# mapbox/robosat

Measured on AMD Instinct MI355X. Metric: 512x512 tiles/sec train+predict, 1/2/4/8 MI355X; mIoU vs CPU ref, higher is better.
Workload: dtype f32; 1 GPU; rs predict ResNet50-UNet, bs=16 3x512x512 fp32 per GPU, 2 classes (BASELINE configs[1]); parallelism=tiles sharded over 1 rank(s), no collective

## Files before the change

### include/robosat_hip.h

```cpp
#ifndef ROBOSAT_HIP_H
#define ROBOSAT_HIP_H

#include <stdint.h>

#ifdef __cplusplus
extern "C" {
#endif

#define RS_EINVAL (-22)

typedef void* rs_stream_t;

typedef uint16_t rs_bf16;
#define RS_F32 0
#define RS_BF16 1

int rs_abi_version(void);

typedef struct rs_conv_desc {
  int32_t N;
  int32_t Hs, Ws;
  int32_t C1, C2;
  int32_t ups;
  int32_t kh, kw, stride, pad;
  int32_t Ho, Wo;
  int32_t Cout;
  int32_t relu;
  int32_t stem;
} rs_conv_desc;

int rs_conv2d_fwd(const rs_conv_desc* d, const float* src1, const float* src2, const float* weight,
                  const float* scale, const float* shift, const float* residual, const float* relu_mask, float* out,
                  rs_stream_t stream);

int rs_conv2d_tile(const rs_conv_desc* d);
const char* rs_conv2d_tile_name(int tile);

int rs_pack_stem_weight(const float* w_krsc, float* packed, int Cout, int kh, int kw, int Cin, rs_stream_t stream);


int rs_nchw_to_nhwc4(const float* x, float* y, int N, int C, int H, int W, rs_stream_t stream);

int rs_maxpool2d_fwd(const float* x, float* y, uint8_t* argmax, int N, int H, int W, int C, int k, int stride, int pad,
                     int Ho, int Wo, rs_stream_t stream);

int rs_bn_fold(const float* gamma, const float* beta, const float* mean, const float* var, float eps, float* scale,
               float* shift, int C, rs_stream_t stream);

int rs_final_conv1x1(const float* x, const float* w, const float* bias, float* out, int N, int H, int W, int Cin,
                     int C, int softmax, rs_stream_t stream);



long rs_conv2d_wgrad_workspace_bytes(const rs_conv_desc* d);
int rs_conv2d_wgrad_form(const rs_conv_desc* d);
int rs_conv2d_wgrad(const rs_conv_desc* d, const float* dy, const float* src1, const float* src2, float* dw,
                    void* workspace, rs_stream_t stream);
int rs_unpack_stem_weight(const float* packed, float* w_krsc, int Cout, int kh, int kw, int Cin, rs_stream_t stream);

int rs_pack_dgrad_weight(const float* w_krsc, float* out, int Cout, int kh, int kw, int Cin, rs_stream_t stream);

long rs_bn_workspace_bytes(long M, int C);
int rs_bn_train_stats(const float* y, long M, int C, float eps, float momentum, const float* gamma, const float* beta,
                      float* mean, float* invstd, float* scale, float* shift, float* running_mean, float* running_var,
                      long long* num_batches_tracked, void* workspace, rs_stream_t stream);
int rs_bn_apply(const float* y, const float* scale, const float* shift, const float* residual, float* out, long M, int C,
                int relu, rs_stream_t stream);
int rs_bn_bwd(const float* dz, const float* zmask, const float* y, const float* mean, const float* invstd,
              const float* gamma, float* dy, float* dmasked, float* dgamma, float* dbeta, long M, int C, void* workspace,
              rs_stream_t stream);

int rs_maxpool2d_bwd(const float* dy, const uint8_t* argmax, float* dx, int N, int H, int W, int C, int k, int stride,
                     int pad, int Ho, int Wo, int accumulate, rs_stream_t stream);

int rs_upsample2x_bwd(const float* dup, float* d1, float* d2, const float* mask1, const float* mask2, int N, int H, int W,
                      int C1, int C2, int accumulate1, rs_stream_t stream);

long rs_final_conv1x1_bwd_workspace_bytes(int Cin, int C);
int rs_final_conv1x1_bwd(const float* x, const float* w, const float* dlogits, float* dx, float* dw, float* db, int N, int H,
                         int W, int Cin, int C, int relu_mask, void* workspace, rs_stream_t stream);


long rs_nll_loss_workspace_bytes(void);
int rs_nll_loss_fwd(const float* logits, const long long* targets, const float* weight, float* loss, float* stats, int N,
                    int C, int H, int W, int mode, float gamma, void* workspace, rs_stream_t stream);
int rs_nll_loss_bwd(const float* logits, const long long* targets, const float* weight, const float* stats,
                    const float* grad_out, float* dlogits, int N, int C, int H, int W, int mode, float gamma,
                    rs_stream_t stream);

long rs_miou_loss_workspace_bytes(int N, int C);
int rs_miou_loss_fwd(const float* logits, const long long* targets, const float* weight, float* loss, float* stats, int N,
                     int C, int H, int W, void* workspace, rs_stream_t stream);
int rs_miou_loss_bwd(const float* logits, const long long* targets, const float* weight, const float* stats,
                     const float* grad_out, float* dlogits, int N, int C, int H, int W, rs_stream_t stream);

long rs_lovasz_workspace_bytes(int N, int C, int H, int W);
int rs_lovasz_fwd(const float* logits, const long long* targets, float* loss, float* grad_unit, int N, int C, int H, int W,
                  void* workspace, rs_stream_t stream);
int rs_scale_by_scalar(const float* src, const float* scalar, float* dst, long n, rs_stream_t stream);

long rs_lovasz_softmax_workspace_bytes(int N, int C, int H, int W, int per_image);
int rs_lovasz_softmax_fwd(const float* logits, const long long* targets, float* loss, float* grad_unit, float* probs_out, int N,
                          int C, int H, int W, int per_image, int all_classes, void* workspace, rs_stream_t stream);

int rs_confusion_counts(const float* scores, const long long* targets, unsigned long long* counts, int N, int C, int H,
                        int W, rs_stream_t stream);


int rs_conv2d_fwd_bf16(const rs_conv_desc* d, const rs_bf16* src1, const rs_bf16* src2, const rs_bf16* weight,
                       const float* scale, const float* shift, const rs_bf16* residual, const rs_bf16* relu_mask,
                       rs_bf16* out, rs_stream_t stream);
int rs_conv2d_tile_bf16(const rs_conv_desc* d);
int rs_conv2d_config(const rs_conv_desc* d, int es, int form, int* tile, int* rowb);
int rs_conv2d_set_tuning(int tile, int rowb);
int rs_set_knob(const char* name, int value);
int rs_get_knob(const char* name, int* value);
const char* rs_conv2d_tile_name_bf16(int tile);

long rs_conv2d_wgrad_bf16_workspace_bytes(const rs_conv_desc* d);
int rs_conv2d_wgrad_bf16_form(const rs_conv_desc* d);
int rs_conv2d_wgrad_bf16_tile(const rs_conv_desc* d);
int rs_conv2d_wgrad_bf16(const rs_conv_desc* d, const rs_bf16* dy, const rs_bf16* src1, const rs_bf16* src2, float* dw,
                         void* workspace, rs_stream_t stream);

int rs_cast_f32_to_bf16(const float* src, rs_bf16* dst, long n, rs_stream_t stream);
int rs_cast_bf16_to_f32_scaled(const rs_bf16* src, float* dst, long n, float scale, rs_stream_t stream);
int rs_cast_f32_to_bf16_scaled(const float* src, rs_bf16* dst, long n, float scale, rs_stream_t stream);
int rs_pack_dgrad_weight_bf16(const float* w_krsc, rs_bf16* out, int Cout, int kh, int kw, int Cin, rs_stream_t stream);

int rs_nchw_to_nhwc4_bf16(const float* x, rs_bf16* y, int N, int C, int H, int W, rs_stream_t stream);
int rs_pack_stem_weight_bf16(const float* w_krsc, rs_bf16* packed, int Cout, int kh, int kw, int Cin, rs_stream_t stream);
int rs_stem_conv_fwd_bf16(const rs_bf16* x, const rs_bf16* w_packed, const float* scale, const float* shift, rs_bf16* out,
                          int N, int H, int W, int relu, rs_stream_t stream);
long rs_stem_conv_wgrad_bf16_workspace_bytes(int N, int H, int W);
int rs_stem_conv_wgrad_bf16(const rs_bf16* dy, const rs_bf16* x, float* dw_packed, int N, int H, int W, void* workspace,
                            rs_stream_t stream);

int rs_maxpool2d_fwd_dt(const void* x, int x_dtype, void* y, int y_dtype, uint8_t* argmax, int N, int H, int W, int C, int k,
                        int stride, int pad, int Ho, int Wo, rs_stream_t stream);
int rs_maxpool2d_bwd_dt(const void* dy, int dy_dtype, const uint8_t* argmax, void* dx, int dx_dtype, int N, int H, int W,
                        int C, int k, int stride, int pad, int Ho, int Wo, int accumulate, rs_stream_t stream);
int rs_final_conv1x1_dt(const void* x, int x_dtype, const float* w, const float* bias, float* out, int N, int H, int W,
                        int Cin, int C, int softmax, rs_stream_t stream);
int rs_final_conv1x1_bwd_dt(const void* x, const float* w, const float* dlogits, void* dx, float* dw, float* db, int dtype,
                            int N, int H, int W, int Cin, int C, int relu_mask, void* workspace, rs_stream_t stream);
int rs_bn_train_stats_dt(const void* y, int dtype, long M, int C, float eps, float momentum, const float* gamma,
                         const float* beta, float* mean, float* invstd, float* scale, float* shift, float* running_mean,
                         float* running_var, long long* num_batches_tracked, void* workspace, rs_stream_t stream);
int rs_bn_apply_dt(const void* y, const float* scale, const float* shift, const void* residual, void* out, int dtype, long M,
                   int C, int relu, rs_stream_t stream);
int rs_bn_bwd_dt(const void* dz, const void* zmask, const void* y, const float* mean, const float* invstd, const float* gamma,
                 void* dy, void* dmasked, float* dgamma, float* dbeta, int dtype, long M, int C, void* workspace,
                 rs_stream_t stream);
int rs_upsample2x_bwd_dt(const void* dup, void* d1, void* d2, const void* mask1, const void* mask2, int dtype, int N, int H,
                         int W, int C1, int C2, int accumulate1, rs_stream_t stream);

long rs_conv2d_bnstats_rows(const rs_conv_desc* d);
long rs_conv2d_bnstats_rows_dt(const rs_conv_desc* d, int dtype);
int rs_conv2d_fwd_bnstats_dt(const rs_conv_desc* d, int dtype, const void* src1, const void* src2, const void* weight,
                             void* out, float* stats_partial, rs_stream_t stream);
int rs_bn_finalize_stats(const float* partial, long rows, long M, int C, float eps, float momentum, const float* gamma,
                         const float* beta, float* mean, float* invstd, float* scale, float* shift, float* running_mean,
                         float* running_var, long long* num_batches_tracked, void* workspace, rs_stream_t stream);

int rs_pack_phase_weight_dt(const float* w_krsc, void* out, int dtype, int Cout, int Cin, rs_stream_t stream);
int rs_pack_s2_dgrad_phase_weight_dt(const float* w_krsc, void* out, int dtype, int Cout, int Cin, rs_stream_t stream);
int rs_conv2d_fwd_phase_dt(const rs_conv_desc* d, int dtype, const void* src1, const void* src2, const void* weight_phase,
                           const float* scale, const float* shift, const void* residual, const void* relu_mask, void* out,
                           rs_stream_t stream);

int rs_conv2d_phase_wino_ok(const rs_conv_desc* d);
const char* rs_conv2d_phase_wino_name(const rs_conv_desc* d);
int rs_pack_wino_phase_weight(const float* w_phase, float* u, int Cout, int Cin, rs_stream_t stream);
int rs_conv2d_fwd_phase_wino(const rs_conv_desc* d, const float* src1, const float* src2, const float* u, float* out,
                             rs_stream_t stream);
int rs_conv2d_dgrad_phase_wino_ok(const rs_conv_desc* d);
const char* rs_conv2d_dgrad_phase_wino_name(const rs_conv_desc* d);
int rs_pack_wino_dgrad_weight(const float* wd4x4, float* u, int Cin, int Cout, rs_stream_t stream);
int rs_conv2d_dgrad_phase_wino(const rs_conv_desc* d, const float* dz, const float* u, float* out, const float* mask, float* out2,
                               const float* mask2, int csplit, rs_stream_t stream);

int rs_conv2d_wino33_ok(const rs_conv_desc* d);
const char* rs_conv2d_wino33_name(const rs_conv_desc* d);
int rs_pack_wino33_weight(const float* w_krsc, float* u, int Cout, int Cin, rs_stream_t stream);
int rs_conv2d_fwd_wino33(const rs_conv_desc* d, const float* src, const float* u, const float* scale, const float* shift, float* out,
                         rs_stream_t stream);
int rs_conv2d_wino33_head_ok(const rs_conv_desc* d, int C);
const char* rs_conv2d_wino33_head_name(void);
int rs_conv2d_fwd_wino33_head(const rs_conv_desc* d, const float* src, const float* u, const float* scale, const float* shift,
                              const float* final_w, const float* final_b, int C, int mode, const double* anchors, int overlap,
                              float* out, uint8_t* qout, rs_stream_t stream);
int rs_bottleneck_tail_f32(const float* x, const float* w3, const float* scale3, const float* shift3, const float* identity,
                           const float* w1, const float* scale1, const float* shift1, float* out, float* z, long M, int C1, int Cmid,
                           int C2, rs_stream_t stream);
int rs_conv1x1_wave_f32(const float* x, const float* w, const float* scale, const float* shift, const float* residual, int relu, float* out,
                        long M, int C1, int Cout, rs_stream_t stream);
long rs_conv2d_wino33_stats_rows(const rs_conv_desc* d);
int rs_conv2d_fwd_wino33_stats(const rs_conv_desc* d, const float* src, const float* u, float* out, float* stats, rs_stream_t stream);
int rs_conv2d_dgrad_wino33(const rs_conv_desc* d, const float* dy, const float* u, const float* mask, const uint8_t* mask_bits,
                           const float* bn_y, const float* bn_mean, const float* bn_invstd, float* out, float* stats,
                           rs_stream_t stream);

int rs_pack_dgrad_phase_weight_dt(const float* w_krsc, void* out, int dtype, int Cout, int Cin, rs_stream_t stream);
typedef struct rs_wprep_item {
  const float* w;
  rs_bf16* cast;
  rs_bf16* dgrad;
  int Cout, taps, Cin;
  int tile_begin;
} rs_wprep_item;
int rs_weight_prep_bf16(const rs_wprep_item* items_dev, int n, int total_tiles, rs_stream_t stream);
int rs_weight_prep_f32(const rs_wprep_item* items_dev, int n, int total_tiles, rs_stream_t stream);
int rs_combine_dgrad_phase_weight_dt(const float* w_dgrad, void* out, int dtype, int Cout, int Cin, rs_stream_t stream);
int rs_conv2d_fwd_split_dt(const rs_conv_desc* d, int dtype, const void* src1, const void* weight, void* out1, const void* mask1,
                           void* out2, const void* mask2, int csplit, rs_stream_t stream);
int rs_cat_split_bwd_dt(const void* dcat, void* d1, void* d2, const void* mask1, const void* mask2, int dtype, int N, int H,
                        int W, int C1, int C2, int accumulate1, rs_stream_t stream);
int rs_scatter_add_stride2_dt(const void* t, void* out, int dtype, int N, int Hs, int Ws, int Ho, int Wo, int C, rs_stream_t stream);

int rs_conv2d_dgrad_bnstats_dt(const rs_conv_desc* d, int dtype, const void* dy, const void* weight, const void* residual,
                               const void* relu_mask, const void* bn_y, const float* bn_mean, const float* bn_invstd,
                               void* out, float* stats_partial, rs_stream_t stream);
int rs_bn_bwd_from_partials_dt(const void* g, const void* y, const float* mean, const float* invstd, const float* gamma,
                               void* dy, float* dgamma, float* dbeta, const float* partial, long rows, int dtype, long M,
                               int C, void* workspace, rs_stream_t stream);
int rs_bn_apply_bits_dt(const void* y, const float* scale, const float* shift, const void* residual, void* out,
                        unsigned char* bits, int dtype, long M, int C, int relu, rs_stream_t stream);
int rs_conv2d_dgrad_bnstats_bits_dt(const rs_conv_desc* d, int dtype, const void* dy, const void* weight, const void* residual,
                                    const unsigned char* relu_mask_bits, const void* bn_y, const float* bn_mean,
                                    const float* bn_invstd, void* out, float* stats_partial, rs_stream_t stream);


int rs_u8_to_nhwc4_norm(const uint8_t* img, float* out, const float* mean, const float* std, int N, int H, int W, int C,
                        rs_stream_t stream);

int rs_final_conv1x1_quantize_dt(const void* x, int x_dtype, const float* w, const float* bias, const double* anchors,
                                 uint8_t* out, int N, int H, int W, int Cin, int C, int overlap, rs_stream_t stream);

int rs_final_conv1x1_argmax_dt(const void* x, int x_dtype, const float* w, const float* bias, uint8_t* out, int N, int H,
                               int W, int Cin, int C, rs_stream_t stream);

#define RS_TTA_IN_U8 0
#define RS_TTA_IN_F32 1
#define RS_TTA_PROBS 0
#define RS_TTA_QUANTIZE 1
#define RS_TTA_ARGMAX 2
int rs_tta_fan_out(const void* x, int x_kind, const float* mean, const float* std, void* out, int out_dtype, const int* ops,
                   int V, int N, int H, int W, int C, rs_stream_t stream);
int rs_tta_merge(const float* probs, const int* ops, int V, int mode, const double* anchors, int overlap, void* out, int N,
                 int C, int H, int W, rs_stream_t stream);


int rs_confusion_matrix(const float* scores, const int64_t* targets, int64_t* counts, int N, int C, int H, int W,
                        rs_stream_t stream);

int rs_label_histogram_u8(const uint8_t* labels, long n, int64_t* counts256, rs_stream_t stream);

int rs_softvote_masks(const uint8_t* q, const double* weights, const double* anchors, uint8_t* out, int K, long P, int C,
                      rs_stream_t stream);

int rs_augment_tiles(const uint8_t* images, const uint8_t* masks, const int32_t* index, const int32_t* op, const float* mean,
                     const float* std, float* out_images, int64_t* out_masks, int N, int S, int C, rs_stream_t stream);


int rs_features_clean_form(int H, int W);
long rs_features_clean_workspace_bytes(int B, int H, int W);
int rs_features_clean(const uint8_t* images, uint8_t* out, void* workspace, int B, int H, int W, int index, int eps_open,
                      const int32_t* dx_open, int eps_close, const int32_t* dx_close, int form, rs_stream_t stream);

int rs_features_label(const uint8_t* masks, int32_t* labels, int32_t* err, int B, int H, int W, rs_stream_t stream);

int rs_features_components(const int32_t* labels, int32_t* slotmap, int32_t* raw, int32_t* table, int32_t* counters,
                           long capacity, int B, int H, int W, int min_area, rs_stream_t stream);

int rs_features_edges(const int32_t* labels, const int32_t* table, long rows, uint8_t* keep, int32_t* edges, long capacity,
                      int32_t* counter, int B, int H, int W, rs_stream_t stream);

int rs_features_halo(const uint8_t* src, uint8_t* dst, const int32_t* nbr, int T, int H, int W, int A, int fill, int crop,
                     rs_stream_t stream);
int rs_features_stitch_labels(int32_t* labels, const int32_t* nbr, int32_t* err, int T, int H, int W, rs_stream_t stream);
int rs_features_components_stitched(const int32_t* labels, const int32_t* origin, int32_t* slotmap, int32_t* raw, int32_t* table,
                                    int32_t* counters, long capacity, int T, int H, int W, int min_area, rs_stream_t stream);
int rs_features_edges_stitched(const int32_t* labels, const int32_t* nbr, const int32_t* origin, const int32_t* table, long rows,
                               uint8_t* keep, int32_t* edges, long capacity, int32_t* counter, int T, int H, int W,
                               rs_stream_t stream);

int rs_features_thin(const uint8_t* masks, uint8_t* out, void* workspace, const int32_t* nbr, int32_t* counters, int B, int H, int W,
                     int pairs, int resume, rs_stream_t stream);
int rs_features_skeleton_links(const uint8_t* skeleton, const int32_t* labels, const int32_t* nbr, const int32_t* origin,
                               const int32_t* table, long rows, uint8_t* keep, int32_t* links, long capacity, int32_t* counter, int B,
                               int H, int W, rs_stream_t stream);


#ifdef __cplusplus
}
#endif
#endif
```

### robosat_amd/_lib.py

```python

import ctypes
import os
from ctypes import POINTER, c_char_p, c_float, c_int, c_int32, c_long, c_void_p

import torch

_HERE = os.path.dirname(os.path.abspath(__file__))
LIB_PATH = os.environ.get("ROBOSAT_HIP_LIB") or os.path.join(_HERE, "librobosat_hip.so")

RS_EINVAL = -22
ABI_VERSION = 24
RS_F32, RS_BF16 = 0, 1
RS_TTA_IN_U8, RS_TTA_IN_F32 = 0, 1
RS_TTA_PROBS, RS_TTA_QUANTIZE, RS_TTA_ARGMAX = 0, 1, 2


class ConvDesc(ctypes.Structure):

    _fields_ = [
        ("N", c_int32), ("Hs", c_int32), ("Ws", c_int32), ("C1", c_int32), ("C2", c_int32), ("ups", c_int32),
        ("kh", c_int32), ("kw", c_int32), ("stride", c_int32), ("pad", c_int32), ("Ho", c_int32), ("Wo", c_int32),
        ("Cout", c_int32), ("relu", c_int32), ("stem", c_int32),
    ]


P = c_void_p

SIGNATURES = {
    "rs_abi_version": (c_int, []),
    "rs_conv2d_fwd": (c_int, [POINTER(ConvDesc), P, P, P, P, P, P, P, P, P]),
    "rs_conv2d_tile": (c_int, [POINTER(ConvDesc)]),
    "rs_conv2d_tile_name": (c_char_p, [c_int]),
    "rs_pack_stem_weight": (c_int, [P, P, c_int, c_int, c_int, c_int, P]),
    "rs_nchw_to_nhwc4": (c_int, [P, P, c_int, c_int, c_int, c_int, P]),
    "rs_maxpool2d_fwd": (c_int, [P, P, P, c_int, c_int, c_int, c_int, c_int, c_int, c_int, c_int, c_int, P]),
    "rs_bn_fold": (c_int, [P, P, P, P, c_float, P, P, c_int, P]),
    "rs_final_conv1x1": (c_int, [P, P, P, P, c_int, c_int, c_int, c_int, c_int, c_int, P]),
    "rs_conv2d_wgrad_workspace_bytes": (c_long, [POINTER(ConvDesc)]),
    "rs_conv2d_wgrad": (c_int, [POINTER(ConvDesc), P, P, P, P, P, P]),
    "rs_unpack_stem_weight": (c_int, [P, P, c_int, c_int, c_int, c_int, P]),
    "rs_pack_dgrad_weight": (c_int, [P, P, c_int, c_int, c_int, c_int, P]),
    "rs_bn_workspace_bytes": (c_long, [c_long, c_int]),
    "rs_bn_train_stats": (c_int, [P, c_long, c_int, c_float, c_float, P, P, P, P, P, P, P, P, P, P, P]),
    "rs_bn_apply": (c_int, [P, P, P, P, P, c_long, c_int, c_int, P]),
    "rs_bn_bwd": (c_int, [P, P, P, P, P, P, P, P, P, P, c_long, c_int, P, P]),
    "rs_maxpool2d_bwd": (c_int, [P, P, P, c_int, c_int, c_int, c_int, c_int, c_int, c_int, c_int, c_int, c_int, P]),
    "rs_upsample2x_bwd": (c_int, [P, P, P, P, P, c_int, c_int, c_int, c_int, c_int, c_int, P]),
    "rs_final_conv1x1_bwd_workspace_bytes": (c_long, [c_int, c_int]),
    "rs_final_conv1x1_bwd": (c_int, [P, P, P, P, P, P, c_int, c_int, c_int, c_int, c_int, c_int, P, P]),
    "rs_nll_loss_workspace_bytes": (c_long, []),
    "rs_nll_loss_fwd": (c_int, [P, P, P, P, P, c_int, c_int, c_int, c_int, c_int, c_float, P, P]),
    "rs_nll_loss_bwd": (c_int, [P, P, P, P, P, P, c_int, c_int, c_int, c_int, c_int, c_float, P]),
    "rs_miou_loss_workspace_bytes": (c_long, [c_int, c_int]),
    "rs_miou_loss_fwd": (c_int, [P, P, P, P, P, c_int, c_int, c_int, c_int, P, P]),
    "rs_miou_loss_bwd": (c_int, [P, P, P, P, P, P, c_int, c_int, c_int, c_int, P]),
    "rs_lovasz_workspace_bytes": (c_long, [c_int, c_int, c_int, c_int]),
    "rs_lovasz_fwd": (c_int, [P, P, P, P, c_int, c_int, c_int, c_int, P, P]),
    "rs_scale_by_scalar": (c_int, [P, P, P, c_long, P]),
    "rs_lovasz_softmax_workspace_bytes": (c_long, [c_int, c_int, c_int, c_int, c_int]),
    "rs_lovasz_softmax_fwd": (c_int, [P, P, P, P, P, c_int, c_int, c_int, c_int, c_int, c_int, P, P]),
    "rs_confusion_counts": (c_int, [P, P, P, c_int, c_int, c_int, c_int, P]),
    "rs_conv2d_fwd_bf16": (c_int, [POINTER(ConvDesc), P, P, P, P, P, P, P, P, P]),
    "rs_conv2d_tile_bf16": (c_int, [POINTER(ConvDesc)]),
    "rs_conv2d_config": (c_int, [POINTER(ConvDesc), c_int, c_int, POINTER(c_int), POINTER(c_int)]),
    "rs_conv2d_set_tuning": (c_int, [c_int, c_int]),
    "rs_set_knob": (c_int, [c_char_p, c_int]),
    "rs_get_knob": (c_int, [c_char_p, POINTER(c_int)]),
    "rs_conv2d_tile_name_bf16": (c_char_p, [c_int]),
    "rs_conv2d_wgrad_bf16_workspace_bytes": (c_long, [POINTER(ConvDesc)]),
    "rs_conv2d_wgrad_bf16_form": (c_int, [POINTER(ConvDesc)]),
    "rs_conv2d_wgrad_form": (c_int, [POINTER(ConvDesc)]),
    "rs_conv2d_wgrad_bf16_tile": (c_int, [POINTER(ConvDesc)]),
    "rs_conv2d_wgrad_bf16": (c_int, [POINTER(ConvDesc), P, P, P, P, P, P]),
    "rs_cast_f32_to_bf16": (c_int, [P, P, c_long, P]),
    "rs_cast_bf16_to_f32_scaled": (c_int, [P, P, c_long, c_float, P]),
    "rs_cast_f32_to_bf16_scaled": (c_int, [P, P, c_long, c_float, P]),
    "rs_weight_prep_bf16": (c_int, [P, c_int, c_int, P]),
    "rs_weight_prep_f32": (c_int, [P, c_int, c_int, P]),
    "rs_pack_dgrad_weight_bf16": (c_int, [P, P, c_int, c_int, c_int, c_int, P]),
    "rs_maxpool2d_fwd_dt": (c_int, [P, c_int, P, c_int, P, c_int, c_int, c_int, c_int, c_int, c_int, c_int, c_int, c_int, P]),
    "rs_maxpool2d_bwd_dt": (c_int, [P, c_int, P, P, c_int, c_int, c_int, c_int, c_int, c_int, c_int, c_int, c_int, c_int, c_int, P]),
    "rs_final_conv1x1_dt": (c_int, [P, c_int, P, P, P, c_int, c_int, c_int, c_int, c_int, c_int, P]),
    "rs_final_conv1x1_bwd_dt": (c_int, [P, P, P, P, P, P, c_int, c_int, c_int, c_int, c_int, c_int, c_int, P, P]),
    "rs_bn_train_stats_dt": (c_int, [P, c_int, c_long, c_int, c_float, c_float, P, P, P, P, P, P, P, P, P, P, P]),
    "rs_bn_apply_dt": (c_int, [P, P, P, P, P, c_int, c_long, c_int, c_int, P]),
    "rs_bn_bwd_dt": (c_int, [P, P, P, P, P, P, P, P, P, P, c_int, c_long, c_int, P, P]),
    "rs_upsample2x_bwd_dt": (c_int, [P, P, P, P, P, c_int, c_int, c_int, c_int, c_int, c_int, c_int, P]),
    "rs_conv2d_bnstats_rows": (c_long, [POINTER(ConvDesc)]),
    "rs_conv2d_bnstats_rows_dt": (c_long, [POINTER(ConvDesc), c_int]),
    "rs_conv2d_fwd_bnstats_dt": (c_int, [POINTER(ConvDesc), c_int, P, P, P, P, P, P]),
    "rs_bn_finalize_stats": (c_int, [P, c_long, c_long, c_int, c_float, c_float, P, P, P, P, P, P, P, P, P, P, P]),
    "rs_pack_phase_weight_dt": (c_int, [P, P, c_int, c_int, c_int, P]),
    "rs_pack_s2_dgrad_phase_weight_dt": (c_int, [P, P, c_int, c_int, c_int, P]),
    "rs_conv2d_fwd_phase_dt": (c_int, [POINTER(ConvDesc), c_int, P, P, P, P, P, P, P, P, P]),
    "rs_conv2d_phase_wino_ok": (c_int, [POINTER(ConvDesc)]),
    "rs_conv2d_phase_wino_name": (c_char_p, [POINTER(ConvDesc)]),
    "rs_pack_wino_phase_weight": (c_int, [P, P, c_int, c_int, P]),
    "rs_conv2d_fwd_phase_wino": (c_int, [POINTER(ConvDesc), P, P, P, P, P]),
    "rs_conv2d_dgrad_phase_wino_ok": (c_int, [POINTER(ConvDesc)]),
    "rs_conv2d_dgrad_phase_wino_name": (c_char_p, [POINTER(ConvDesc)]),
    "rs_pack_wino_dgrad_weight": (c_int, [P, P, c_int, c_int, P]),
    "rs_conv2d_dgrad_phase_wino": (c_int, [POINTER(ConvDesc), P, P, P, P, P, P, c_int, P]),
    "rs_conv2d_wino33_ok": (c_int, [POINTER(ConvDesc)]),
    "rs_conv2d_wino33_name": (c_char_p, [POINTER(ConvDesc)]),
    "rs_pack_wino33_weight": (c_int, [P, P, c_int, c_int, P]),
    "rs_conv2d_fwd_wino33": (c_int, [POINTER(ConvDesc), P, P, P, P, P, P]),
    "rs_conv2d_wino33_head_ok": (c_int, [POINTER(ConvDesc), c_int]),
    "rs_conv2d_wino33_head_name": (c_char_p, []),
    "rs_conv2d_fwd_wino33_head": (c_int, [POINTER(ConvDesc), P, P, P, P, P, P, c_int, c_int, P, c_int, P, P, P]),
    "rs_bottleneck_tail_f32": (c_int, [P, P, P, P, P, P, P, P, P, P, c_long, c_int, c_int, c_int, P]),
    "rs_conv1x1_wave_f32": (c_int, [P, P, P, P, P, c_int, P, c_long, c_int, c_int, P]),
    "rs_conv2d_wino33_stats_rows": (c_long, [POINTER(ConvDesc)]),
    "rs_conv2d_fwd_wino33_stats": (c_int, [POINTER(ConvDesc), P, P, P, P, P]),
    "rs_conv2d_dgrad_wino33": (c_int, [POINTER(ConvDesc), P, P, P, P, P, P, P, P, P, P]),
    "rs_pack_dgrad_phase_weight_dt": (c_int, [P, P, c_int, c_int, c_int, P]),
    "rs_combine_dgrad_phase_weight_dt": (c_int, [P, P, c_int, c_int, c_int, P]),
    "rs_conv2d_fwd_split_dt": (c_int, [POINTER(ConvDesc), c_int, P, P, P, P, P, P, c_int, P]),
    "rs_cat_split_bwd_dt": (c_int, [P, P, P, P, P, c_int, c_int, c_int, c_int, c_int, c_int, c_int, P]),
    "rs_scatter_add_stride2_dt": (c_int, [P, P, c_int, c_int, c_int, c_int, c_int, c_int, c_int, P]),
    "rs_conv2d_dgrad_bnstats_dt": (c_int, [POINTER(ConvDesc), c_int, P, P, P, P, P, P, P, P, P, P]),
    "rs_bn_bwd_from_partials_dt": (c_int, [P, P, P, P, P, P, P, P, P, c_long, c_int, c_long, c_int, P, P]),
    "rs_bn_apply_bits_dt": (c_int, [P, P, P, P, P, P, c_int, c_long, c_int, c_int, P]),
    "rs_conv2d_dgrad_bnstats_bits_dt": (c_int, [POINTER(ConvDesc), c_int, P, P, P, P, P, P, P, P, P, P]),
    "rs_nchw_to_nhwc4_bf16": (c_int, [P, P, c_int, c_int, c_int, c_int, P]),
    "rs_pack_stem_weight_bf16": (c_int, [P, P, c_int, c_int, c_int, c_int, P]),
    "rs_stem_conv_fwd_bf16": (c_int, [P, P, P, P, P, c_int, c_int, c_int, c_int, P]),
    "rs_stem_conv_wgrad_bf16_workspace_bytes": (c_long, [c_int, c_int, c_int]),
    "rs_stem_conv_wgrad_bf16": (c_int, [P, P, P, c_int, c_int, c_int, P, P]),
    "rs_u8_to_nhwc4_norm": (c_int, [P, P, POINTER(c_float), POINTER(c_float), c_int, c_int, c_int, c_int, P]),
    "rs_final_conv1x1_quantize_dt": (c_int, [P, c_int, P, P, P, P, c_int, c_int, c_int, c_int, c_int, c_int, P]),
    "rs_final_conv1x1_argmax_dt": (c_int, [P, c_int, P, P, P, c_int, c_int, c_int, c_int, c_int, P]),
    "rs_tta_fan_out": (c_int, [P, c_int, POINTER(c_float), POINTER(c_float), P, c_int, POINTER(c_int), c_int, c_int, c_int, c_int, c_int, P]),
    "rs_tta_merge": (c_int, [P, POINTER(c_int), c_int, c_int, P, c_int, P, c_int, c_int, c_int, c_int, P]),
    "rs_confusion_matrix": (c_int, [P, P, P, c_int, c_int, c_int, c_int, P]),
    "rs_label_histogram_u8": (c_int, [P, c_long, P, P]),
    "rs_softvote_masks": (c_int, [P, P, P, P, c_int, c_long, c_int, P]),
    "rs_augment_tiles": (c_int, [P, P, P, P, POINTER(c_float), POINTER(c_float), P, P, c_int, c_int, c_int, P]),
    "rs_features_clean_form": (c_int, [c_int, c_int]),
    "rs_features_clean_workspace_bytes": (c_long, [c_int, c_int, c_int]),
    "rs_features_clean": (c_int, [P, P, P, c_int, c_int, c_int, c_int, c_int, POINTER(c_int32), c_int, POINTER(c_int32), c_int, P]),
    "rs_features_label": (c_int, [P, P, P, c_int, c_int, c_int, P]),
    "rs_features_components": (c_int, [P, P, P, P, P, c_long, c_int, c_int, c_int, c_int, P]),
    "rs_features_edges": (c_int, [P, P, c_long, P, P, c_long, P, c_int, c_int, c_int, P]),
    "rs_features_halo": (c_int, [P, P, P, c_int, c_int, c_int, c_int, c_int, c_int, P]),
    "rs_features_stitch_labels": (c_int, [P, P, P, c_int, c_int, c_int, P]),
    "rs_features_components_stitched": (c_int, [P, P, P, P, P, P, c_long, c_int, c_int, c_int, c_int, P]),
    "rs_features_edges_stitched": (c_int, [P, P, P, P, c_long, P, P, c_long, P, c_int, c_int, c_int, P]),
    "rs_features_thin": (c_int, [P, P, P, P, P, c_int, c_int, c_int, c_int, c_int, P]),
    "rs_features_skeleton_links": (c_int, [P, P, P, P, P, c_long, P, P, c_long, P, c_int, c_int, c_int, P]),
}

_lib = None


def kernel_source_digest():

    import hashlib

    h = hashlib.sha256()
    src = os.path.join(_HERE, "csrc")
    names = sorted(n for n in os.listdir(src) if n.endswith((".hip", ".h")))
    for path in [os.path.join(src, n) for n in names] + [os.path.join(os.path.dirname(_HERE), "include", "robosat_hip.h")]:
        h.update(os.path.basename(path).encode() + b"\0")
        with open(path, "rb") as fp:
            h.update(fp.read())
    return h.hexdigest()[:16]


def lib():

    global _lib
    if _lib is None:
        if not os.path.exists(LIB_PATH):
            raise RuntimeError(
                "robosat_amd: {} is missing -- the MI355X kernels are not built and there is no CPU fallback. "
                "Build with `python -c 'import __graft_entry__ as g; g.build()'` "
                "(or `make -C robosat_amd/csrc`).".format(LIB_PATH)
            )
        handle = ctypes.CDLL(LIB_PATH, mode=ctypes.RTLD_GLOBAL)
        for name, (restype, argtypes) in SIGNATURES.items():
            fn = getattr(handle, name)
            fn.restype, fn.argtypes = restype, argtypes
        got = handle.rs_abi_version()
        if got != ABI_VERSION:
            raise RuntimeError("robosat_amd: librobosat_hip.so ABI {} != expected {}".format(got, ABI_VERSION))
        _lib = handle
    return _lib


def check(rc, what):
    if rc != 0:
        if rc == RS_EINVAL:
            raise ValueError("{}: invalid arguments (RS_EINVAL)".format(what))
        raise RuntimeError("{}: HIP error {}".format(what, rc))
```

### robosat_amd/csrc/common.h

```cpp
#pragma once
#include <hip/hip_runtime.h>
#include <stdint.h>

#include "../../include/robosat_hip.h"

typedef float f32x4 __attribute__((ext_vector_type(4)));
typedef float f32x16 __attribute__((ext_vector_type(16)));
typedef __bf16 bf16_t;
typedef __bf16 bf16x4 __attribute__((ext_vector_type(4)));
typedef __bf16 bf16x8 __attribute__((ext_vector_type(8)));
typedef unsigned int u32x2 __attribute__((ext_vector_type(2)));
typedef unsigned int u32x4 __attribute__((ext_vector_type(4)));
typedef short s16x4 __attribute__((ext_vector_type(4)));
typedef short s16x8 __attribute__((ext_vector_type(8)));

__device__ __forceinline__ f32x4 rs_ld4(const float* p) { return *reinterpret_cast<const f32x4*>(p); }
__device__ __forceinline__ f32x4 rs_ld4(const bf16_t* p) {
  return __builtin_convertvector(*reinterpret_cast<const bf16x4*>(p), f32x4);
}
__device__ __forceinline__ void rs_st4(float* p, f32x4 v) { *reinterpret_cast<f32x4*>(p) = v; }
__device__ __forceinline__ void rs_st4(bf16_t* p, f32x4 v) {
  *reinterpret_cast<bf16x4*>(p) = __builtin_convertvector(v, bf16x4);
}
__device__ __forceinline__ float rs_ld1(const float* p) { return *p; }
__device__ __forceinline__ float rs_ld1(const bf16_t* p) { return (float)*p; }

template <int V>
struct rs_vecf {
  float v[V];
};
template <int V, typename T>
__device__ __forceinline__ rs_vecf<V> rs_ldv(const T* p) {
  rs_vecf<V> r;
  if constexpr (V == 4) {
    const f32x4 t = rs_ld4(p);
#pragma unroll
    for (int e = 0; e < 4; ++e) r.v[e] = t[e];
  } else if constexpr (sizeof(T) == 2) {
    const bf16x8 t = *reinterpret_cast<const bf16x8*>(p);
#pragma unroll
    for (int e = 0; e < 8; ++e) r.v[e] = (float)t[e];
  } else {
    const f32x4 a = *reinterpret_cast<const f32x4*>(p), b = *(reinterpret_cast<const f32x4*>(p) + 1);
#pragma unroll
    for (int e = 0; e < 4; ++e) r.v[e] = a[e], r.v[4 + e] = b[e];
  }
  return r;
}
template <int V, typename T>
__device__ __forceinline__ void rs_stv(T* p, const rs_vecf<V>& r) {
  if constexpr (V == 4) {
    rs_st4(p, f32x4{r.v[0], r.v[1], r.v[2], r.v[3]});
  } else if constexpr (sizeof(T) == 2) {
    bf16x8 t;
#pragma unroll
    for (int e = 0; e < 8; ++e) t[e] = (bf16_t)r.v[e];
    *reinterpret_cast<bf16x8*>(p) = t;
  } else {
    *reinterpret_cast<f32x4*>(p) = f32x4{r.v[0], r.v[1], r.v[2], r.v[3]};
    *(reinterpret_cast<f32x4*>(p) + 1) = f32x4{r.v[4], r.v[5], r.v[6], r.v[7]};
  }
}

__device__ __forceinline__ void rs_ld_row32(const bf16_t* p, float (&v)[32]) {
  bf16x8 t[4];
#pragma unroll
  for (int j = 0; j < 4; ++j) t[j] = *reinterpret_cast<const bf16x8*>(p + j * 8);
#pragma unroll
  for (int j = 0; j < 4; ++j)
#pragma unroll
    for (int e = 0; e < 8; ++e) v[j * 8 + e] = (float)t[j][e];
}
__device__ __forceinline__ void rs_ld_row32(const float* p, float (&v)[32]) {
  f32x4 t[8];
#pragma unroll
  for (int j = 0; j < 8; ++j) t[j] = *reinterpret_cast<const f32x4*>(p + j * 4);
#pragma unroll
  for (int j = 0; j < 8; ++j)
#pragma unroll
    for (int e = 0; e < 4; ++e) v[j * 4 + e] = t[j][e];
}
__device__ __forceinline__ void rs_st_row32(bf16_t* p, const float (&v)[32]) {
#pragma unroll
  for (int j = 0; j < 4; ++j) {
    bf16x8 t;
#pragma unroll
    for (int e = 0; e < 8; ++e) t[e] = (bf16_t)v[j * 8 + e];
    *reinterpret_cast<bf16x8*>(p + j * 8) = t;
  }
}
__device__ __forceinline__ void rs_st_row32(float* p, const float (&v)[32]) {
#pragma unroll
  for (int j = 0; j < 8; ++j) {
    f32x4 t;
#pragma unroll
    for (int e = 0; e < 4; ++e) t[e] = v[j * 4 + e];
    *reinterpret_cast<f32x4*>(p + j * 4) = t;
  }
}

#define RS_LAUNCH_RESULT() ((int)hipGetLastError())

__device__ __forceinline__ void rs_lds_writes_done() { asm volatile("s_waitcnt lgkmcnt(0)" ::: "memory"); }

__device__ __forceinline__ int rs_xcd_remap(int b, int nwg) {
  const int xcd = b & 7, k = b >> 3;
  const int q = nwg >> 3, r = nwg & 7;
  const int base = (xcd < r) ? xcd * (q + 1) : r * (q + 1) + (xcd - r) * q;
  return base + k;
}

__device__ __forceinline__ float rs_xor16_sum(float v) {
  float a = v, b = v;
  asm("s_nop 1\n\tv_permlane16_swap_b32 %0, %1" : "+v"(a), "+v"(b));
  return a + b;
}
__device__ __forceinline__ float rs_xor32_sum(float v) {
  float a = v, b = v;
  asm("s_nop 1\n\tv_permlane32_swap_b32 %0, %1" : "+v"(a), "+v"(b));
  return a + b;
}

__device__ __forceinline__ float rs_row16_sum(float v) {
  v += __builtin_bit_cast(float, __builtin_amdgcn_update_dpp(0, __builtin_bit_cast(int, v), 0x128, 0xf, 0xf, false));
  v += __builtin_bit_cast(float, __builtin_amdgcn_update_dpp(0, __builtin_bit_cast(int, v), 0x124, 0xf, 0xf, false));
  v += __builtin_bit_cast(float, __builtin_amdgcn_update_dpp(0, __builtin_bit_cast(int, v), 0x122, 0xf, 0xf, false));
  v += __builtin_bit_cast(float, __builtin_amdgcn_update_dpp(0, __builtin_bit_cast(int, v), 0x121, 0xf, 0xf, false));
  return v;
}

__device__ __forceinline__ float rs_wave_sum(float v) {
#pragma unroll
  for (int o = 32; o > 0; o >>= 1) v += __shfl_xor(v, o, 64);
  return v;
}

__device__ __forceinline__ double rs_wave_sum(double v) {
#pragma unroll
  for (int o = 32; o > 0; o >>= 1) v += __shfl_xor(v, o, 64);
  return v;
}

static inline int rs_cdiv(long a, long b) { return (int)((a + b - 1) / b); }

inline int rs_cu_count() {
  static const int n = [] {
    int dev = 0, cus = 0;
    if (hipGetDevice(&dev) != hipSuccess || hipDeviceGetAttribute(&cus, hipDeviceAttributeMultiprocessorCount, dev) != hipSuccess || cus <= 0)
      cus = 256;
    return cus;
  }();
  return n;
}

struct rs_fastdiv {
  unsigned int mul;
  unsigned int shift;
  unsigned int div;
};

static inline rs_fastdiv rs_make_fastdiv(unsigned int d) {
  rs_fastdiv f;
  unsigned int s = 0;
  while ((1ull << s) < d) ++s;
  f.shift = s;
  f.mul = (unsigned int)((((1ull << s) - d) << 32) / d + 1);
  f.div = d;
  return f;
}

__host__ __device__ __forceinline__ unsigned int rs_div(unsigned int n, const rs_fastdiv f) {
#if defined(__HIP_DEVICE_COMPILE__)
  return (__umulhi(n, f.mul) + n) >> f.shift;
#else
  return (unsigned int)((((unsigned long long)n * f.mul) >> 32) + n) >> f.shift;
#endif
}

struct RsKnobs {
  int conv_tile = -1;
  int conv_rowb = 0;
  int conv_big = 1;
  int conv_min256 = 384;
  int conv_halo = 1;
  int conv_halo_min = 192;
  int conv_halo512 = -1;
  int conv1x1_ew = -1;
  int conv1x1_np = 0;
  int conv1x1_ew_bf16 = 0;
  int halo_ko = 0;
  int wgrad_f32_phase = 1;
  int wgrad_f32_dma = -1;
  int wgrad_f32_blocks = 2048;
  int wgrad_f32_wino = 1;
  int wgrad_f32_wino_blocks = 1024;
  int wgrad_f32_wino33 = 1;
  int wgrad_f32_wino33_blocks = 256;
  int wgrad_blocks = 96;
  int wgrad_blocks_phase = 1536;
  int wgrad_phase4 = 1;
  int wgrad_blocks_phase4 = 256;
  int wgrad_ring = 3;
  int lovasz_xcd = 1;
  int wino_wide = 1;
};
__attribute__((visibility("hidden"))) RsKnobs& rs_knobs();

__attribute__((visibility("hidden"))) int rs_wgrad_thin_plan(const rs_conv_desc* d, int* blocks, int* slices);
__attribute__((visibility("hidden"))) int rs_wgrad_thin_launch(const rs_conv_desc* d, const void* dy, const void* src,
                                                               float* partial, void* stream);

__attribute__((visibility("hidden"))) int rs_conv_thin_bf16_launch(int mode, const void* src, const void* wgt, const void* mask,
                                                                   void* out, int N, int Hs, int Ws, int relu, void* stream);

__attribute__((visibility("hidden"))) long rs_reduce_scratch_floats(long n, int splits);
__attribute__((visibility("hidden"))) int rs_reduce_splits(const float* ws, float* out, long n, int splits, float* scratch,
                                                           void* stream);

__attribute__((visibility("hidden"))) int rs_conv_dma_f32(const rs_conv_desc* d, const float* src1, const float* src2,
                                                          const float* weight, const float* scale, const float* shift,
                                                          const float* residual, const float* relu_mask, float* out,
                                                          void* stream);
__attribute__((visibility("hidden"))) int rs_conv_dma_tile(const rs_conv_desc* d);
```

### robosat_amd/csrc/conv_igemm_dma.hip

```cpp
#include "conv_igemm_dma_kernel.h"

namespace {

__global__ void pack_dgrad_weight_bf16_kernel(const float* __restrict__ w, bf16_t* __restrict__ out, int Cout, int taps,
                                              int Cin) {
  __shared__ float tile[32][33];
  const int tap = blockIdx.z;
  const int ci0 = blockIdx.x * 32, co0 = blockIdx.y * 32;
  const int tx = threadIdx.x & 31, ty = threadIdx.x >> 5;
  for (int r = ty; r < 32; r += 8) {
    const int co = co0 + r, ci = ci0 + tx;
    tile[r][tx] = (co < Cout && ci < Cin) ? w[((long)co * taps + tap) * Cin + ci] : 0.f;
  }
  __syncthreads();
  const int ftap = taps - 1 - tap;
  for (int r = ty; r < 32; r += 8) {
    const int ci = ci0 + r, co = co0 + tx;
    if (ci < Cin && co < Cout) out[((long)ci * taps + ftap) * Cout + co] = (bf16_t)tile[tx][r];
  }
}

template <typename T>
__global__ __launch_bounds__(256) void weight_prep_kernel(const rs_wprep_item* __restrict__ items, int n) {
  __shared__ float tile[32][33];
  const int bid = blockIdx.x;
  int lo = 0, hi = n - 1;
  while (lo < hi) {
    const int mid = (lo + hi + 1) >> 1;
    if (items[mid].tile_begin <= bid) lo = mid;
    else hi = mid - 1;
  }
  const rs_wprep_item it = items[lo];
  int t = bid - it.tile_begin;
  const int tci = (it.Cin + 31) / 32, tco = (it.Cout + 31) / 32;
  const int ci0 = (t % tci) * 32;
  t /= tci;
  const int co0 = (t % tco) * 32;
  const int tap = t / tco;
  const int tx = threadIdx.x & 31, ty = threadIdx.x >> 5;
  T* cast = reinterpret_cast<T*>(it.cast);
  T* dgrad = reinterpret_cast<T*>(it.dgrad);
  for (int r = ty; r < 32; r += 8) {
    const int co = co0 + r, ci = ci0 + tx;
    float v = 0.f;
    if (co < it.Cout && ci < it.Cin) {
      const long i = ((long)co * it.taps + tap) * it.Cin + ci;
      v = it.w[i];
      if (cast) cast[i] = (T)v;
    }
    tile[r][tx] = v;
  }
  if (!dgrad) return;
  __syncthreads();
  const int ftap = it.taps - 1 - tap;
  for (int r = ty; r < 32; r += 8) {
    const int ci = ci0 + r, co = co0 + tx;
    if (ci < it.Cin && co < it.Cout) dgrad[((long)ci * it.taps + ftap) * it.Cout + co] = (T)tile[tx][r];
  }
}

extern "C" int rs_weight_prep_bf16(const rs_wprep_item* items_dev, int n, int total_tiles, rs_stream_t stream) {
  if (!items_dev || n <= 0 || total_tiles <= 0) return RS_EINVAL;
  weight_prep_kernel<bf16_t><<<total_tiles, 256, 0, (hipStream_t)stream>>>(items_dev, n);
  return RS_LAUNCH_RESULT();
}

extern "C" int rs_weight_prep_f32(const rs_wprep_item* items_dev, int n, int total_tiles, rs_stream_t stream) {
  if (!items_dev || n <= 0 || total_tiles <= 0) return RS_EINVAL;
  weight_prep_kernel<float><<<total_tiles, 256, 0, (hipStream_t)stream>>>(items_dev, n);
  return RS_LAUNCH_RESULT();
}

const char* const kTileNamesBf16[NTILES] = {"conv_igemm_bf16<128x128>", "conv_igemm_bf16<128x64>", "conv_igemm_bf16<128x32>",
                                            "conv_igemm_bf16<64x64>", "", "conv_igemm_bf16<256x128>",
                                            "conv_igemm_bf16<256x256>", "conv_thin_bf16", "conv_halo_bf16", "conv1x1_ew_bf16<128x128>"};
const int kTileBM[NTILES] = {128, 128, 128, 64, 128, 256, 256, 128, 256, 128};
const int kTileBN[NTILES] = {128, 64, 32, 64, 64, 128, 256, 32, 128, 64};

struct Tuning {
  int tile, rowb, big, min256, halo, halo_min, halo512;
};
Tuning tuning() {
  const RsKnobs& k = rs_knobs();
  return {k.conv_tile, k.conv_rowb, k.conv_big, k.conv_min256, k.conv_halo, k.conv_halo_min, k.conv_halo512};
}

bool valid(const rs_conv_desc* d) {
  if (!d) return false;
  if (d->N <= 0 || d->Hs <= 0 || d->Ws <= 0 || d->Ho <= 0 || d->Wo <= 0) return false;
  if (d->kh <= 0 || d->kw <= 0 || d->kh > kMaxK || d->kw > kMaxK || d->stride <= 0 || d->pad < 0) return false;
  if (d->Cout <= 0 || (d->Cout % 32) != 0) return false;
  if (d->ups < 0 || d->ups > 2 || d->stem) return false;
  if (d->C1 <= 0 || (d->C1 % 32) != 0 || d->C2 < 0 || (d->C2 % 32) != 0) return false;
  return true;
}

bool phase_ok(const rs_conv_desc* d) {
  return d->ups == 1 && d->kh == 3 && d->kw == 3 && d->stride == 1 && d->pad == 1 && d->Ho == 2 * d->Hs && d->Wo == 2 * d->Ws;
}

int pick_tile(const rs_conv_desc* d, bool phase4 = false, int es = 4, bool stats = false) {
  const long M = phase4 ? (long)d->N * d->Hs * d->Ws * 4 : (long)d->N * d->Ho * d->Wo;
  const long want = 512;
  const Tuning tu = tuning();
  const int ft = tu.tile;
  if (ft >= 0 && ft < NTILES && ft != TSTEM_RESERVED && ft != TTHIN && ft != THALO && ft != TEW && (d->Cout % kTileBN[ft] == 0 || (ft == T128x128 && d->Cout > 128)) &&
      (ft != T256x256 || (es == 2 && !stats)))
    return ft;
  if (tu.big && es == 2 && !stats) {
    const long mrows = phase4 ? (long)d->N * d->Hs * d->Ws : M;
    const long nph = phase4 ? 4 : 1;
    const long nk128 = (long)(phase4 ? 4 : d->kh * d->kw) * (d->C1 + d->C2) * es / 128;
    if (d->Cout % 256 == 0 && nk128 >= ((phase4 || d->kh > 1) ? 16 : 32) && rs_cdiv(mrows, 256) * (d->Cout / 256) * nph >= tu.min256) return T256x256;
  }
  if (es == 4 && !stats && !phase4 && (long)d->kh * d->kw * (d->C1 + d->C2) <= 64 && d->Cout % 64 == 0 && (long)rs_cdiv(M, 128) * (d->Cout / 64) >= want)
    return T128x64;
  if (d->Cout % 128 == 0 && (long)rs_cdiv(M, 128) * (d->Cout / 128) >= want) return T128x128;
  if (d->Cout > 128 && d->Cout % 128 != 0 && (long)rs_cdiv(d->Cout, 128) * 128 * 4 <= (long)d->Cout * 5 &&
      (long)rs_cdiv(M, 128) * rs_cdiv(d->Cout, 128) >= want)
    return T128x128;
  if (d->Cout % 64 == 0) {
    if ((long)rs_cdiv(M, 128) * (d->Cout / 64) >= want) return T128x64;
    return T64x64;
  }
  return T128x32;
}

int pick_rowb(const rs_conv_desc* d, int es, bool phase4 = false, bool stats = false) {
  const int forced = tuning().rowb;
  const int tile = pick_tile(d, phase4, es, stats);
  if (forced == 64 || forced == 128) return forced;
  const long blocks = (long)rs_cdiv((long)d->N * d->Ho * d->Wo, kTileBM[tile]) * rs_cdiv(d->Cout, kTileBN[tile]);
  const long nk128 = (long)(phase4 ? 4 : d->kh * d->kw) * (d->C1 + d->C2) * es / 128;
  if (es == 4) return (nk128 <= 16 || blocks >= 2048) ? 64 : 128;
  if (tile == T256x256) return nk128 <= 8 ? 64 : 128;
  if (kTileBN[tile] <= 64) return nk128 <= 4 ? 64 : 128;
  if (phase4 || d->kh == 4) return 128;
  if (nk128 <= 8 || (blocks >= 2048 && nk128 <= 24)) return 64;
  return 128;
}

void launch(int rowb, bool phase4, int epi, int tile, int grid, hipStream_t s, const ConvArgsT<float>& a) {
  if (phase4) rs_conv_launch_f32_phase_eval(tile, rowb, grid, s, a);
  else if (epi == EPI_STATS) rs_conv_launch_f32_plain_stats(tile, rowb, grid, s, a);
  else if (epi == EPI_BWD) rs_conv_launch_f32_plain_bwd(tile, rowb, grid, s, a);
  else rs_conv_launch_f32_plain_eval(tile, rowb, grid, s, a);
}
void launch(int rowb, bool phase4, int epi, int tile, int grid, hipStream_t s, const ConvArgsT<bf16_t>& a) {
  if (phase4) rs_conv_launch_bf16_phase_eval(tile, rowb, grid, s, a);
  else if (epi == EPI_STATS) rs_conv_launch_bf16_plain_stats(tile, rowb, grid, s, a);
  else if (epi == EPI_BWD) rs_conv_launch_bf16_plain_bwd(tile, rowb, grid, s, a);
  else rs_conv_launch_bf16_plain_eval(tile, rowb, grid, s, a);
}

int thin_mode(const rs_conv_desc* d, bool phase4, bool plain_epilogue) {
  const int ft = tuning().tile;
  if (!plain_epilogue || (ft != -1 && ft != TTHIN) || d->C2 != 0) return -1;
  if (phase4) return (d->C1 == 128 && d->Cout == 32) ? 1 : -1;
  if (d->ups != 0) return -1;
  if (d->kh == 3 && d->kw == 3 && d->stride == 1 && d->pad == 1 && d->C1 == 32 && d->Cout == 32 && d->Ho == d->Hs && d->Wo == d->Ws) return 0;
  if (d->kh == 4 && d->kw == 4 && d->stride == 2 && d->pad == 1 && d->C1 == 32 && d->Cout == 128 && 2 * d->Ho == d->Hs && 2 * d->Wo == d->Ws)
    return 2;
  return -1;
}

int halo_mode(const rs_conv_desc* d, bool phase4, int csplit, int epi, int* bn_out, int* bm_out = nullptr) {
  const Tuning tu = tuning();
  if (!tu.halo || (tu.tile != -1 && tu.tile != THALO)) return HALO_NONE;
  bool big = tu.tile == THALO ? tu.rowb == 64 : tu.halo512 != 0;
  const bool c64 = (d->C1 % 64) == 0 && (d->C2 % 64) == 0;
  if ((d->C1 % 32) != 0 || (d->C2 % 32) != 0) return HALO_NONE;
  int bn;
  if (d->Cout % 128 == 0) bn = 128;
  else if (d->Cout > 128 && (long)rs_cdiv(d->Cout, 128) * 128 * 4 <= (long)d->Cout * 5) bn = 128;
  else if (d->Cout % 64 == 0) bn = 64;
  else return HALO_NONE;
  if (csplit > 0 && (csplit % bn) != 0) return HALO_NONE;
  int mode, gh, gw;
  if (phase4) {
    mode = HALO_PHASE, gh = d->Hs, gw = d->Ws;
  } else if (d->ups == 0 && d->kh == 3 && d->kw == 3 && d->stride == 1 && d->pad == 1 && d->Ho == d->Hs && d->Wo == d->Ws) {
    mode = HALO_33, gh = d->Ho, gw = d->Wo;
  } else if (d->ups == 0 && d->kh == 4 && d->kw == 4 && d->stride == 2 && d->pad == 1 && d->Hs == 2 * d->Ho && d->Ws == 2 * d->Wo && d->C2 == 0) {
    mode = HALO_DG4, gh = d->Ho, gw = d->Wo;
  } else {
    return HALO_NONE;
  }
  if (mode != HALO_33 && epi != EPI_EVAL) return HALO_NONE;
  if (tu.tile != THALO && tu.halo512 < 0) big = (long)d->N * (gh / 16) * (gw / 32) >= 256;
  if (big && (bn != 128 || (gh % 16) != 0)) big = false;
  if (!big && !c64) return HALO_NONE;
  const int ph = big ? 16 : 8;
  if ((gh % ph) != 0 || (gw % 32) != 0) return HALO_NONE;
  const long cmax = d->C1 > d->C2 ? d->C1 : d->C2;
  if ((long)d->Hs * d->Ws * cmax * 2 >= (1L << 31)) return HALO_NONE;
  const long blocks = (long)d->N * (gh / ph) * (gw / 32) * rs_cdiv(d->Cout, bn) * (phase4 ? 4 : 1);
  if (tu.tile != THALO) {
    if (blocks < tu.halo_min) return HALO_NONE;
    if (mode == HALO_33 && bn != 128) return HALO_NONE;
    if (mode == HALO_PHASE && d->Cout % 256 == 0) return HALO_NONE;
    if (mode == HALO_DG4 && d->C1 < 128) return HALO_NONE;
  }
  if (bn_out) *bn_out = bn;
  if (bm_out) *bm_out = ph * 32;
  return mode;
}

bool ew_f32_mode(const rs_conv_desc* d, bool phase4, bool plain) {
  const int ew = rs_knobs().conv1x1_ew;
  return ew != 0 && tuning().tile < 0 && !phase4 && plain && rs_conv1x1_ew_f32_ok(d) && (ew > 0 || d->C1 <= 64);
}

bool np_f32_mode(const rs_conv_desc* d, bool phase4, bool plain, bool has_res) {
  const int np = rs_knobs().conv1x1_np;
  return np != 0 && tuning().tile < 0 && !phase4 && plain && rs_conv1x1_np_f32_ok(d) && (np > 0 || (has_res && d->C1 >= 128 && d->C1 <= 512));
}

template <typename T>
int conv_fwd(const rs_conv_desc* d, const void* src1, const void* src2, const void* weight, const float* scale,
             const float* shift, const void* residual, const void* relu_mask, void* out, rs_stream_t stream,
             float* stats = nullptr, const void* bn_y = nullptr, const float* bn_mean = nullptr,
             const float* bn_invstd = nullptr, bool phase4 = false, void* out2 = nullptr, const void* mask2 = nullptr,
             int csplit = 0, const unsigned char* mask_bits = nullptr) {
  if (!valid(d) || !src1 || !weight || !out) return RS_EINVAL;
  if (mask_bits && (relu_mask || !bn_y || (d->Cout & 7))) return RS_EINVAL;
  if (out2 && (csplit <= 0 || csplit >= d->Cout || residual || stats)) return RS_EINVAL;
  if (phase4 && (!phase_ok(d) || stats)) return RS_EINVAL;
  if (d->C2 > 0 && !src2) return RS_EINVAL;
  constexpr long ES = (long)sizeof(T);
  if constexpr (sizeof(T) == 2) {
    const int tm = thin_mode(d, phase4, !scale && !shift && !residual && !stats && !out2);
    if (tm >= 0) {
      const int rc = rs_conv_thin_bf16_launch(tm, src1, weight, relu_mask, out, d->N, d->Hs, d->Ws, d->relu, stream);
      if (rc != RS_EINVAL) return rc;
    }
  }
  ConvArgsT<T> a;
  a.src1 = reinterpret_cast<const T*>(src1);
  a.src2 = reinterpret_cast<const T*>(src2);
  a.wgt = reinterpret_cast<const T*>(weight);
  a.scale = scale;
  a.shift = shift;
  a.res = reinterpret_cast<const T*>(residual);
  a.mask = reinterpret_cast<const T*>(relu_mask);
  a.out = reinterpret_cast<T*>(out);
  a.stats = stats;
  a.bn_y = reinterpret_cast<const T*>(bn_y);
  a.bn_mean = bn_mean;
  a.bn_invstd = bn_invstd;
  a.mask_bits = mask_bits;
  a.out2 = reinterpret_cast<T*>(out2);
  a.mask2 = reinterpret_cast<const T*>(mask2);
  a.csplit = csplit;
  a.N = d->N;
  a.Hs = d->Hs;
  a.Ws = d->Ws;
  a.C1 = d->C1;
  a.C2 = d->C2;
  a.phase4 = phase4 ? 1 : 0;
  a.ups = phase4 ? 0 : d->ups;
  a.Hv = a.ups == 0 ? d->Hs : (a.ups == 1 ? 2 * d->Hs : 2 * d->Hs - 1);
  a.Wv = a.ups == 0 ? d->Ws : (a.ups == 1 ? 2 * d->Ws : 2 * d->Ws - 1);
  a.kh = phase4 ? 2 : d->kh;
  a.kw = phase4 ? 2 : d->kw;
  a.stride = d->stride;
  a.pad = d->pad;
  a.Ho = d->Ho;
  a.Wo = d->Wo;
  a.Cout = d->Cout;
  if ((long)d->N * d->Ho * d->Wo >= (1L << 31)) return RS_EINVAL;
  const long M = phase4 ? (long)d->N * d->Hs * d->Ws : (long)d->N * d->Ho * d->Wo;
  a.M = (int)M;
  {
    const long cmax = d->C1 > d->C2 ? d->C1 : d->C2;
    const long img_bytes = (long)d->Hs * d->Ws * cmax * ES;
    const long rows_per_image = phase4 ? (long)d->Hs * d->Ws : (long)d->Ho * d->Wo;
    const long span = (512 / rows_per_image + 2) * img_bytes;
    if (span >= (1L << 31)) return RS_EINVAL;
    if ((long)d->Cout * d->kh * d->kw * (d->C1 + d->C2) * ES >= (1L << 31)) return RS_EINVAL;
  }
  const int kc128 = 128 / (int)ES;
  const bool can128 = d->C1 % kc128 == 0 && d->C2 % kc128 == 0;
  const int kc = (can128 && pick_rowb(d, (int)ES, phase4, stats != nullptr) == 128) ? kc128 : kc128 / 2;
  a.cpt = (d->C1 + d->C2) / kc;
  a.ntaps = a.kh * a.kw;
  a.nk = a.ntaps * a.cpt;
  a.Kw = a.nk * kc;
  a.relu = d->relu;
  a.tpx = a.tpi = 0;

  int epi = EPI_EVAL;
  if (stats) {
    epi = bn_y ? EPI_BWD : EPI_STATS;
    if (scale || shift || d->relu || out2) return RS_EINVAL;
    if (epi == EPI_STATS && (residual || relu_mask)) return RS_EINVAL;
    if (epi == EPI_BWD && (!bn_mean || !bn_invstd)) return RS_EINVAL;
  }
  if constexpr (sizeof(T) == 4) {
    if (ew_f32_mode(d, phase4, epi == EPI_EVAL && !relu_mask && !out2 && !mask_bits)) return rs_conv1x1_ew_f32_launch(a, (hipStream_t)stream);
#ifdef RS_EXP_BUILD
    if (np_f32_mode(d, phase4, epi == EPI_EVAL && !relu_mask && !out2 && !mask_bits, residual != nullptr)) return rs_conv1x1_np_f32_launch(a, (hipStream_t)stream);
#endif
  }
  if constexpr (sizeof(T) == 2) {
    int bn = 0, bm = 256;
    const int hm = halo_mode(d, phase4, out2 ? csplit : 0, epi, &bn, &bm);
    if (hm != HALO_NONE) {
      const int gh = hm == HALO_PHASE ? d->Hs : d->Ho, gw = hm == HALO_PHASE ? d->Ws : d->Wo;
      const int ctot = d->C1 + d->C2;
      a.cpt = ctot / (bm == 512 ? 32 : 64);
      a.nk = a.cpt * (hm == HALO_DG4 ? 4 : 1);
      a.Kw = (hm == HALO_PHASE ? 4 : (hm == HALO_33 ? 9 : 16)) * ctot;
      a.tpx = gw / 32;
      a.tpi = a.tpx * (gh / (bm / 32));
      a.ntiles = rs_cdiv(d->Cout, bn);
      const int grid = d->N * a.tpi * a.ntiles * (phase4 ? 4 : 1);
      hipStream_t hs = (hipStream_t)stream;
      if (bm == 512) bn |= 0x1000;
      if (hm == HALO_33) rs_conv_launch_bf16_halo33(bn, epi, grid, hs, a);
#ifdef RS_HALO_KO_BUILD
      else if (hm == HALO_PHASE && bn == 128 && rs_knobs().halo_ko) rs_conv_launch_bf16_halo_phase_ko(rs_knobs().halo_ko, grid, hs, a);
#endif
      else if (hm == HALO_PHASE) rs_conv_launch_bf16_halo_phase(bn, 0, grid, hs, a);
      else rs_conv_launch_bf16_halo_dg4(bn, 0, grid, hs, a);
      return RS_LAUNCH_RESULT();
    }
  }

  const int tile = pick_tile(d, phase4, (int)ES, stats != nullptr);
#ifdef RS_EXP_BUILD
  if constexpr (sizeof(T) == 2) {
    if (rs_knobs().conv1x1_ew_bf16 > 0 && tuning().tile < 0 && epi == EPI_STATS && !phase4 && kTileBM[tile] == 128 &&
        rs_conv1x1_ew_bf16_stats_ok(d))
      return rs_conv1x1_ew_bf16_stats_launch(a, (hipStream_t)stream);
  }
#endif
  if (out2 && (csplit % kTileBN[tile]) != 0) return RS_EINVAL;
  a.ntiles = rs_cdiv(d->Cout, kTileBN[tile]);
  const int grid = rs_cdiv(M, kTileBM[tile]) * a.ntiles * (phase4 ? 4 : 1);
  hipStream_t s = (hipStream_t)stream;
  launch(kc == kc128 ? 128 : 64, phase4, epi, tile, grid, s, a);
  return RS_LAUNCH_RESULT();
}

}

int rs_conv_dma_f32(const rs_conv_desc* d, const float* src1, const float* src2, const float* weight, const float* scale,
                    const float* shift, const float* residual, const float* relu_mask, float* out, void* stream) {
  return conv_fwd<float>(d, src1, src2, weight, scale, shift, residual, relu_mask, out, stream);
}

int rs_conv_dma_tile(const rs_conv_desc* d) { return valid(d) ? pick_tile(d) : RS_EINVAL; }

extern "C" int rs_conv2d_set_tuning(int tile, int rowb) {
  if (tile < -1 || tile >= NTILES || tile == TSTEM_RESERVED || tile == TEW || (rowb != 0 && rowb != 64 && rowb != 128)) return RS_EINVAL;
  rs_knobs().conv_tile = tile;
  rs_knobs().conv_rowb = rowb;
  return 0;
}

extern "C" int rs_conv2d_config(const rs_conv_desc* d, int es, int form, int* tile, int* rowb) {
  if (form < 0 || form > 3) return RS_EINVAL;
  const int phase4 = form & 1;
  const bool plain = (form & 2) == 0;
  if (!valid(d) || (es != 2 && es != 4) || (phase4 && !phase_ok(d))) return RS_EINVAL;
  const int kc128 = 128 / es;
  const bool can128 = d->C1 % kc128 == 0 && d->C2 % kc128 == 0;
  if (es == 2 && thin_mode(d, phase4 != 0, true) >= 0) {
    if (tile) *tile = TTHIN;
    if (rowb) *rowb = d->C1 * 2;
    return 0;
  }
  if (es == 2) {
    int bn = 0, bm = 256;
    if (halo_mode(d, phase4 != 0, 0, EPI_EVAL, &bn, &bm) != HALO_NONE) {
      if (tile) *tile = THALO;
      if (rowb) *rowb = bn | (bm == 512 ? 0x1000 : 0);
      return 0;
    }
  }
  if (es == 4 && ew_f32_mode(d, phase4 != 0, plain)) {
    if (tile) *tile = TEW;
    if (rowb) *rowb = 64;
    return 0;
  }
  if (tile) *tile = pick_tile(d, phase4 != 0, es);
  if (rowb) *rowb = (can128 && pick_rowb(d, es, phase4 != 0) == 128) ? 128 : 64;
  return 0;
}

template <typename T>
__global__ void pack_phase_weight_kernel(const float* __restrict__ w, T* __restrict__ out, int Cout, int Cin, long total) {
  const long i = (long)blockIdx.x * blockDim.x + threadIdx.x;
  if (i >= total) return;
  const int ci = (int)(i % Cin);
  long t = i / Cin;
  const int s = (int)(t & 1), r = (int)((t >> 1) & 1);
  t >>= 2;
  const int co = (int)(t % Cout);
  const int ph = (int)(t / Cout), py = ph >> 1, px = ph & 1;
  const int ky0 = py == 0 ? (r == 0 ? 0 : 1) : (r == 0 ? 0 : 2), ky1 = py == 0 ? (r == 0 ? 0 : 2) : (r == 0 ? 1 : 2);
  const int kx0 = px == 0 ? (s == 0 ? 0 : 1) : (s == 0 ? 0 : 2), kx1 = px == 0 ? (s == 0 ? 0 : 2) : (s == 0 ? 1 : 2);
  float acc = 0.f;
  for (int ky = ky0; ky <= ky1; ++ky)
    for (int kx = kx0; kx <= kx1; ++kx) acc += w[(((long)co * 3 + ky) * 3 + kx) * Cin + ci];
  out[i] = (T)acc;
}

template <typename T>
__global__ void pack_s2_dgrad_phase_weight_kernel(const float* __restrict__ w, T* __restrict__ out, int Cout, int Cin, long total) {
  const long i = (long)blockIdx.x * blockDim.x + threadIdx.x;
  if (i >= total) return;
  const int cd = (int)(i % Cout);
  long t = i / Cout;
  const int s = (int)(t & 1), r = (int)((t >> 1) & 1);
  t >>= 2;
  const int cg = (int)(t % Cin);
  const int ph = (int)(t / Cin), py = ph >> 1, px = ph & 1;
  const int ky = py == 0 ? (r == 1 ? 1 : -1) : (r == 0 ? 2 : 0);
  const int kx = px == 0 ? (s == 1 ? 1 : -1) : (s == 0 ? 2 : 0);
  out[i] = (T)((ky < 0 || kx < 0) ? 0.f : w[(((long)cd * 3 + ky) * 3 + kx) * Cin + cg]);
}

template <typename T>
__global__ void pack_dgrad_phase_weight_kernel(const float* __restrict__ w, T* __restrict__ out, int Cout, int Cin, long total) {
  const long i = (long)blockIdx.x * blockDim.x + threadIdx.x;
  if (i >= total) return;
  const int co = (int)(i % Cout);
  long t = i / Cout;
  const int tx = (int)(t & 3), ty = (int)((t >> 2) & 3);
  const int ci = (int)(t >> 4);
  const int ky0 = ty == 0 ? 2 : (ty == 1 ? 1 : 0), ky1 = ty == 0 ? 2 : (ty == 1 ? 2 : (ty == 2 ? 1 : 0));
  const int kx0 = tx == 0 ? 2 : (tx == 1 ? 1 : 0), kx1 = tx == 0 ? 2 : (tx == 1 ? 2 : (tx == 2 ? 1 : 0));
  float acc = 0.f;
  for (int ky = ky0; ky <= ky1; ++ky)
    for (int kx = kx0; kx <= kx1; ++kx) acc += w[(((long)co * 3 + ky) * 3 + kx) * Cin + ci];
  out[i] = (T)acc;
}

template <typename T>
__global__ void combine_dgrad_phase_weight_kernel(const float* __restrict__ wt, T* __restrict__ out, int Cout, long total) {
  const long i = (long)blockIdx.x * blockDim.x + threadIdx.x;
  if (i >= total) return;
  const int co = (int)(i % Cout);
  long t = i / Cout;
  const int tx = (int)(t & 3), ty = (int)((t >> 2) & 3);
  const long ci = t >> 4;
  const int ky0 = ty == 0 ? 2 : (ty == 1 ? 1 : 0), ky1 = ty == 0 ? 2 : (ty == 1 ? 2 : (ty == 2 ? 1 : 0));
  const int kx0 = tx == 0 ? 2 : (tx == 1 ? 1 : 0), kx1 = tx == 0 ? 2 : (tx == 1 ? 2 : (tx == 2 ? 1 : 0));
  float acc = 0.f;
  for (int ky = ky0; ky <= ky1; ++ky)
    for (int kx = kx0; kx <= kx1; ++kx) acc += wt[(ci * 9 + (8 - (ky * 3 + kx))) * Cout + co];
  out[i] = (T)acc;
}

extern "C" int rs_combine_dgrad_phase_weight_dt(const float* w_dgrad, void* out, int dtype, int Cout, int Cin,
                                                rs_stream_t stream) {
  if (!w_dgrad || !out || Cout <= 0 || Cin <= 0) return RS_EINVAL;
  const long total = 16L * Cout * Cin;
  hipStream_t s = (hipStream_t)stream;
  if (dtype == RS_F32)
    combine_dgrad_phase_weight_kernel<float><<<rs_cdiv(total, 256), 256, 0, s>>>(w_dgrad, reinterpret_cast<float*>(out), Cout, total);
  else if (dtype == RS_BF16)
    combine_dgrad_phase_weight_kernel<bf16_t><<<rs_cdiv(total, 256), 256, 0, s>>>(w_dgrad, reinterpret_cast<bf16_t*>(out), Cout, total);
  else
    return RS_EINVAL;
  return RS_LAUNCH_RESULT();
}

extern "C" int rs_pack_dgrad_phase_weight_dt(const float* w_krsc, void* out, int dtype, int Cout, int Cin, rs_stream_t stream) {
  if (!w_krsc || !out || Cout <= 0 || Cin <= 0) return RS_EINVAL;
  const long total = 16L * Cout * Cin;
  hipStream_t s = (hipStream_t)stream;
  if (dtype == RS_F32)
    pack_dgrad_phase_weight_kernel<float><<<rs_cdiv(total, 256), 256, 0, s>>>(w_krsc, reinterpret_cast<float*>(out), Cout, Cin, total);
  else if (dtype == RS_BF16)
    pack_dgrad_phase_weight_kernel<bf16_t><<<rs_cdiv(total, 256), 256, 0, s>>>(w_krsc, reinterpret_cast<bf16_t*>(out), Cout, Cin, total);
  else
    return RS_EINVAL;
  return RS_LAUNCH_RESULT();
}

extern "C" int rs_pack_s2_dgrad_phase_weight_dt(const float* w_krsc, void* out, int dtype, int Cout, int Cin, rs_stream_t stream) {
  if (!w_krsc || !out || Cout <= 0 || Cin <= 0) return RS_EINVAL;
  const long total = 16L * Cout * Cin;
  hipStream_t s = (hipStream_t)stream;
  if (dtype == RS_F32)
    pack_s2_dgrad_phase_weight_kernel<float><<<rs_cdiv(total, 256), 256, 0, s>>>(w_krsc, reinterpret_cast<float*>(out), Cout, Cin, total);
  else if (dtype == RS_BF16)
    pack_s2_dgrad_phase_weight_kernel<bf16_t><<<rs_cdiv(total, 256), 256, 0, s>>>(w_krsc, reinterpret_cast<bf16_t*>(out), Cout, Cin, total);
  else
    return RS_EINVAL;
  return RS_LAUNCH_RESULT();
}

extern "C" int rs_pack_phase_weight_dt(const float* w_krsc, void* out, int dtype, int Cout, int Cin, rs_stream_t stream) {
  if (!w_krsc || !out || Cout <= 0 || Cin <= 0) return RS_EINVAL;
  const long total = 16L * Cout * Cin;
  hipStream_t s = (hipStream_t)stream;
  if (dtype == RS_F32)
    pack_phase_weight_kernel<float><<<rs_cdiv(total, 256), 256, 0, s>>>(w_krsc, reinterpret_cast<float*>(out), Cout, Cin, total);
  else if (dtype == RS_BF16)
    pack_phase_weight_kernel<bf16_t><<<rs_cdiv(total, 256), 256, 0, s>>>(w_krsc, reinterpret_cast<bf16_t*>(out), Cout, Cin, total);
  else
    return RS_EINVAL;
  return RS_LAUNCH_RESULT();
}

extern "C" int rs_conv2d_fwd_split_dt(const rs_conv_desc* d, int dtype, const void* src1, const void* weight, void* out1,
                                      const void* mask1, void* out2, const void* mask2, int csplit, rs_stream_t stream) {
  if (!out2 || (d && d->C2 != 0)) return RS_EINVAL;
  if (dtype == RS_F32)
    return conv_fwd<float>(d, src1, nullptr, weight, nullptr, nullptr, nullptr, mask1, out1, stream, nullptr, nullptr, nullptr,
                           nullptr, false, out2, mask2, csplit);
  if (dtype == RS_BF16)
    return conv_fwd<bf16_t>(d, src1, nullptr, weight, nullptr, nullptr, nullptr, mask1, out1, stream, nullptr, nullptr,
                            nullptr, nullptr, false, out2, mask2, csplit);
  return RS_EINVAL;
}

extern "C" int rs_conv2d_fwd_phase_dt(const rs_conv_desc* d, int dtype, const void* src1, const void* src2,
                                      const void* weight_phase, const float* scale, const float* shift,
                                      const void* residual, const void* relu_mask, void* out, rs_stream_t stream) {
  if (dtype == RS_F32)
    return conv_fwd<float>(d, src1, src2, weight_phase, scale, shift, residual, relu_mask, out, stream, nullptr, nullptr,
                           nullptr, nullptr, true);
  if (dtype == RS_BF16)
    return conv_fwd<bf16_t>(d, src1, src2, weight_phase, scale, shift, residual, relu_mask, out, stream, nullptr, nullptr,
                            nullptr, nullptr, true);
  return RS_EINVAL;
}

extern "C" long rs_conv2d_bnstats_rows(const rs_conv_desc* d) {
  if (!valid(d)) return RS_EINVAL;
  return rs_cdiv((long)d->N * d->Ho * d->Wo, kTileBM[pick_tile(d, false, 4, true)]);
}

extern "C" long rs_conv2d_bnstats_rows_dt(const rs_conv_desc* d, int dtype) {
  if (!valid(d) || (dtype != RS_F32 && dtype != RS_BF16)) return RS_EINVAL;
  int bn = 0, bm = 256;
  if (dtype == RS_BF16 && halo_mode(d, false, 0, EPI_STATS, &bn, &bm) != HALO_NONE) return (long)d->N * (d->Ho / (bm / 32)) * (d->Wo / 32);
  return rs_conv2d_bnstats_rows(d);
}

extern "C" int rs_conv2d_dgrad_bnstats_dt(const rs_conv_desc* d, int dtype, const void* dy, const void* weight,
                                          const void* residual, const void* relu_mask, const void* bn_y,
                                          const float* bn_mean, const float* bn_invstd, void* out, float* stats_partial,
                                          rs_stream_t stream) {
  if (!stats_partial || !bn_y || !bn_mean || !bn_invstd || (d && d->C2 != 0)) return RS_EINVAL;
  if (dtype == RS_F32)
    return conv_fwd<float>(d, dy, nullptr, weight, nullptr, nullptr, residual, relu_mask, out, stream, stats_partial, bn_y,
                           bn_mean, bn_invstd);
  if (dtype == RS_BF16)
    return conv_fwd<bf16_t>(d, dy, nullptr, weight, nullptr, nullptr, residual, relu_mask, out, stream, stats_partial, bn_y,
                            bn_mean, bn_invstd);
  return RS_EINVAL;
}

extern "C" int rs_conv2d_dgrad_bnstats_bits_dt(const rs_conv_desc* d, int dtype, const void* dy, const void* weight,
                                               const void* residual, const unsigned char* relu_mask_bits, const void* bn_y,
                                               const float* bn_mean, const float* bn_invstd, void* out, float* stats_partial,
                                               rs_stream_t stream) {
  if (!stats_partial || !bn_y || !bn_mean || !bn_invstd || !relu_mask_bits || (d && d->C2 != 0)) return RS_EINVAL;
  if (dtype == RS_F32)
    return conv_fwd<float>(d, dy, nullptr, weight, nullptr, nullptr, residual, nullptr, out, stream, stats_partial, bn_y, bn_mean,
                           bn_invstd, false, nullptr, nullptr, 0, relu_mask_bits);
  if (dtype == RS_BF16)
    return conv_fwd<bf16_t>(d, dy, nullptr, weight, nullptr, nullptr, residual, nullptr, out, stream, stats_partial, bn_y, bn_mean,
                            bn_invstd, false, nullptr, nullptr, 0, relu_mask_bits);
  return RS_EINVAL;
}

extern "C" int rs_conv2d_fwd_bnstats_dt(const rs_conv_desc* d, int dtype, const void* src1, const void* src2,
                                        const void* weight, void* out, float* stats_partial, rs_stream_t stream) {
  if (!stats_partial) return RS_EINVAL;
  if (dtype == RS_F32) return conv_fwd<float>(d, src1, src2, weight, nullptr, nullptr, nullptr, nullptr, out, stream, stats_partial);
  if (dtype == RS_BF16) return conv_fwd<bf16_t>(d, src1, src2, weight, nullptr, nullptr, nullptr, nullptr, out, stream, stats_partial);
  return RS_EINVAL;
}

extern "C" int rs_conv2d_tile_bf16(const rs_conv_desc* d) { return valid(d) ? pick_tile(d, false, 2) : RS_EINVAL; }

extern "C" const char* rs_conv2d_tile_name_bf16(int tile) {
  return (tile >= 0 && tile < NTILES) ? kTileNamesBf16[tile] : "";
}

extern "C" int rs_conv2d_fwd_bf16(const rs_conv_desc* d, const rs_bf16* src1, const rs_bf16* src2, const rs_bf16* weight,
                                  const float* scale, const float* shift, const rs_bf16* residual, const rs_bf16* relu_mask,
                                  rs_bf16* out, rs_stream_t stream) {
  return conv_fwd<bf16_t>(d, src1, src2, weight, scale, shift, residual, relu_mask, out, stream);
}

extern "C" int rs_pack_dgrad_weight_bf16(const float* w_krsc, rs_bf16* out, int Cout, int kh, int kw, int Cin,
                                         rs_stream_t stream) {
  if (!w_krsc || !out || Cout <= 0 || kh <= 0 || kw <= 0 || Cin <= 0) return RS_EINVAL;
  dim3 grid(rs_cdiv(Cin, 32), rs_cdiv(Cout, 32), kh * kw);
  pack_dgrad_weight_bf16_kernel<<<grid, 256, 0, (hipStream_t)stream>>>(w_krsc, reinterpret_cast<bf16_t*>(out), Cout, kh * kw,
                                                                       Cin);
  return RS_LAUNCH_RESULT();
}
```

### robosat_amd/csrc/conv_igemm_dma_kernel.h

```cpp
#pragma once
#include <stdlib.h>

#include <type_traits>
#include <utility>

#include "lds_dma.h"

enum { EPI_EVAL = 0, EPI_STATS = 1, EPI_BWD = 2 };
constexpr int kMaxK = 4;
enum Tile { T128x128 = 0, T128x64, T128x32, T64x64, TSTEM_RESERVED, T256x128, T256x256, TTHIN, THALO, TEW, NTILES };
enum { HALO_NONE = 0, HALO_33 = 1, HALO_PHASE = 2, HALO_DG4 = 3 };

template <typename T>
struct ConvArgsT {
  const T* src1;
  const T* src2;
  const T* wgt;
  const float* scale;
  const float* shift;
  const T* res;
  const T* mask;
  T* out;
  float* stats;
  const T* bn_y;
  const float* bn_mean;
  const float* bn_invstd;
  const unsigned char* mask_bits;
  T* out2;
  const T* mask2;
  int csplit;
  int N, Hs, Ws, C1, C2, Hv, Wv, ups;
  int kh, kw, stride, pad, Ho, Wo, Cout;
  int M, cpt, nk, Kw, relu, ntiles, ntaps, phase4;
  int tpx, tpi;
};


#define RS_CONV_LAUNCHER(name, T) \
  __attribute__((visibility("hidden"))) void name(int tile, int rowb, int grid, hipStream_t s, const ConvArgsT<T>& a)
RS_CONV_LAUNCHER(rs_conv_launch_f32_plain_eval, float);
RS_CONV_LAUNCHER(rs_conv_launch_f32_plain_stats, float);
RS_CONV_LAUNCHER(rs_conv_launch_f32_plain_bwd, float);
RS_CONV_LAUNCHER(rs_conv_launch_f32_phase_eval, float);
RS_CONV_LAUNCHER(rs_conv_launch_bf16_plain_eval, bf16_t);
RS_CONV_LAUNCHER(rs_conv_launch_bf16_plain_stats, bf16_t);
RS_CONV_LAUNCHER(rs_conv_launch_bf16_plain_bwd, bf16_t);
RS_CONV_LAUNCHER(rs_conv_launch_bf16_phase_eval, bf16_t);
RS_CONV_LAUNCHER(rs_conv_launch_bf16_halo33, bf16_t);
RS_CONV_LAUNCHER(rs_conv_launch_bf16_halo_phase, bf16_t);
RS_CONV_LAUNCHER(rs_conv_launch_bf16_halo_dg4, bf16_t);
__attribute__((visibility("hidden"))) void rs_conv_launch_bf16_halo_phase_ko(int ko, int grid, hipStream_t s, const ConvArgsT<bf16_t>& a);
__attribute__((visibility("hidden"))) int rs_conv1x1_ew_f32_ok(const rs_conv_desc* d);
__attribute__((visibility("hidden"))) int rs_conv1x1_ew_f32_launch(const ConvArgsT<float>& a, hipStream_t s);
__attribute__((visibility("hidden"))) int rs_conv1x1_np_f32_ok(const rs_conv_desc* d);
__attribute__((visibility("hidden"))) int rs_conv1x1_np_f32_launch(const ConvArgsT<float>& a, hipStream_t s);
__attribute__((visibility("hidden"))) int rs_conv1x1_ew_bf16_stats_ok(const rs_conv_desc* d);
__attribute__((visibility("hidden"))) int rs_conv1x1_ew_bf16_stats_launch(const ConvArgsT<bf16_t>& a, hipStream_t s);

#ifdef RS_CONV_INSTANTIATE
namespace {

template <typename T>
struct Piece;
template <>
struct Piece<float> {
  __device__ static __forceinline__ void load(const float* p, float (&v)[4]) {
    const f32x4 t = *reinterpret_cast<const f32x4*>(p);
#pragma unroll
    for (int e = 0; e < 4; ++e) v[e] = t[e];
  }
  __device__ static __forceinline__ void round(const float (&v)[4], float (&w)[4]) {
#pragma unroll
    for (int e = 0; e < 4; ++e) w[e] = v[e];
  }
  __device__ static __forceinline__ void store(float* p, const float (&v)[4]) {
    f32x4 t;
#pragma unroll
    for (int e = 0; e < 4; ++e) t[e] = v[e];
    *reinterpret_cast<f32x4*>(p) = t;
  }
};
template <>
struct Piece<bf16_t> {
  __device__ static __forceinline__ void load(const bf16_t* p, float (&v)[8]) {
    const bf16x8 t = *reinterpret_cast<const bf16x8*>(p);
#pragma unroll
    for (int e = 0; e < 8; ++e) v[e] = (float)t[e];
  }
  __device__ static __forceinline__ void round(const float (&v)[8], float (&w)[8]) {
#pragma unroll
    for (int e = 0; e < 8; ++e) w[e] = (float)(bf16_t)v[e];
  }
  __device__ static __forceinline__ void store(bf16_t* p, const float (&v)[8]) {
    bf16x8 t;
#pragma unroll
    for (int e = 0; e < 8; ++e) t[e] = (bf16_t)v[e];
    *reinterpret_cast<bf16x8*>(p) = t;
  }
};

__device__ __forceinline__ void mma16(f32x16& acc, const u32x4 a, const u32x4 b, bf16_t) {
  acc = __builtin_amdgcn_mfma_f32_32x32x16_bf16(__builtin_bit_cast(bf16x8, a), __builtin_bit_cast(bf16x8, b), acc, 0, 0, 0);
}
__device__ __forceinline__ void mma16(f32x16& acc, const u32x4 a, const u32x4 b, float) {
  const f32x4 fa = __builtin_bit_cast(f32x4, a), fb = __builtin_bit_cast(f32x4, b);
#pragma unroll
  for (int t = 0; t < 4; ++t) acc = __builtin_amdgcn_mfma_f32_32x32x2f32(fa[t], fb[t], acc, 0, 0, 0);
}

constexpr unsigned int kDmaClamp = 0xFFFE0000u;
constexpr int kDmaOOB = (int)0xFFFF0000u;
static_assert((unsigned int)kDmaOOB > kDmaClamp && (unsigned int)kDmaOOB - kDmaClamp == 0x10000u && 0u - (unsigned int)kDmaOOB == 0x10000u,
              "the sentinel is out of range for every descriptor, with 64 KiB for soff on either side");

template <class F, int... I>
__device__ __forceinline__ void rb_for_each(F&& f, std::integer_sequence<int, I...>) {
  (f(std::integral_constant<int, I>()), ...);
}
constexpr int halo_tap_of_piece(int j, int ntap, int njh) { return j * (ntap - 2) / njh; }
constexpr int halo_pieces_at_tap(int t, int ntap, int njh) {
  int n = 0;
  for (int j = 0; j < njh; ++j) n += halo_tap_of_piece(j, ntap, njh) == t ? 1 : 0;
  return n;
}

constexpr int conv_waves_per_simd(int nw, int bm, int bn, int rowb, int es, int epi, int halo = 0) {
  if (halo) return 2;
  const int lds = 2 * (bm + bn) * rowb + 9 * bm * 4;
  const int blocks = 160 * 1024 / lds;
  const int w = blocks * nw / 4;
  const int cap = nw == 8 ? (bm * bn >= 256 * 256 ? 1 : 2) : ((es == 4 && epi == 2 && bm * bn >= 128 * 128) ? 2 : 4);
  return w < 1 ? 1 : (w > cap ? cap : w);
}

template <typename T, int BM, int BN, int WGM, int WGN, int ROWB, bool PHASE, int EPI, int HALO = HALO_NONE, int KO = 0>
__global__ __launch_bounds__(64 * WGM * WGN, conv_waves_per_simd(WGM * WGN, BM, BN, ROWB, (int)sizeof(T), EPI, HALO)) void conv_igemm_dma(
    const ConvArgsT<T> p) {
  static_assert(WGM * WGN == 4 || WGM * WGN == 8, "4 or 8 waves per block");
  static_assert(ROWB == 128 || ROWB == 64, "a K-chunk is a 128- or 64-byte row");
  constexpr int NBUF = 2;
  constexpr int NW = WGM * WGN;
  constexpr int NT = 64 * NW;
  constexpr int ES = (int)sizeof(T);
  constexpr int EPP = 16 / ES;
  constexpr int KC = ROWB / ES;
  constexpr int WM = BM / WGM, WN = BN / WGN;
  constexpr int TM = WM / 32, TN = WN / 32;
  constexpr int CPR = ROWB / 16;
  constexpr int RI = 64 / CPR;
  constexpr int IA = BM / RI, IB = BN / RI;
  constexpr int NI = (IA + IB + NW - 1) / NW;
  constexpr int KS = CPR / 2;
  constexpr int BUF = (BM + BN) * ROWB;
  constexpr int LDO = BN + 4;
  constexpr bool HL = HALO != HALO_NONE;
  constexpr int PWD = 32, PHT = BM / 32;
  constexpr int HK = HALO == HALO_33 ? 3 : 2;
  constexpr int HNT = HK * HK;
  constexpr int HWD = PWD + HK - 1, HHT = PHT + HK - 1, HROWS = HHT * HWD;
  constexpr int NJH = ((HROWS + RI - 1) / RI + NW - 1) / NW;
  constexpr int HALOB = ((HROWS + RI - 1) / RI) * 1024;
  constexpr int HSCRATCH = 2 * HALOB;
  constexpr int HBOFF = 2 * HALOB + 1024;
  constexpr int DRING = 4;
  constexpr int BSLOT = BN * ROWB;
  constexpr int NBW = IB / NW;
  constexpr int PIPE = HL ? HBOFF + DRING * BSLOT : NBUF * BUF;
  constexpr int STAGE = WGM * 32 * LDO * 4;
  constexpr int MAINB = PIPE > STAGE ? PIPE : STAGE;
  constexpr int TABN = HL ? BM : (2 * kMaxK + 1) * BM;
  static_assert(TM >= 1 && TN >= 1, "wave tile must hold one 32x32 MFMA tile");
  static_assert((IA % NW) == 0 && IB >= 1 && (BM % RI) == 0 && (BN % RI) == 0, "DMA instruction split");
  static_assert(!HL || (sizeof(T) == 2 && NW == 8 && (IB % NW) == 0 && WM % 32 == 0 && HNT >= 4 && KS % 2 == 0 && (HALO == HALO_PHASE) == PHASE),
                "halo forms: bf16, 8 waves, whole weight DMA instructions per wave");
  static_assert(MAINB + TABN * 4 <= 160 * 1024, "LDS");

  __shared__ __attribute__((aligned(16))) unsigned char smem[MAINB + TABN * 4];
  int* taby = reinterpret_cast<int*>(smem + MAINB);
  int* tabx = taby + kMaxK * BM;
  int* orow = HL ? taby : tabx + kMaxK * BM;

  const int tid = threadIdx.x;
  const int lane = tid & 63;
  const int wave = __builtin_amdgcn_readfirstlane(tid >> 6);
  const int wm = wave / WGN, wn = wave % WGN;

  int bid = rs_xcd_remap(blockIdx.x, gridDim.x);
  int py = 0, px = 0;
  if (PHASE) {
    py = (bid >> 1) & 1;
    px = bid & 1;
    bid >>= 2;
  }
  const int mt = bid / p.ntiles, nt = bid - mt * p.ntiles;
  const int m0 = mt * BM, n0 = nt * BN;

  const int Hd = PHASE ? p.Hs : p.Ho, Wd = PHASE ? p.Ws : p.Wo;
  const int HdWd = Hd * Wd;
  int hn = 0, hy0 = 0, hx0 = 0;
  if constexpr (HL) {
    hn = __builtin_amdgcn_readfirstlane(mt / p.tpi);
    const int rem = mt - hn * p.tpi;
    const int ty = __builtin_amdgcn_readfirstlane(rem / p.tpx);
    hy0 = ty * PHT;
    hx0 = (rem - ty * p.tpx) * PWD;
  }
  const int nfirst = HL ? hn : __builtin_amdgcn_readfirstlane(m0 / HdWd);
  const int ush = p.ups ? 1 : 0;
  const int upar = p.ups == 2 ? 1 : 0;
  const int pad_y = PHASE ? 1 - py : p.pad, pad_x = PHASE ? 1 - px : p.pad;

  if constexpr (HL) {
    for (int e = tid; e < BM; e += NT) {
      const int y = hy0 + e / PWD, x = hx0 + e % PWD;
      int v = -1;
      if (y < Hd && x < Wd) v = PHASE ? (hn * p.Ho + 2 * y + py) * p.Wo + 2 * x + px : (hn * Hd + y) * Wd + x;
      orow[e] = v;
    }
  }
  for (int e = tid; e < (HL ? 0 : (p.kh + p.kw + 1) * BM); e += NT) {
    const int t = e / BM, row = e - t * BM;
    const int m = m0 + row;
    int v = -1;
    if (m < p.M) {
      const int n = m / HdWd;
      const int rem = m - n * HdWd;
      const int oy = rem / Wd;
      const int ox = rem - oy * Wd;
      if (t < p.kh) {
        const int iy = oy * p.stride - pad_y + t;
        if (((unsigned)iy < (unsigned)p.Hv) && ((iy & upar) == 0)) v = ((n - nfirst) * p.Hs + (iy >> ush)) * p.Ws;
      } else if (t < p.kh + p.kw) {
        const int ix = ox * p.stride - pad_x + (t - p.kh);
        if (((unsigned)ix < (unsigned)p.Wv) && ((ix & upar) == 0)) v = ix >> ush;
      } else {
        v = PHASE ? (n * p.Ho + 2 * oy + py) * p.Wo + 2 * ox + px : m;
      }
    }
    if (t < p.kh) taby[t * BM + row] = v;
    else if (t < p.kh + p.kw) tabx[(t - p.kh) * BM + row] = v;
    else orow[row] = v;
  }

  const long img1 = (long)p.Hs * p.Ws * p.C1;
  const long img2 = (long)p.Hs * p.Ws * p.C2;
  const __amdgpu_buffer_rsrc_t rsrc1 = rs_dma_rsrc<kDmaClamp>(p.src1 + nfirst * img1, (long)(p.N - nfirst) * img1 * ES);
  const __amdgpu_buffer_rsrc_t rsrc2 = rs_dma_rsrc<kDmaClamp>(p.C2 ? p.src2 + nfirst * img2 : p.src1, (long)(p.N - nfirst) * img2 * ES);
  const __amdgpu_buffer_rsrc_t rsrcw =
      rs_dma_rsrc<kDmaClamp>(p.wgt + (long)(2 * py + px) * p.Cout * p.Kw, (long)p.Cout * p.Kw * ES);

  const int ra = lane / CPR, pp = lane % CPR;
  const int fsw = ROWB == 128 ? ((4 * (wave & 1) + (ra >> 1)) & 7) : ((ra >> 2) & 3);
  const int gp = pp ^ fsw;
  const unsigned int lds0 = __builtin_amdgcn_readfirstlane(rs_lds_addr(smem));
  constexpr int NIA = IA / NW;
  int wrow[NI];
#pragma unroll
  for (int j = 0; j < NI; ++j) wrow[j] = ((n0 + RI * (wave + NW * j - IA) + ra) * p.Kw + gp * EPP) * ES;
  __syncthreads();

  int pbase[NIA];
  auto load_tap = [&](int (&dst)[NIA], int r, int s_, bool first) __attribute__((always_inline)) {
    const int cs2 = (first ? p.C1 : p.C2) * ES;
#pragma unroll
    for (int j = 0; j < NIA; ++j) {
      const int row = RI * (wave + NW * j) + ra;
      const int y = taby[r * BM + row], x = tabx[s_ * BM + row];
      dst[j] = (y | x) < 0 ? kDmaOOB : (y + x) * cs2 + gp * 16;
    }
  };
  int lr = 0, ls = 0, lc = 0, lk = 0;
  unsigned int fL = lds0;
  __amdgpu_buffer_rsrc_t frs = rsrc1;
  int fsa = 0, fsb = 0;
  auto begin_chunk = [&](int buf) __attribute__((always_inline)) {
    const int c0 = lc * KC;
    const bool first = c0 < p.C1;
    if (lc == 0 || c0 == p.C1) load_tap(pbase, lr, ls, first);
    fL = lds0 + buf * BUF;
    frs = first ? rsrc1 : rsrc2;
    fsa = (first ? c0 : c0 - p.C1) * ES;
    fsb = lk * ROWB;
    ++lk;
    ++lc;
    const int w1 = (lc == p.cpt) ? 1 : 0;
    lc = w1 ? 0 : lc;
    ls += w1;
    const int w2 = (ls == p.kw) ? 1 : 0;
    ls = w2 ? 0 : ls;
    lr += w2;
  };
  auto issue_piece = [&](int j) __attribute__((always_inline)) {
    const int ii = wave + NW * j;
    if (j < NIA) {
      rs_dma16(frs, fL + ii * 1024, pbase[j], fsa);
    } else if ((IB % NW) == 0 || ii < IA + IB) {
      rs_dma16(rsrcw, fL + ii * 1024, wrow[j], fsb);
    }
  };

  f32x16 acc[TN][TM];
#pragma unroll
  for (int a = 0; a < TN; ++a)
#pragma unroll
    for (int b = 0; b < TM; ++b)
#pragma unroll
      for (int r = 0; r < 16; ++r) acc[a][b][r] = 0.f;

  const int frow = lane & 31;
  const int fl = ROWB == 128 ? ((frow >> 1) & 7) : ((frow >> 2) & 3);
  int foff[KS];
#pragma unroll
  for (int s = 0; s < KS; ++s) foff[s] = ((2 * s + (lane >> 5)) ^ fl) * 16;
  const int abase = (wm * WM + frow) * ROWB;
  const int bbase = (BM + wn * WN + frow) * ROWB;

  auto read_frag = [&](const unsigned char* L, int s, u32x4 (&a)[TM], u32x4 (&b)[TN]) __attribute__((always_inline)) {
#pragma unroll
    for (int tm = 0; tm < TM; ++tm) a[tm] = *reinterpret_cast<const u32x4*>(L + abase + 32 * tm * ROWB + foff[s]);
#pragma unroll
    for (int tn = 0; tn < TN; ++tn) b[tn] = *reinterpret_cast<const u32x4*>(L + bbase + 32 * tn * ROWB + foff[s]);
  };
  if constexpr (!HL) {
  if (p.nk > 0) {
    begin_chunk(0);
#pragma unroll
    for (int q = 0; q < NI; ++q) issue_piece(q);
  }
  }
  constexpr int NMMA = KS * TM * TN;
  constexpr int PSTEP = NMMA / (2 * NI) >= 1 ? NMMA / (2 * NI) : 1;
  constexpr int PIN = (NMMA + PSTEP - 1) / PSTEP < NI ? (NMMA + PSTEP - 1) / PSTEP : NI;
  auto chunk = [&](int kc, auto fetch_tag) __attribute__((always_inline)) {
    constexpr bool FETCH = decltype(fetch_tag)::value;
    rs_dma_wait();
    __syncthreads();
    if (FETCH) begin_chunk((kc + 1) % NBUF);
    const unsigned char* L = smem + (kc % NBUF) * BUF;
    u32x4 fa[2][TM], fb[2][TN];
    read_frag(L, 0, fa[0], fb[0]);
#pragma unroll
    for (int s = 0; s < KS; ++s) {
      if (s + 1 < KS) read_frag(L, s + 1, fa[(s + 1) & 1], fb[(s + 1) & 1]);
#pragma unroll
      for (int tm = 0; tm < TM; ++tm)
#pragma unroll
        for (int tn = 0; tn < TN; ++tn) {
          const int q = (s * TM + tm) * TN + tn;
          if (FETCH && q % PSTEP == 0 && q / PSTEP < PIN) issue_piece(q / PSTEP);
          mma16(acc[tn][tm], fb[s & 1][tn], fa[s & 1][tm], T());
        }
    }
    if (FETCH) {
#pragma unroll
      for (int q = PIN; q < NI; ++q) issue_piece(q);
    }
  };
  if constexpr (!HL) {
    int kc = 0;
    for (; kc < p.nk - 1; ++kc) chunk(kc, std::true_type());
    for (; kc < p.nk; ++kc) chunk(kc, std::false_type());
  } else {
    constexpr int RPT = WM / 32;
    constexpr int NHI = (HROWS + RI - 1) / RI;
    const int hi = lane >> 5, l31 = lane & 31;
    const int ctot = p.C1 + p.C2;
    int ho1[NJH], ho2[NJH];
    auto halo_pix = [&](int pa, int pb) __attribute__((always_inline)) {
      int hpix[NJH];
#pragma unroll
      for (int j = 0; j < NJH; ++j) {
        const int R = RI * (wave + NW * j) + ra;
        const int hyy = R / HWD, hxx = R - hyy * HWD;
        int v = -1;
        if (HALO == HALO_DG4) {
          const int su = hy0 - pa + hyy, sv = hx0 - pb + hxx;
          if (R < HROWS && (unsigned)su < (unsigned)p.Ho && (unsigned)sv < (unsigned)p.Wo) v = (2 * su + pa) * p.Ws + 2 * sv + pb;
        } else {
          const int sy = hy0 - pad_y + hyy, sx = hx0 - pad_x + hxx;
          if (R < HROWS && (unsigned)sy < (unsigned)p.Hs && (unsigned)sx < (unsigned)p.Ws) v = sy * p.Ws + sx;
        }
        hpix[j] = v;
      }
#pragma unroll
      for (int j = 0; j < NJH; ++j) {
        ho1[j] = hpix[j] >= 0 ? hpix[j] * (p.C1 * ES) + gp * 16 : kDmaOOB;
        ho2[j] = hpix[j] >= 0 ? hpix[j] * (p.C2 * ES) + gp * 16 : kDmaOOB;
      }
    };
    int hwrow[NBW];
#pragma unroll
    for (int j = 0; j < NBW; ++j) hwrow[j] = ((n0 + RI * (wave + NW * j) + ra) * p.Kw + gp * EPP) * ES;
    struct Grp {
      int c0;
      int pa, pb;
      int live;
    };
    const int Q = p.nk;
    auto group = [&](int q) __attribute__((always_inline)) {
      Grp g;
      g.live = q < Q ? 1 : 0;
      const int qq = g.live ? q : 0;
      const int pl = HALO == HALO_DG4 ? qq / p.cpt : 0;
      g.c0 = (qq - pl * p.cpt) * KC;
      g.pa = pl >> 1;
      g.pb = pl & 1;
      return g;
    };
    auto issue_halo = [&](int j, int buf, const Grp& g) __attribute__((always_inline)) {
      const int first = g.c0 < p.C1 ? 1 : 0;
      const int v = g.live ? (first ? ho1[j] : ho2[j]) : kDmaOOB;
      const int ii = wave + NW * j;
      rs_dma16(first ? rsrc1 : rsrc2, lds0 + (ii < NHI ? buf * HALOB + ii * 1024 : HSCRATCH), v, (first ? g.c0 : g.c0 - p.C1) * ES);
    };
    auto issue_w = [&](int j, int slot, const Grp& g, int tap) __attribute__((always_inline)) {
      const int tau = HALO == HALO_DG4 ? (2 * (tap >> 1) + 1 - g.pa) * 4 + 2 * (tap & 1) + 1 - g.pb : tap;
      rs_dma16(rsrcw, lds0 + HBOFF + slot * BSLOT + (wave + NW * j) * 1024, g.live ? hwrow[j] : kDmaOOB, (tau * ctot + g.c0) * ES);
    };
    int rb0[TM];
#pragma unroll
    for (int tm = 0; tm < TM; ++tm) rb0[tm] = (wm * RPT + tm) * HWD + l31;
    constexpr bool PRE = HNT * TM <= 18;
    int ab[PRE ? HNT : 1][PRE ? TM : 1];
    if constexpr (PRE) {
      rb_for_each(
          [&](auto tc) __attribute__((always_inline)) {
            constexpr int t = decltype(tc)::value;
            constexpr int toff = (t / HK) * HWD + (t % HK);
#pragma unroll
            for (int tm = 0; tm < TM; ++tm) {
              const int R = rb0[tm] + toff;
              const int key = ROWB == 128 ? ((R >> 1) & 7) << 4 : ((R >> 2) & 3) << 4;
              ab[t][tm] = R * ROWB + ((hi << 4) ^ key);
              asm volatile("" : "+v"(ab[t][tm]));
            }
          },
          std::make_integer_sequence<int, HNT>());
    }
    const int bfl = ROWB == 128 ? ((l31 >> 1) & 7) : ((l31 >> 2) & 3);
    int bfo[KS];
#pragma unroll
    for (int s = 0; s < KS; ++s) bfo[s] = HBOFF + (wn * WN + l31) * ROWB + (((2 * s + hi) ^ bfl) * 16);
    auto rd = [&](int hbuf, int slot, int toff, int ks, u32x4 (&a)[TM], u32x4 (&b)[TN], int t = 0) __attribute__((always_inline)) {
#pragma unroll
      for (int tm = 0; tm < TM; ++tm) {
        if constexpr (PRE) {
          a[tm] = *reinterpret_cast<const u32x4*>(smem + ((ab[t][tm] ^ (ks << 5)) + hbuf * HALOB));
        } else {
          const int R = rb0[tm] + toff;
          const int key = ROWB == 128 ? ((R >> 1) & 7) << 4 : ((R >> 2) & 3) << 4;
          a[tm] = *reinterpret_cast<const u32x4*>(smem + hbuf * HALOB + R * ROWB + (((2 * ks + hi) << 4) ^ key));
        }
      }
#pragma unroll
      for (int tn = 0; tn < TN; ++tn) b[tn] = *reinterpret_cast<const u32x4*>(smem + slot * BSLOT + 32 * tn * ROWB + bfo[ks]);
    };

    Grp cur = group(0), nxt = group(1);
    halo_pix(cur.pa, cur.pb);
#pragma unroll
    for (int j = 0; j < NJH; ++j) issue_halo(j, 0, cur);
#pragma unroll
    for (int d = 0; d < 3; ++d)
#pragma unroll
      for (int j = 0; j < NBW; ++j) issue_w(j, d, cur, d);
    if (HALO == HALO_DG4) halo_pix(nxt.pa, nxt.pb);
    constexpr int NMMA = KS * TM * TN;
    u32x4 fa[2][TM], fb[2][TN];
    rs_dma_wait_n<NBW>();
    __syncthreads();
    __builtin_amdgcn_sched_barrier(0);
    rd(0, 0, 0, 0, fa[0], fb[0], 0);
    for (int q = 0; q < Q; ++q) {
      const int hbuf = q & 1, nbuf = (q + 1) & 1;
      if constexpr (!PRE) {
#pragma unroll
        for (int tm = 0; tm < TM; ++tm) asm volatile("" : "+v"(rb0[tm]));
      }
      rb_for_each(
          [&](auto tc) __attribute__((always_inline)) {
            constexpr int t = decltype(tc)::value;
            constexpr int tprev = (t + HNT - 1) % HNT;
            __builtin_amdgcn_sched_barrier(0);
            if constexpr (KO != 1) {
              rs_dma_wait_n<NBW + halo_pieces_at_tap(tprev, HNT, NJH)>();
#ifdef RS_HALO_FENCED_BARRIER
              __syncthreads();
#else
              __builtin_amdgcn_s_barrier();
#endif
            }
            __builtin_amdgcn_sched_barrier(0);
            constexpr int NHT = halo_pieces_at_tap(t, HNT, NJH);
            constexpr int NP = NBW + NHT;
            constexpr int PST = NMMA / (2 * NP) >= 1 ? NMMA / (2 * NP) : 1;
            constexpr int t3 = (t + 3) % HNT;
            const int gstep = q * HNT + t;
            auto piece = [&](int i) __attribute__((always_inline)) {
              if constexpr (KO == 2) return;
              if (i < NBW) {
                issue_w(i, (gstep + 3) & (DRING - 1), (t + 3 < HNT) ? cur : nxt, t3);
              } else {
                int seen = 0;
#pragma unroll
                for (int j = 0; j < NJH; ++j) {
                  if (halo_tap_of_piece(j, HNT, NJH) == t) {
                    if (seen == i - NBW) issue_halo(j, nbuf, nxt);
                    ++seen;
                  }
                }
              }
            };
            constexpr int toff = (t / HK) * HWD + (t % HK);
            constexpr int tn1 = (t + 1) % HNT;
            constexpr int toff1 = (tn1 / HK) * HWD + (tn1 % HK);
            const int hbuf1 = (t + 1 < HNT) ? hbuf : nbuf;
            const int slot = gstep & (DRING - 1), slot1 = (gstep + 1) & (DRING - 1);
#pragma unroll
            for (int ks = 0; ks < KS; ++ks) {
              if constexpr (KO != 3) {
                if (ks + 1 < KS) rd(hbuf, slot, toff, ks + 1, fa[(ks + 1) & 1], fb[(ks + 1) & 1], t);
                else rd(hbuf1, slot1, toff1, 0, fa[0], fb[0], tn1);
              }
#pragma unroll
              for (int tm = 0; tm < TM; ++tm)
#pragma unroll
                for (int tn = 0; tn < TN; ++tn) {
                  const int i = (ks * TM + tm) * TN + tn;
                  if (i % PST == 0 && i / PST < NP) piece(i / PST);
                  if constexpr (KO == 4) {
                    asm volatile("" ::"v"(fb[ks & 1][tn]), "v"(fa[ks & 1][tm]));
                  } else if constexpr (KO == 3) {
                    mma16(acc[tn][tm], fb[0][tn], fa[0][tm], T());
                  } else {
                    mma16(acc[tn][tm], fb[ks & 1][tn], fa[ks & 1][tm], T());
                  }
                }
            }
#pragma unroll
            for (int i = (NMMA + PST - 1) / PST; i < NP; ++i) piece(i);
          },
          std::make_integer_sequence<int, HNT>());
      cur = nxt;
      nxt = group(q + 2);
      if (HALO == HALO_DG4) halo_pix(nxt.pa, nxt.pb);
    }
    rs_dma_wait();
    __builtin_amdgcn_sched_barrier(0);
  }
  __syncthreads();
  if constexpr (HL) __builtin_amdgcn_sched_barrier(0);

  float* lds = reinterpret_cast<float*>(smem);
  constexpr int TPR = BN / EPP;
  constexpr int RPI = NT / TPR;
  const int cc = tid % TPR, rr = tid / TPR;
  const int col = n0 + cc * EPP;
  const bool cvalid = col < p.Cout;
  constexpr int NSC = EPI == EPI_EVAL ? EPP : 1, NST = EPI == EPI_EVAL ? 1 : EPP, NBN = EPI == EPI_BWD ? EPP : 1;
  float sc[NSC], sh[NSC];
  if constexpr (EPI == EPI_EVAL) {
#pragma unroll
    for (int e = 0; e < EPP; ++e) {
      sc[e] = (p.scale && cvalid) ? p.scale[col + e] : 1.f;
      sh[e] = (p.shift && cvalid) ? p.shift[col + e] : 0.f;
    }
  }
  T* outp = p.out;
  const T* maskp = p.mask;
  int ostride = p.Cout, ocol = col;
  if (EPI == EPI_EVAL && p.out2) {
    if (n0 >= p.csplit) {
      outp = p.out2;
      maskp = p.mask2;
      ostride = p.Cout - p.csplit;
      ocol = col - p.csplit;
    } else {
      ostride = p.csplit;
    }
  }
  float st0[NST], st1[NST];
  float bmu[NBN], bis[NBN];
#pragma unroll
  for (int e = 0; e < NST; ++e) st0[e] = st1[e] = 0.f;
  if constexpr (EPI == EPI_BWD) {
#pragma unroll
    for (int e = 0; e < EPP; ++e) {
      bmu[e] = cvalid ? p.bn_mean[col + e] : 0.f;
      bis[e] = cvalid ? p.bn_invstd[col + e] : 0.f;
    }
  }
  constexpr int NIT = WN / (2 * EPP);
  constexpr int G = (ES == 4 && EPI == EPI_BWD) ? 1 : 2;
  static_assert(NIT * RPI == WGM * 32 && NIT % G == 0, "row groups tile the pass");
  const bool has_res = EPI != EPI_STATS && p.res != nullptr, has_mask = EPI != EPI_STATS && maskp != nullptr;
  const bool has_bits = EPI == EPI_BWD && p.mask_bits != nullptr;
  constexpr bool has_bny = EPI == EPI_BWD;
  auto load_group = [&](int tm, int g0, long (&o)[G], bool (&ok)[G], u32x4 (&rr_)[G], u32x4 (&rm_)[G], u32x4 (&ry_)[G])
      __attribute__((always_inline)) {
#pragma unroll
    for (int i = 0; i < G; ++i) {
      const int lrow = rr + (g0 + i) * RPI;
      const int row = (lrow >> 5) * WM + 32 * tm + (lrow & 31);
      const int opix = orow[row];
      ok[i] = opix >= 0 && cvalid;
      o[i] = ok[i] ? (long)opix * ostride + ocol : 0;
    }
    if (has_res) {
#pragma unroll
      for (int i = 0; i < G; ++i) rr_[i] = *reinterpret_cast<const u32x4*>(p.res + o[i]);
    }
    if (has_mask) {
#pragma unroll
      for (int i = 0; i < G; ++i) rm_[i] = *reinterpret_cast<const u32x4*>(maskp + o[i]);
    }
    if constexpr (EPI == EPI_BWD) {
      if (has_bits) {
#pragma unroll
        for (int i = 0; i < G; ++i) rm_[i][0] = p.mask_bits[o[i] >> 3];
      }
    }
    if constexpr (has_bny) {
#pragma unroll
      for (int i = 0; i < G; ++i) ry_[i] = *reinterpret_cast<const u32x4*>(p.bn_y + o[i]);
    }
  };
  auto unpack = [&](const u32x4 raw, float (&v)[EPP]) __attribute__((always_inline)) {
    if constexpr (ES == 4) {
      const f32x4 t = __builtin_bit_cast(f32x4, raw);
#pragma unroll
      for (int e = 0; e < 4; ++e) v[e] = t[e];
    } else {
      const bf16x8 t = __builtin_bit_cast(bf16x8, raw);
#pragma unroll
      for (int e = 0; e < 8; ++e) v[e] = (float)t[e];
    }
  };
  auto finish_group = [&](int g0, const long (&o)[G], const bool (&ok)[G], const u32x4 (&rr_)[G], const u32x4 (&rm_)[G],
                          const u32x4 (&ry_)[G]) __attribute__((always_inline)) {
#pragma unroll
    for (int i = 0; i < G; ++i) {
      const int lrow = rr + (g0 + i) * RPI;
      float v[EPP];
#pragma unroll
      for (int h = 0; h < EPP / 4; ++h) {
        const f32x4 t = *reinterpret_cast<const f32x4*>(&lds[lrow * LDO + cc * EPP + 4 * h]);
#pragma unroll
        for (int e = 0; e < 4; ++e) v[4 * h + e] = EPI == EPI_EVAL ? t[e] * sc[(4 * h + e) % NSC] + sh[(4 * h + e) % NSC] : t[e];
      }
      if (has_res) {
        float r[EPP];
        unpack(rr_[i], r);
#pragma unroll
        for (int e = 0; e < EPP; ++e) v[e] += r[e];
      }
      if (EPI == EPI_EVAL && p.relu) {
#pragma unroll
        for (int e = 0; e < EPP; ++e) v[e] = fmaxf(v[e], 0.f);
      }
      if (has_mask) {
        float z[EPP];
        unpack(rm_[i], z);
#pragma unroll
        for (int e = 0; e < EPP; ++e) v[e] = z[e] > 0.f ? v[e] : 0.f;
      }
      if constexpr (EPI == EPI_BWD) {
        if (has_bits) {
          const unsigned int bits = EPP == 8 ? rm_[i][0] : (rm_[i][0] >> (o[i] & 4));
#pragma unroll
          for (int e = 0; e < EPP; ++e) v[e] = ((bits >> e) & 1u) ? v[e] : 0.f;
        }
      }
      if (ok[i]) Piece<T>::store(outp + o[i], v);
      if constexpr (EPI != EPI_EVAL) {
        float w[EPP];
        Piece<T>::round(v, w);
        const float keep = ok[i] ? 1.f : 0.f;
        if constexpr (EPI == EPI_BWD) {
          float yv[EPP];
          unpack(ry_[i], yv);
#pragma unroll
          for (int e = 0; e < EPP; ++e) {
            st0[e % NST] += keep * w[e];
            st1[e % NST] += keep * (w[e] * ((yv[e] - bmu[e % NBN]) * bis[e % NBN]));
          }
        } else {
#pragma unroll
          for (int e = 0; e < EPP; ++e) {
            st0[e % NST] += keep * w[e];
            st1[e % NST] += keep * (w[e] * w[e]);
          }
        }
      }
    }
  };
#pragma unroll
  for (int tm = 0; tm < TM; ++tm) {
    long o[G];
    bool ok[G];
    u32x4 rr_[G], rm_[G], ry_[G];
    load_group(tm, 0, o, ok, rr_, rm_, ry_);
    if (tm > 0) __syncthreads();
    {
      const int pr = wm * 32 + (lane & 31);
      const int ccol = wn * WN + 4 * (lane >> 5);
#pragma unroll
      for (int tn = 0; tn < TN; ++tn)
#pragma unroll
        for (int g = 0; g < 4; ++g) {
          f32x4 v;
          v[0] = acc[tn][tm][4 * g + 0];
          v[1] = acc[tn][tm][4 * g + 1];
          v[2] = acc[tn][tm][4 * g + 2];
          v[3] = acc[tn][tm][4 * g + 3];
          *reinterpret_cast<f32x4*>(&lds[pr * LDO + ccol + 32 * tn + 8 * g]) = v;
        }
    }
    __syncthreads();
    finish_group(0, o, ok, rr_, rm_, ry_);
#pragma unroll
    for (int g0 = G; g0 < NIT; g0 += G) {
      load_group(tm, g0, o, ok, rr_, rm_, ry_);
      finish_group(g0, o, ok, rr_, rm_, ry_);
    }
  }
  if constexpr (EPI != EPI_EVAL) {
    __syncthreads();
    float* r0 = lds;
    float* r1 = lds + RPI * BN;
#pragma unroll
    for (int e = 0; e < EPP; ++e) {
      r0[rr * BN + cc * EPP + e] = st0[e % NST];
      r1[rr * BN + cc * EPP + e] = st1[e % NST];
    }
    __syncthreads();
    if (tid < 2 * BN) {
      const float* r = tid < BN ? r0 : r1;
      const int c = tid < BN ? tid : tid - BN;
      float a = 0.f;
#pragma unroll 4
      for (int l = 0; l < RPI; ++l) a += r[l * BN + c];
      if (n0 + c < p.Cout) p.stats[((long)mt * 2 + (tid < BN ? 0 : 1)) * p.Cout + n0 + c] = a;
    }
  }
}


template <typename T, int ROWB, bool PHASE, int EPI>
void launch_rows(int tile, int grid, hipStream_t s, const ConvArgsT<T>& a) {
  if constexpr (sizeof(T) == 2 && EPI == EPI_EVAL) {
    if (tile == T256x256) {
      conv_igemm_dma<T, 256, 256, 2, 4, ROWB, PHASE, EPI><<<grid, 512, 0, s>>>(a);
      return;
    }
  }
  switch (tile) {
    case T128x128: conv_igemm_dma<T, 128, 128, 2, 2, ROWB, PHASE, EPI><<<grid, 256, 0, s>>>(a); break;
    case T128x64: conv_igemm_dma<T, 128, 64, 2, 2, ROWB, PHASE, EPI><<<grid, 256, 0, s>>>(a); break;
    case T128x32: conv_igemm_dma<T, 128, 32, 4, 1, ROWB, PHASE, EPI><<<grid, 256, 0, s>>>(a); break;
    case T256x128: conv_igemm_dma<T, 256, 128, 4, 2, ROWB, PHASE, EPI><<<grid, 512, 0, s>>>(a); break;
    default: conv_igemm_dma<T, 64, 64, 2, 2, ROWB, PHASE, EPI><<<grid, 256, 0, s>>>(a); break;
  }
}

}

template <int HALO, bool PHASE, int EPI>
void launch_halo(int bn, int grid, hipStream_t s, const ConvArgsT<bf16_t>& a) {
  if (bn == (128 | 0x1000)) conv_igemm_dma<bf16_t, 512, 128, 4, 2, 64, PHASE, EPI, HALO><<<grid, 512, 0, s>>>(a);
  else if (bn == 128) conv_igemm_dma<bf16_t, 256, 128, 4, 2, 128, PHASE, EPI, HALO><<<grid, 512, 0, s>>>(a);
  else conv_igemm_dma<bf16_t, 256, 64, 4, 2, 128, PHASE, EPI, HALO><<<grid, 512, 0, s>>>(a);
}

#define RS_CONV_DEFINE_LAUNCHER(name, T, PHASE, EPI)                                            \
  void name(int tile, int rowb, int grid, hipStream_t s, const ConvArgsT<T>& a) {               \
    if (rowb == 128) launch_rows<T, 128, PHASE, EPI>(tile, grid, s, a);                         \
    else launch_rows<T, 64, PHASE, EPI>(tile, grid, s, a);                                      \
  }
#endif
```

### robosat_amd/csrc/knobs.hip

```cpp
#include <stdio.h>
#include <stdlib.h>
#include <string.h>

#include "common.h"

namespace {

struct Entry {
  const char* name;
  const char* env;
  int RsKnobs::*field;
  int lo, hi;
};

bool in_range(const Entry& e, int v) {
  if (v < e.lo || v > e.hi) return false;
  if (e.field == &RsKnobs::conv_rowb) return v == 0 || v == 64 || v == 128;
  return true;
}

const Entry kEntries[] = {
    {"conv_tile", "RS_CONV_TILE", &RsKnobs::conv_tile, -1, 9},
    {"conv_rowb", "RS_CONV_ROWB", &RsKnobs::conv_rowb, 0, 128},
    {"conv_big", "RS_CONV_BIG", &RsKnobs::conv_big, 0, 1},
    {"conv_min256", "RS_CONV_MIN256", &RsKnobs::conv_min256, 0, 1048576},
    {"conv_halo", "RS_CONV_HALO", &RsKnobs::conv_halo, 0, 1},
    {"conv_halo_min", "RS_CONV_HALO_MIN", &RsKnobs::conv_halo_min, 0, 1048576},
    {"conv_halo512", "RS_CONV_HALO512", &RsKnobs::conv_halo512, -1, 1},
    {"conv1x1_ew", "RS_CONV1X1_EW", &RsKnobs::conv1x1_ew, -1, 1},
    {"conv1x1_np", "RS_CONV1X1_NP", &RsKnobs::conv1x1_np, -1, 1},
    {"conv1x1_ew_bf16", "RS_CONV1X1_EW_BF16", &RsKnobs::conv1x1_ew_bf16, 0, 1},
    {"halo_ko", "RS_HALO_KO", &RsKnobs::halo_ko, 0, 4},
    {"wgrad_f32_phase", "RS_WGRAD_F32_PHASE", &RsKnobs::wgrad_f32_phase, 0, 1},
    {"wgrad_f32_dma", "RS_WGRAD_F32_DMA", &RsKnobs::wgrad_f32_dma, -1, 1},
    {"wgrad_f32_blocks", "RS_WGRAD_F32_BLOCKS", &RsKnobs::wgrad_f32_blocks, 1, 1048576},
    {"wgrad_f32_wino", "RS_WGRAD_F32_WINO", &RsKnobs::wgrad_f32_wino, 0, 1},
    {"wgrad_f32_wino_blocks", "RS_WGRAD_F32_WINO_BLOCKS", &RsKnobs::wgrad_f32_wino_blocks, 1, 1048576},
    {"wgrad_f32_wino33", "RS_WGRAD_F32_WINO33", &RsKnobs::wgrad_f32_wino33, 0, 1},
    {"wgrad_f32_wino33_blocks", "RS_WGRAD_F32_WINO33_BLOCKS", &RsKnobs::wgrad_f32_wino33_blocks, 1, 1048576},
    {"wgrad_blocks", "RS_WGRAD_BLOCKS", &RsKnobs::wgrad_blocks, 1, 1048576},
    {"wgrad_blocks_phase", "RS_WGRAD_BLOCKS_PHASE", &RsKnobs::wgrad_blocks_phase, 1, 1048576},
    {"wgrad_phase4", "RS_WGRAD_PHASE4", &RsKnobs::wgrad_phase4, 0, 1},
    {"wgrad_blocks_phase4", "RS_WGRAD_BLOCKS_PHASE4", &RsKnobs::wgrad_blocks_phase4, 1, 1048576},
    {"wgrad_ring", "RS_WGRAD_RING", &RsKnobs::wgrad_ring, 2, 7},
    {"lovasz_xcd", "RS_LOVASZ_XCD", &RsKnobs::lovasz_xcd, 0, 1},
    {"wino_wide", "ROBOSAT_WINO_WIDE", &RsKnobs::wino_wide, 0, 1},
};

}

RsKnobs& rs_knobs() {
  static RsKnobs k = [] {
    RsKnobs v;
    for (const Entry& e : kEntries)
      if (const char* s = getenv(e.env)) {
        const int x = atoi(s);
        if (in_range(e, x)) v.*(e.field) = x;
        else fprintf(stderr, "robosat_hip: %s=%s is outside [%d, %d]: ignored, the rule stays\n", e.env, s, e.lo, e.hi);
      }
    return v;
  }();
  return k;
}

extern "C" int rs_set_knob(const char* name, int value) {
  if (!name) return RS_EINVAL;
  for (const Entry& e : kEntries)
    if (strcmp(name, e.name) == 0) {
      if (!in_range(e, value)) return RS_EINVAL;
      rs_knobs().*(e.field) = value;
      return 0;
    }
  return RS_EINVAL;
}

extern "C" int rs_get_knob(const char* name, int* value) {
  if (!name || !value) return RS_EINVAL;
  for (const Entry& e : kEntries)
    if (strcmp(name, e.name) == 0) {
      *value = rs_knobs().*(e.field);
      return 0;
    }
  return RS_EINVAL;
}
```

### robosat_amd/ops.py

```python

import ctypes
import os

import torch

from . import _lib
from ._lib import RS_BF16, RS_F32, ConvDesc, check

BF16 = torch.bfloat16


def _dt(t):

    dtype = getattr(t, "dtype", t)
    if dtype == torch.float32:
        return RS_F32
    if dtype == torch.bfloat16:
        return RS_BF16
    raise TypeError("robosat_amd: activations are fp32 or bf16, got {}".format(dtype))


def _esize(t):

    return 2 if getattr(t, "dtype", t) == BF16 else 4


def _dev(t, name, dtype=torch.float32):
    if t is None:
        return None
    if not t.is_cuda:
        raise RuntimeError("robosat_amd: `{}` is on {} -- the hot path only runs on the MI355X (no CPU fallback)".format(name, t.device))
    if t.dtype != dtype:
        raise TypeError("robosat_amd: `{}` must be {}, got {}".format(name, dtype, t.dtype))
    if not t.is_contiguous():
        raise ValueError("robosat_amd: `{}` must be contiguous".format(name))
    return ctypes.c_void_p(t.data_ptr())


def _stream():
    return ctypes.c_void_p(torch.cuda.current_stream().cuda_stream)


def _call(name, *args):

    rc = getattr(_lib.lib(), name)(*args)
    if rc:
        check(rc, name)


SWITCHES = {
    "ROBOSAT_WINOGRAD": "fp32 Winograd forward forms (DecoderBlock, stride-1 3x3); off: the generic phase / implicit-GEMM kernels",
    "ROBOSAT_WINO_DGRAD": "Winograd data gradient of the fp32 DecoderBlock; off: the 4x4 / stride-2 kernel",
    "ROBOSAT_WINO33_STATS": "train-mode fp32 conv3x3 -> BatchNorm front half in the Winograd form; off: conv2d_bnstats",
    "ROBOSAT_WINO33_BWD": "Winograd data gradient of the fp32 stride-1 3x3 convolutions; off: the generic kernel",
    "ROBOSAT_FUSED_HEAD": "dec5 + self.final in one launch; off: two launches",
    "ROBOSAT_TAIL_FUSE": "layer1's fused Bottleneck tail and its wave 1x1 kernel; off: the generic 1x1 convolutions",
    "ROBOSAT_S2_DGRAD": "stride-2 data gradients in compact form (3x3: phase form, 1x1: scatter-add); off: zero-insertion convolutions",
    "ROBOSAT_S2_DGRAD_3X3": "the 3x3 half of ROBOSAT_S2_DGRAD alone",
    "ROBOSAT_WGRAD_STREAM": "weight gradients on a side stream; off: serial backward (clean per-kernel timings)",
}


def switch(name):

    if name not in SWITCHES:
        raise KeyError("robosat_amd: unknown switch {!r}: one of {}".format(name, ", ".join(SWITCHES)))
    return os.environ.get(name, "1") != "0"


PROFILE = None


def _start():

    if PROFILE is None:
        return None
    ev = torch.cuda.Event(enable_timing=True), torch.cuda.Event(enable_timing=True)
    ev[0].record()
    return ev


def _stop(ev):
    ev[1].record()


def _record(ev, name, flops, shape, nbytes, executed=None):

    PROFILE.append((name, flops, shape, ev[0], ev[1], nbytes, flops if executed is None else executed))


def _shape(d):

    return (d.C1 + d.C2, d.Cout, d.kh, d.stride, d.ups, d.Ho, d.Wo)


def _partial(rows_fn, d, device, *args):

    rows = getattr(_lib.lib(), rows_fn)(ctypes.byref(d), *args)
    if rows <= 0:
        raise ValueError("{}: invalid arguments".format(rows_fn))
    return torch.empty((rows, 2, d.Cout), device=device, dtype=torch.float32)


def conv_flops(d):

    cin = 3 if d.stem else d.C1 + d.C2
    return 2.0 * d.N * d.Cout * cin * d.kh * d.kw * d.Ho * d.Wo


def conv_bytes(d, esize, epilogue_tensors=0):

    cin = 4 if d.stem else d.C1 + d.C2
    return esize * (d.N * d.Hs * d.Ws * cin + d.Cout * d.kh * d.kw * cin + (1 + epilogue_tensors) * d.N * d.Ho * d.Wo * d.Cout)


def conv_desc(src1, weight, src2=None, ups=0, stride=1, pad=0, relu=False, stem=0, out_hw=None, bands=4):
    n, hs, ws, c1 = src1.shape
    cout, kh, kw_, _ = weight.shape
    c2 = 0 if src2 is None else src2.shape[3]
    kw = int(stem) if stem else kw_
    if out_hw is None:
        assert ups in (0, 1)
        hv, wv = (hs * 2, ws * 2) if ups == 1 else (hs, ws)
        out_hw = ((hv + 2 * pad - kh) // stride + 1, (wv + 2 * pad - kw) // stride + 1)
    return ConvDesc(n, hs, ws, c1, c2, ups, kh, kw, stride, pad, out_hw[0], out_hw[1], cout, int(relu),
                    (3 if bands <= 3 else 1) if stem else 0)


def conv2d(src1, weight, src2=None, ups=0, stride=1, pad=0, scale=None, shift=None, residual=None, relu=False,
           stem=0, out_hw=None, out=None, relu_mask=None, alg_scale=1.0, bands=4):

    d = conv_desc(src1, weight, src2, ups, stride, pad, relu, stem, out_hw, bands)
    act = src1.dtype
    bf = act == BF16
    if bf and stem:
        raise ValueError("the 7x7 stem runs on the fp32 kernel (cast happens at the stem max-pool)")
    if out is None:
        out = torch.empty((d.N, d.Ho, d.Wo, d.Cout), device=src1.device, dtype=act)
    if src2 is not None:
        assert src2.shape[:3] == src1.shape[:3]
    if not stem:
        assert weight.shape[3] == d.C1 + d.C2, "weight Cin {} != {}+{}".format(weight.shape[3], d.C1, d.C2)
    if residual is not None:
        assert residual.shape == out.shape
    if relu_mask is not None:
        assert relu_mask.shape == out.shape
    ev = _start()
    _call("rs_conv2d_fwd_bf16" if bf else "rs_conv2d_fwd", ctypes.byref(d), _dev(src1, "src1", act), _dev(src2, "src2", act),
          _dev(weight, "weight", act), _dev(scale, "scale"), _dev(shift, "shift"), _dev(residual, "residual", act),
          _dev(relu_mask, "relu_mask", act), _dev(out, "out", act), _stream())
    if ev:
        _stop(ev)
        name = conv_tile_name(d, bf, plain=relu_mask is None)
        if alg_scale != 1.0 and not name.startswith(("conv_thin", "conv_halo")):
            name = name.replace("<", "<dgrad4x4,")
        _record(ev, name, conv_flops(d) * alg_scale, _shape(d),
                conv_bytes(d, _esize(act), (residual is not None) + (relu_mask is not None)), conv_flops(d))
    return out


def conv2d_bnstats(src1, weight, src2=None, ups=0, stride=1, pad=0):

    d = conv_desc(src1, weight, src2, ups, stride, pad, False, 0, None)
    act = src1.dtype
    out = torch.empty((d.N, d.Ho, d.Wo, d.Cout), device=src1.device, dtype=act)
    partial = _partial("rs_conv2d_bnstats_rows_dt", d, src1.device, _dt(src1))
    assert weight.shape[3] == d.C1 + d.C2
    ev = _start()
    _call("rs_conv2d_fwd_bnstats_dt", ctypes.byref(d), _dt(src1), _dev(src1, "src1", act), _dev(src2, "src2", act),
          _dev(weight, "weight", act), _dev(out, "out", act), _dev(partial, "partial"), _stream())
    if ev:
        _stop(ev)
        _record(ev, conv_tile_name(d, act == BF16, plain=False), conv_flops(d), _shape(d), conv_bytes(d, _esize(act)))
    return out, partial


def conv2d_dgrad_bnstats(dy, wd, out_hw, bn_y, bn_mean, bn_invstd, ups=0, pad=0, residual=None, relu_mask=None,
                         relu_mask_bits=None, stride=1):

    d = conv_desc(dy, wd, None, ups, stride, pad, False, 0, out_hw)
    act = dy.dtype
    out = torch.empty((d.N, d.Ho, d.Wo, d.Cout), device=dy.device, dtype=act)
    assert bn_y.shape == out.shape
    partial = _partial("rs_conv2d_bnstats_rows_dt", d, dy.device, _dt(dy))
    ev = _start()
    if relu_mask_bits is not None:
        assert relu_mask_bits.numel() * 8 == out.numel(), "one mask bit per output element"
        _call("rs_conv2d_dgrad_bnstats_bits_dt", ctypes.byref(d), _dt(dy), _dev(dy, "dy", act), _dev(wd, "weight", act),
              _dev(residual, "residual", act), _dev(relu_mask_bits, "relu_mask_bits", torch.uint8), _dev(bn_y, "bn_y", act),
              _dev(bn_mean, "bn_mean"), _dev(bn_invstd, "bn_invstd"), _dev(out, "out", act), _dev(partial, "partial"), _stream())
    else:
        _call("rs_conv2d_dgrad_bnstats_dt", ctypes.byref(d), _dt(dy), _dev(dy, "dy", act), _dev(wd, "weight", act),
              _dev(residual, "residual", act), _dev(relu_mask, "relu_mask", act), _dev(bn_y, "bn_y", act), _dev(bn_mean, "bn_mean"),
              _dev(bn_invstd, "bn_invstd"), _dev(out, "out", act), _dev(partial, "partial"), _stream())
    if ev:
        _stop(ev)
        _record(ev, conv_tile_name(d, act == BF16, plain=False), conv_flops(d), _shape(d),
                conv_bytes(d, _esize(act), 1 + (residual is not None) + (relu_mask is not None))
                + (out.numel() // 8 if relu_mask_bits is not None else 0))
    return out, partial


def bn_bwd_from_partials(g, y, mean, invstd, gamma, partial, dgamma=None, dbeta=None):

    c = y.shape[-1]
    m = y.numel() // c
    dy = torch.empty_like(y)
    if dgamma is None:
        dgamma = torch.empty(c, device=y.device, dtype=torch.float32)
    if dbeta is None:
        dbeta = torch.empty(c, device=y.device, dtype=torch.float32)
    t = y.dtype
    _call("rs_bn_bwd_from_partials_dt", _dev(g, "g", t), _dev(y, "y", t), _dev(mean, "mean"), _dev(invstd, "invstd"), _dev(gamma, "gamma"),
          _dev(dy, "dy", t), _dev(dgamma, "dgamma"), _dev(dbeta, "dbeta"), _dev(partial, "partial"), partial.shape[0], _dt(y), m, c,
          _workspace(64 * 2 * c * 8 + 3 * c * 4, y.device), _stream())
    return dy, dgamma, dbeta


def bn_finalize_stats(partial, m, gamma, beta, eps, momentum, running_mean=None, running_var=None, num_batches_tracked=None):

    rows, _, c = partial.shape
    mean, invstd, scale, shift = (torch.empty(c, device=partial.device, dtype=torch.float32) for _ in range(4))
    _call("rs_bn_finalize_stats", _dev(partial, "partial"), rows, m, c, ctypes.c_float(eps), ctypes.c_float(momentum), _dev(gamma, "gamma"),
          _dev(beta, "beta"), _dev(mean, "mean"), _dev(invstd, "invstd"), _dev(scale, "scale"), _dev(shift, "shift"),
          _dev(running_mean, "running_mean"), _dev(running_var, "running_var"),
          _dev(num_batches_tracked, "num_batches_tracked", torch.int64), _workspace(64 * 2 * c * 8, partial.device), _stream())
    return mean, invstd, scale, shift


def pack_phase_weight(w_krsc, dtype=torch.float32):

    cout, kh, kw, cin = w_krsc.shape
    assert kh == 3 and kw == 3
    out = torch.empty((4, cout, 2, 2, cin), device=w_krsc.device, dtype=dtype)
    _call("rs_pack_phase_weight_dt", _dev(w_krsc, "w"), _dev(out, "out", dtype), _dt(dtype), cout, cin, _stream())
    return out


def pack_s2_dgrad_phase_weight(w_krsc, dtype=torch.float32):

    cout, kh, kw, cin = w_krsc.shape
    assert kh == 3 and kw == 3
    out = torch.empty((4, cin, 2, 2, cout), device=w_krsc.device, dtype=dtype)
    _call("rs_pack_s2_dgrad_phase_weight_dt", _dev(w_krsc, "w"), _dev(out, "out", dtype), _dt(dtype), cout, cin, _stream())
    return out


def pack_dgrad_phase_weight(w_krsc, dtype=torch.float32):

    cout, kh, kw, cin = w_krsc.shape
    assert kh == 3 and kw == 3
    out = torch.empty((cin, 4, 4, cout), device=w_krsc.device, dtype=dtype)
    wt = pack_dgrad_weight(w_krsc, torch.float32)
    _call("rs_combine_dgrad_phase_weight_dt", _dev(wt, "wt"), _dev(out, "out", dtype), _dt(dtype), cout, cin, _stream())
    return out


def conv2d_split(src, weight, c1, stride=1, pad=0, out_hw=None, mask1=None, mask2=None, alg_scale=1.0):

    d = conv_desc(src, weight, None, 0, stride, pad, False, 0, out_hw)
    act = src.dtype
    c2 = d.Cout - c1
    out1 = torch.empty((d.N, d.Ho, d.Wo, c1), device=src.device, dtype=act)
    out2 = torch.empty((d.N, d.Ho, d.Wo, c2), device=src.device, dtype=act)
    ev = _start()
    _call("rs_conv2d_fwd_split_dt", ctypes.byref(d), _dt(src), _dev(src, "src", act), _dev(weight, "weight", act), _dev(out1, "out1", act),
          _dev(mask1, "mask1", act), _dev(out2, "out2", act), _dev(mask2, "mask2", act), c1, _stream())
    if ev:
        _stop(ev)
        name = conv_tile_name(d, act == BF16, plain=False)
        if alg_scale != 1.0 and not name.startswith("conv_halo"):
            name = name.replace("<", "<dgrad4x4,")
        _record(ev, name, conv_flops(d) * alg_scale, _shape(d),
                conv_bytes(d, _esize(act), ((mask1 is not None) * c1 + (mask2 is not None) * (d.Cout - c1)) / d.Cout), conv_flops(d))
    return out1, out2


def cat_split_bwd(dcat, c1, c2=0, mask1=None, mask2=None, out1=None):

    n, h, w, ct = dcat.shape
    assert ct == c1 + c2
    t = dcat.dtype
    acc = out1 is not None
    d1 = out1 if acc else torch.empty((n, h, w, c1), device=dcat.device, dtype=t)
    d2 = torch.empty((n, h, w, c2), device=dcat.device, dtype=t) if c2 else None
    _call("rs_cat_split_bwd_dt", _dev(dcat, "dcat", t), _dev(d1, "d1", t), _dev(d2, "d2", t), _dev(mask1, "mask1", t),
          _dev(mask2, "mask2", t), _dt(dcat), n, h, w, c1, c2, int(acc), _stream())
    return d1, d2


def _phase_desc(n, hs, ws, c1, c2, cout, relu=False):

    return ConvDesc(n, hs, ws, c1, c2, 1, 3, 3, 1, 1, 2 * hs, 2 * ws, cout, int(relu), 0)


def _conv33_desc(src, cout, relu):
    n, h, w, c = src.shape
    return ConvDesc(n, h, w, c, 0, 0, 3, 3, 1, 1, h, w, cout, int(relu), 0)


def conv2d_phase(src1, weight_phase, src2=None, scale=None, shift=None, residual=None, relu=False, relu_mask=None):

    n, hs, ws, c1 = src1.shape
    c2 = 0 if src2 is None else src2.shape[3]
    cout = weight_phase.shape[1]
    assert tuple(weight_phase.shape) == (4, cout, 2, 2, c1 + c2)
    if src2 is not None and tuple(src2.shape[:3]) != (n, hs, ws):
        raise RuntimeError("Sizes of tensors must match except in dimension 1: skip {} vs decoder {}".format(
            tuple(src1.shape[:3]), tuple(src2.shape[:3])))
    act = src1.dtype
    d = _phase_desc(n, hs, ws, c1, c2, cout, relu)
    out = torch.empty((n, 2 * hs, 2 * ws, cout), device=src1.device, dtype=act)
    ev = _start()
    _call("rs_conv2d_fwd_phase_dt", ctypes.byref(d), _dt(src1), _dev(src1, "src1", act), _dev(src2, "src2", act),
          _dev(weight_phase, "weight", act), _dev(scale, "scale"), _dev(shift, "shift"), _dev(residual, "residual", act),
          _dev(relu_mask, "relu_mask", act), _dev(out, "out", act), _stream())
    if ev:
        _stop(ev)
        _record(ev, conv_tile_name(d, act == BF16, phase=True), conv_flops(d), _shape(d),
                conv_bytes(d, _esize(act), (residual is not None) + (relu_mask is not None)), conv_flops(d) * 4.0 / 9.0)
    return out


def wino_ok(src1, src2, cout, force=False):

    if src1.dtype != torch.float32 or not (force or switch("ROBOSAT_WINOGRAD")):
        return False
    d = _phase_desc(*src1.shape, 0 if src2 is None else src2.shape[3], cout)
    rc = _lib.lib().rs_conv2d_phase_wino_ok(ctypes.byref(d))
    return rc != 0 if force else rc == 1


def pack_wino_phase_weight(weight_phase):

    _, cout, _, _, cin = weight_phase.shape
    u = torch.empty((4, 9, cout, cin), device=weight_phase.device, dtype=torch.float32)
    _call("rs_pack_wino_phase_weight", _dev(weight_phase, "w_phase"), _dev(u, "u"), cout, cin, _stream())
    return u


def conv2d_phase_wino(src1, u, src2=None, relu=False):

    n, hs, ws, c1 = src1.shape
    c2 = 0 if src2 is None else src2.shape[3]
    cout = u.shape[2]
    assert tuple(u.shape) == (4, 9, cout, c1 + c2)
    if src2 is not None and tuple(src2.shape[:3]) != (n, hs, ws):
        raise RuntimeError("Sizes of tensors must match except in dimension 1: skip {} vs decoder {}".format(
            tuple(src1.shape[:3]), tuple(src2.shape[:3])))
    d = _phase_desc(n, hs, ws, c1, c2, cout, relu)
    out = torch.empty((n, 2 * hs, 2 * ws, cout), device=src1.device, dtype=torch.float32)
    ev = _start()
    _call("rs_conv2d_fwd_phase_wino", ctypes.byref(d), _dev(src1, "src1"), _dev(src2, "src2"), _dev(u, "u"), _dev(out, "out"), _stream())
    if ev:
        _stop(ev)
        name = _lib.lib().rs_conv2d_phase_wino_name(ctypes.byref(d)).decode()
        _record(ev, name, conv_flops(d), _shape(d), conv_bytes(d, 4), conv_flops(d) * 0.25)
    return out


def wino_dgrad_ok(n, hs, ws, c1, c2, cout):

    if not switch("ROBOSAT_WINO_DGRAD"):
        return False
    return _lib.lib().rs_conv2d_dgrad_phase_wino_ok(ctypes.byref(_phase_desc(n, hs, ws, c1, c2, cout))) == 1


def pack_wino_dgrad_weight(wd4x4):

    cin, kh, kw, cout = wd4x4.shape
    assert kh == 4 and kw == 4 and wd4x4.dtype == torch.float32
    u = torch.empty((4, 9, cin, cout), device=wd4x4.device, dtype=torch.float32)
    _call("rs_pack_wino_dgrad_weight", _dev(wd4x4, "wd"), _dev(u, "u"), cin, cout, _stream())
    return u


def conv2d_dgrad_phase_wino(dz, u, c1, c2=0, mask1=None, mask2=None, split=False):

    n, ho, wo, cout = dz.shape
    hs, ws = ho // 2, wo // 2
    assert tuple(u.shape) == (4, 9, c1 + c2, cout) and dz.dtype == torch.float32 and (ho, wo) == (2 * hs, 2 * ws)
    d = _phase_desc(n, hs, ws, c1, c2, cout)
    if split:
        out1 = torch.empty((n, hs, ws, c1), device=dz.device, dtype=torch.float32)
        out2 = torch.empty((n, hs, ws, c2), device=dz.device, dtype=torch.float32)
    else:
        out1, out2 = torch.empty((n, hs, ws, c1 + c2), device=dz.device, dtype=torch.float32), None
        assert mask2 is None
    for m, o in ((mask1, out1), (mask2, out2)):
        assert m is None or tuple(m.shape) == tuple(o.shape)
    ev = _start()
    _call("rs_conv2d_dgrad_phase_wino", ctypes.byref(d), _dev(dz, "dz"), _dev(u, "u"), _dev(out1, "out"), _dev(mask1, "mask"),
          _dev(out2, "out2"), _dev(mask2, "mask2"), c1 if split else 0, _stream())
    if ev:
        _stop(ev)
        alg = 2.0 * n * ho * wo * cout * (c1 + c2) * 9
        ex4 = 2.0 * n * hs * ws * cout * (c1 + c2) * 16
        nbytes = 4 * (n * ho * wo * cout + 16 * cout * (c1 + c2) + n * hs * ws * (c1 + c2) * (1 + (mask1 is not None) * (c1 if split else c1 + c2) / (c1 + c2)
                                                                                            + (mask2 is not None) * c2 / (c1 + c2)))
        _record(ev, _lib.lib().rs_conv2d_dgrad_phase_wino_name(ctypes.byref(d)).decode(), alg, (cout, c1 + c2, 4, 2, 0, hs, ws), nbytes,
                ex4 * 9.0 / 16.0)
    return out1, out2


def wino33_ok(src, cout):

    if src.dtype != torch.float32 or not switch("ROBOSAT_WINOGRAD"):
        return False
    return _lib.lib().rs_conv2d_wino33_ok(ctypes.byref(_conv33_desc(src, cout, False))) == 1


def pack_wino33_weight(w_krsc):

    cout, kh, kw, cin = w_krsc.shape
    assert kh == 3 and kw == 3
    u = torch.empty((16, cout, cin), device=w_krsc.device, dtype=torch.float32)
    _call("rs_pack_wino33_weight", _dev(w_krsc, "w"), _dev(u, "u"), cout, cin, _stream())
    return u


def conv2d_wino33(src, u, scale=None, shift=None, relu=False):

    n, h, w, c = src.shape
    cout = u.shape[1]
    assert tuple(u.shape) == (16, cout, c)
    d = _conv33_desc(src, cout, relu)
    out = torch.empty((n, h, w, cout), device=src.device, dtype=torch.float32)
    ev = _start()
    _call("rs_conv2d_fwd_wino33", ctypes.byref(d), _dev(src, "src"), _dev(u, "u"), _dev(scale, "scale"), _dev(shift, "shift"),
          _dev(out, "out"), _stream())
    if ev:
        _stop(ev)
        name = _lib.lib().rs_conv2d_wino33_name(ctypes.byref(d)).decode()
        _record(ev, name, conv_flops(d), _shape(d), conv_bytes(d, 4), conv_flops(d) * 4.0 / 9.0)
    return out


def conv2d_wino33_bnstats(src, u):

    n, h, w, c = src.shape
    cout = u.shape[1]
    assert tuple(u.shape) == (16, cout, c) and src.dtype == torch.float32
    d = _conv33_desc(src, cout, False)
    out = torch.empty((n, h, w, cout), device=src.device, dtype=torch.float32)
    partial = _partial("rs_conv2d_wino33_stats_rows", d, src.device)
    ev = _start()
    _call("rs_conv2d_fwd_wino33_stats", ctypes.byref(d), _dev(src, "src"), _dev(u, "u"), _dev(out, "out"), _dev(partial, "partial"),
          _stream())
    if ev:
        _stop(ev)
        _record(ev, _lib.lib().rs_conv2d_wino33_name(ctypes.byref(d)).decode().replace("<3x3,", "<3x3+stats,"), conv_flops(d), _shape(d),
                conv_bytes(d, 4), conv_flops(d) * 4.0 / 9.0)
    return out, partial


def wino33_dgrad_ok(dy, cout):

    if not switch("ROBOSAT_WINO33_BWD") or cout % 32:
        return False
    return wino33_ok(dy, cout)


def conv2d_wino33_dgrad(dy, u, relu_mask=None, relu_mask_bits=None, bn=None):

    n, h, w, c = dy.shape
    cout = u.shape[1]
    assert tuple(u.shape) == (16, cout, c) and dy.dtype == torch.float32
    d = _conv33_desc(dy, cout, False)
    out = torch.empty((n, h, w, cout), device=dy.device, dtype=torch.float32)
    partial = None
    y = mean = invstd = None
    if bn is not None:
        y, mean, invstd = bn
        assert y.shape == out.shape
        partial = _partial("rs_conv2d_wino33_stats_rows", d, dy.device)
    if relu_mask is not None:
        assert relu_mask.shape == out.shape
    if relu_mask_bits is not None:
        assert relu_mask_bits.numel() * 8 == out.numel(), "one mask bit per output element"
    ev = _start()
    _call("rs_conv2d_dgrad_wino33", ctypes.byref(d), _dev(dy, "dy"), _dev(u, "u"), _dev(relu_mask, "relu_mask"),
          _dev(relu_mask_bits, "relu_mask_bits", torch.uint8), _dev(y, "bn_y"), _dev(mean, "bn_mean"), _dev(invstd, "bn_invstd"),
          _dev(out, "out"), _dev(partial, "partial"), _stream())
    if ev:
        _stop(ev)
        _record(ev, _lib.lib().rs_conv2d_wino33_name(ctypes.byref(d)).decode().replace("<3x3,", "<3x3+bwd,"), conv_flops(d), _shape(d),
                conv_bytes(d, 4, 1 + (relu_mask is not None) + (bn is not None)) + (out.numel() // 8 if relu_mask_bits is not None else 0),
                conv_flops(d) * 4.0 / 9.0)
    return out, partial


def wino33_head_ok(src, cout, classes):

    if not wino33_ok(src, cout) or not switch("ROBOSAT_FUSED_HEAD"):
        return False
    return _lib.lib().rs_conv2d_wino33_head_ok(ctypes.byref(_conv33_desc(src, cout, True)), int(classes)) == 1


def conv2d_wino33_head(src, u, final_w, final_b, mode="logits", overlap=0, relu=True):

    n, h, w, c = src.shape
    cout, classes = u.shape[1], final_w.shape[0]
    assert tuple(u.shape) == (16, cout, c) and tuple(final_w.shape) == (classes, cout)
    d = _conv33_desc(src, cout, relu)
    m = {"logits": 0, "softmax": 1, "quantize": 2, "argmax": 3}[mode]
    out = qout = anchors = None
    if m <= 1:
        out = torch.empty((n, classes, h, w), device=src.device, dtype=torch.float32)
    elif m == 2:
        shape = (n, h - 2 * overlap, w - 2 * overlap) + ((classes - 1,) if classes > 2 else ())
        qout = torch.empty(shape, device=src.device, dtype=torch.uint8)
        anchors = _anchors(src.device)
    else:
        qout = torch.empty((n, h, w), device=src.device, dtype=torch.uint8)
    ev = _start()
    _call("rs_conv2d_fwd_wino33_head", ctypes.byref(d), _dev(src, "src"), _dev(u, "u"), None, None, _dev(final_w, "final_w"),
          _dev(final_b, "final_b"), classes, m, _dev(anchors, "anchors", torch.float64), int(overlap), _dev(out, "out"),
          _dev(qout, "qout", torch.uint8), _stream())
    if ev:
        _stop(ev)
        fl = conv_flops(d) + 2.0 * n * h * w * cout * classes
        nbytes = 4 * (n * h * w * c + 9 * cout * c + classes * cout) + (4 * classes if m <= 1 else 1) * n * h * w
        _record(ev, _lib.lib().rs_conv2d_wino33_head_name().decode(), fl, _shape(d), nbytes,
                conv_flops(d) * 4.0 / 9.0 + 2.0 * n * h * w * cout * classes)
    return out if m <= 1 else qout


def bottleneck_tail_ok(x, w3, w1):

    m = x.numel() // x.shape[-1]
    return (x.dtype == torch.float32 and x.shape[-1] == 64 and tuple(w3.shape) == (256, 1, 1, 64) and tuple(w1.shape) == (64, 1, 1, 256)
            and m % 32 == 0 and switch("ROBOSAT_TAIL_FUSE"))


def bottleneck_tail(x, w3, scale3, shift3, identity, w1, scale1, shift1):

    n, h, w, c1 = x.shape
    cm, c2 = w3.shape[0], w1.shape[0]
    assert identity.shape == (n, h, w, cm) and w1.shape[3] == cm
    out = torch.empty((n, h, w, cm), device=x.device, dtype=torch.float32)
    z = torch.empty((n, h, w, c2), device=x.device, dtype=torch.float32)
    ev = _start()
    _call("rs_bottleneck_tail_f32", _dev(x, "x"), _dev(w3, "w3"), _dev(scale3, "scale3"), _dev(shift3, "shift3"),
          _dev(identity, "identity"), _dev(w1, "w1"), _dev(scale1, "scale1"), _dev(shift1, "shift1"), _dev(out, "out"), _dev(z, "z"),
          n * h * w, c1, cm, c2, _stream())
    if ev:
        _stop(ev)
        m = n * h * w
        fl = 2.0 * m * cm * (c1 + c2)
        _record(ev, "bottleneck_tail_f32", fl, (c1, cm, 1, 1, 0, h, w), 4 * (m * (c1 + 2 * cm + c2) + cm * (c1 + c2)), fl)
    return out, z


def conv1x1_wave_ok(x, w):

    m = x.numel() // x.shape[-1]
    return (x.dtype == torch.float32 and x.shape[-1] == 64 and tuple(w.shape) == (256, 1, 1, 64) and m % 32 == 0
            and switch("ROBOSAT_TAIL_FUSE"))


def conv1x1_wave(x, w, scale, shift, residual=None, relu=False):

    n, h, wd, c1 = x.shape
    cout = w.shape[0]
    out = torch.empty((n, h, wd, cout), device=x.device, dtype=torch.float32)
    if residual is not None:
        assert residual.shape == out.shape
    ev = _start()
    _call("rs_conv1x1_wave_f32", _dev(x, "x"), _dev(w, "w"), _dev(scale, "scale"), _dev(shift, "shift"), _dev(residual, "residual"),
          int(relu), _dev(out, "out"), n * h * wd, c1, cout, _stream())
    if ev:
        _stop(ev)
        m = n * h * wd
        fl = 2.0 * m * cout * c1
        _record(ev, "conv1x1_wave_f32", fl, (c1, cout, 1, 1, 0, h, wd), 4 * (m * (c1 + cout * (2 if residual is not None else 1)) + cout * c1), fl)
    return out


def conv_tile_name(d, bf16=False, phase=False, plain=True):

    lib = _lib.lib()
    if d.stem:
        return lib.rs_conv2d_tile_name(lib.rs_conv2d_tile(ctypes.byref(d))).decode()
    tile, rowb = ctypes.c_int(0), ctypes.c_int(0)
    form = int(bool(phase)) | (0 if plain else 2)
    _call("rs_conv2d_config", ctypes.byref(d), 2 if bf16 else 4, form, ctypes.byref(tile), ctypes.byref(rowb))
    base = (lib.rs_conv2d_tile_name_bf16 if bf16 else lib.rs_conv2d_tile_name)(tile.value).decode()
    if tile.value == TILES["thin"]:
        return "{}<{}>".format(base, "phase" if phase else ("dgrad4x4" if d.kh == 4 else "3x3"))
    if tile.value == TILES["halo"]:
        return "{}<{},{}x{}>".format(base, "phase" if phase else ("dgrad4x4" if d.kh == 4 else "3x3"),
                                     512 if rowb.value & 0x1000 else 256, rowb.value & 0xFFF)
    return base.replace("<", "<phase," if phase else "<").replace(">", ",r{}>".format(rowb.value))


TILES = {"128x128": 0, "128x64": 1, "128x32": 2, "64x64": 3, "256x128": 5, "256x256": 6, "thin": 7, "halo": 8}


class tuning:

    def __init__(self, tile=None, rowb=0):
        self.tile = -1 if tile is None else (TILES[tile] if isinstance(tile, str) else int(tile))
        self.rowb = int(rowb)

    def __enter__(self):
        _call("rs_conv2d_set_tuning", self.tile, self.rowb)
        return self

    def __exit__(self, *exc):
        _call("rs_conv2d_set_tuning", -1, 0)
        return False


def get_knob(name):

    v = ctypes.c_int(0)
    check(_lib.lib().rs_get_knob(name.encode(), ctypes.byref(v)), "rs_get_knob({})".format(name))
    return v.value


def set_knob(name, value):

    check(_lib.lib().rs_set_knob(name.encode(), int(value)), "rs_set_knob({})".format(name))


class knob:

    def __init__(self, name, value):
        self.name, self.value, self.old = name, int(value), None

    def __enter__(self):
        self.old = get_knob(self.name)
        set_knob(self.name, self.value)
        return self

    def __exit__(self, *exc):
        set_knob(self.name, self.old)
        return False


def cast_bf16(t):

    out = torch.empty(t.shape, device=t.device, dtype=BF16)
    _call("rs_cast_f32_to_bf16", _dev(t, "src"), _dev(out, "dst", BF16), t.numel(), _stream())
    return out


def cast_bf16_scaled(t, scale):

    out = torch.empty(t.shape, device=t.device, dtype=BF16)
    _call("rs_cast_f32_to_bf16_scaled", _dev(t, "src"), _dev(out, "dst", BF16), t.numel(), ctypes.c_float(scale), _stream())
    return out


def cast_f32_scaled(src_bf16, dst_f32, scale):

    assert src_bf16.numel() == dst_f32.numel()
    _call("rs_cast_bf16_to_f32_scaled", _dev(src_bf16, "src", BF16), _dev(dst_f32, "dst"), src_bf16.numel(), ctypes.c_float(scale),
          _stream())
    return dst_f32


class _WPrepItem(ctypes.Structure):
    _fields_ = [("w", ctypes.c_void_p), ("cast", ctypes.c_void_p), ("dgrad", ctypes.c_void_p), ("Cout", ctypes.c_int),
                ("taps", ctypes.c_int), ("Cin", ctypes.c_int), ("tile_begin", ctypes.c_int)]


class WeightPrep:

    def __init__(self, weights_krsc, want_dgrad=True, dtype=BF16):

        assert weights_krsc and all(w.dtype == torch.float32 and w.is_contiguous() and w.dim() == 4 for w in weights_krsc)
        assert dtype == BF16 or want_dgrad
        dev = weights_krsc[0].device
        self.dtype = dtype
        self.weights = list(weights_krsc)
        self.cast = [torch.empty(w.shape, device=dev, dtype=BF16) if dtype == BF16 else None for w in self.weights]
        self.dgrad = [torch.empty((w.shape[3], w.shape[1], w.shape[2], w.shape[0]), device=dev, dtype=dtype) if want_dgrad else None
                      for w in self.weights]
        items = (_WPrepItem * len(self.weights))()
        tiles = 0
        for i, w in enumerate(self.weights):
            cout, kh, kw, cin = w.shape
            items[i] = _WPrepItem(_dev(w, "w").value, _dev(self.cast[i], "cast", BF16).value if dtype == BF16 else None,
                                  _dev(self.dgrad[i], "dgrad", dtype).value if want_dgrad else None, cout, kh * kw, cin, tiles)
            tiles += kh * kw * ((cin + 31) // 32) * ((cout + 31) // 32)
        self.tiles = tiles
        self.table = torch.frombuffer(bytearray(bytes(items)), dtype=torch.uint8).to(dev)
        self.ptrs = tuple(w.data_ptr() for w in self.weights)

    def run(self):
        _call("rs_weight_prep_bf16" if self.dtype == BF16 else "rs_weight_prep_f32", _dev(self.table, "items", torch.uint8),
              len(self.weights), self.tiles, _stream())


def pack_stem_weight(w_krsc, dtype=torch.float32):

    cout, kh, kw, cin = w_krsc.shape
    out = torch.empty((cout, kh, 8, 4), device=w_krsc.device, dtype=dtype)
    _call("rs_pack_stem_weight_bf16" if dtype == BF16 else "rs_pack_stem_weight", _dev(w_krsc, "w"), _dev(out, "out", dtype), cout, kh, kw,
          cin, _stream())
    return out


def nchw_to_nhwc4(x, dtype=torch.float32):
    n, c, h, w = x.shape
    out = torch.empty((n, h, w, 4), device=x.device, dtype=dtype)
    _call("rs_nchw_to_nhwc4_bf16" if dtype == BF16 else "rs_nchw_to_nhwc4", _dev(x, "x"), _dev(out, "out", dtype), n, c, h, w, _stream())
    return out


def stem_conv_bf16(x4, w_packed, scale=None, shift=None, relu=False):

    n, h, w, _ = x4.shape
    out = torch.empty((n, h // 2, w // 2, 64), device=x4.device, dtype=BF16)
    ev = _start()
    _call("rs_stem_conv_fwd_bf16", _dev(x4, "x4", BF16), _dev(w_packed, "w", BF16), _dev(scale, "scale"), _dev(shift, "shift"),
          _dev(out, "out", BF16), n, h, w, int(relu), _stream())
    if ev:
        _stop(ev)
        flops = 2.0 * n * 64 * 3 * 49 * (h // 2) * (w // 2)
        _record(ev, "stem_conv_bf16", flops, (3, 64, 7, 2, 0, h // 2, w // 2), 2 * (x4.numel() + out.numel()))
    return out


def wgrad_kernel_name(d, form=None):

    lib = _lib.lib()
    if form is None:
        form = lib.rs_conv2d_wgrad_bf16_form(ctypes.byref(d))
    if form == 1:
        return "conv_wgrad_thin_bf16<{}{}>".format(min(d.C1, 128), ",ups" if d.ups else "")
    t = lib.rs_conv2d_wgrad_bf16_tile(ctypes.byref(d))
    if t <= 0:
        raise ValueError("rs_conv2d_wgrad_bf16_tile: invalid arguments")
    tile = "{}x{}".format(t >> 16, t & 255) + ("+{}x{}".format(t >> 16, (t >> 8) & 255) if (t >> 8) & 255 else "")
    phase = "" if form != 2 else ("phase4," if (t >> 16, t & 255) == (128, 128) and get_knob("wgrad_phase4") else "phase,")
    return "conv_wgrad_bf16<{}{}>".format(phase, tile)


def stem_conv_wgrad_bf16(dy, x4):

    n, h, w, _ = x4.shape
    lib = _lib.lib()
    dw = torch.empty((64, 7, 8, 4), device=dy.device, dtype=torch.float32)
    ev = _start()
    _call("rs_stem_conv_wgrad_bf16", _dev(dy, "dy", BF16), _dev(x4, "x4", BF16), _dev(dw, "dw"), n, h, w,
          _workspace(lib.rs_stem_conv_wgrad_bf16_workspace_bytes(n, h, w), dy.device), _stream())
    if ev:
        _stop(ev)
        flops = 2.0 * n * 64 * 3 * 49 * (h // 2) * (w // 2)
        _record(ev, "stem_wgrad_bf16", flops, (3, 64, 7, 2, 0, h // 2, w // 2), 2 * (x4.numel() + dy.numel()))
    return dw


def u8_to_nhwc4_norm(img, mean, std):

    n, h, w, c = img.shape
    assert len(mean) == c and len(std) == c
    out = torch.empty((n, h, w, 4), device=img.device, dtype=torch.float32)
    fm, fs = (ctypes.c_float * c)(*mean), (ctypes.c_float * c)(*std)
    _call("rs_u8_to_nhwc4_norm", _dev(img, "img", torch.uint8), _dev(out, "out"), fm, fs, n, h, w, c, _stream())
    return out


_ANCHORS = {}


def _anchors(device):
    import numpy as np

    anchors = _ANCHORS.get(device)
    if anchors is None:
        anchors = torch.from_numpy(np.linspace(0, 1, 256)).to(device)
        _ANCHORS[device] = anchors
    return anchors


def final_conv1x1_quantize(x, w, bias, overlap):

    n, h, wd, cin = x.shape
    c = w.shape[0]
    shape = (n, h - 2 * overlap, wd - 2 * overlap) + ((c - 1,) if c > 2 else ())
    out = torch.empty(shape, device=x.device, dtype=torch.uint8)
    _call("rs_final_conv1x1_quantize_dt", _dev(x, "x", x.dtype), _dt(x), _dev(w, "w"), _dev(bias, "bias"),
          _dev(_anchors(x.device), "anchors", torch.float64), _dev(out, "out", torch.uint8), n, h, wd, cin, c, overlap, _stream())
    return out


def final_conv1x1_argmax(x, w, bias):

    n, h, wd, cin = x.shape
    out = torch.empty((n, h, wd), device=x.device, dtype=torch.uint8)
    _call("rs_final_conv1x1_argmax_dt", _dev(x, "x", x.dtype), _dt(x), _dev(w, "w"), _dev(bias, "bias"), _dev(out, "out", torch.uint8), n,
          h, wd, cin, w.shape[0], _stream())
    return out


TTA_MODES = {"none": (0,), "hflip": (0, 1), "flips": (0, 1, 4, 5), "d4": (0, 1, 2, 3, 4, 5, 6, 7)}


def tta_ops(mode, h, w):

    if mode not in TTA_MODES:
        raise ValueError("unknown TTA mode {!r}: one of {}".format(mode, ", ".join(TTA_MODES)))
    op_list = list(TTA_MODES[mode])
    if h != w and any((op >> 1) & 1 for op in op_list):
        raise ValueError("TTA mode {!r} rotates by 90 degrees and needs square tiles, got {}x{}".format(mode, h, w))
    return op_list


def _tta_fan_out(x, kind, mean, std, op_list, dtype, n, h, w, c):
    v = len(op_list)
    out = torch.empty((n * v, h, w, 4), device=x.device, dtype=dtype)
    fm = fs = None
    if mean is not None:
        assert len(mean) == c and len(std) == c
        fm, fs = (ctypes.c_float * c)(*mean), (ctypes.c_float * c)(*std)
    _call("rs_tta_fan_out", _dev(x, "x", x.dtype), kind, fm, fs, _dev(out, "out", dtype), _dt(dtype), (ctypes.c_int * v)(*op_list), v, n, h,
          w, c, _stream())
    return out


def tta_fan_out_u8(img, mean, std, op_list, dtype=torch.float32):

    n, h, w, c = img.shape
    return _tta_fan_out(img, _lib.RS_TTA_IN_U8, mean, std, op_list, dtype, n, h, w, c)


def tta_fan_out_f32(x, op_list, dtype=torch.float32):

    n, c, h, w = x.shape
    return _tta_fan_out(x, _lib.RS_TTA_IN_F32, None, None, op_list, dtype, n, h, w, c)


def tta_merge(probs, op_list, mode="probs", overlap=0):

    nv, c, h, w = probs.shape
    v = len(op_list)
    assert nv % v == 0
    n = nv // v
    m = {"probs": _lib.RS_TTA_PROBS, "quantize": _lib.RS_TTA_QUANTIZE, "argmax": _lib.RS_TTA_ARGMAX}[mode]
    anchors = None
    if m == _lib.RS_TTA_PROBS:
        out = torch.empty((n, c, h, w), device=probs.device, dtype=torch.float32)
    elif m == _lib.RS_TTA_QUANTIZE:
        out = torch.empty((n, h - 2 * overlap, w - 2 * overlap) + ((c - 1,) if c > 2 else ()), device=probs.device, dtype=torch.uint8)
        anchors = _dev(_anchors(probs.device), "anchors", torch.float64)
    else:
        out = torch.empty((n, h, w), device=probs.device, dtype=torch.uint8)
    _call("rs_tta_merge", _dev(probs, "probs"), (ctypes.c_int * v)(*op_list), v, m, anchors, int(overlap), _dev(out, "out", out.dtype), n,
          c, h, w, _stream())
    return out


def maxpool2d(x, k, stride, pad, want_argmax=False, out_dtype=None):

    n, h, w, c = x.shape
    ho, wo = (h + 2 * pad - k) // stride + 1, (w + 2 * pad - k) // stride + 1
    out = torch.empty((n, ho, wo, c), device=x.device, dtype=out_dtype or x.dtype)
    amax = torch.empty((n, ho, wo, c), device=x.device, dtype=torch.uint8) if want_argmax else None
    _call("rs_maxpool2d_fwd_dt", _dev(x, "x", x.dtype), _dt(x), _dev(out, "out", out.dtype), _dt(out), _dev(amax, "argmax", torch.uint8), n,
          h, w, c, k, stride, pad, ho, wo, _stream())
    return (out, amax) if want_argmax else out


def bn_fold(gamma, beta, mean, var, eps):
    c = gamma.numel()
    scale = torch.empty(c, device=gamma.device, dtype=torch.float32)
    shift = torch.empty(c, device=gamma.device, dtype=torch.float32)
    _call("rs_bn_fold", _dev(gamma, "gamma"), _dev(beta, "beta"), _dev(mean, "mean"), _dev(var, "var"), ctypes.c_float(eps),
          _dev(scale, "scale"), _dev(shift, "shift"), c, _stream())
    return scale, shift


def final_conv1x1(x, w, bias, softmax=False):

    n, h, wd, cin = x.shape
    c = w.shape[0]
    out = torch.empty((n, c, h, wd), device=x.device, dtype=torch.float32)
    _call("rs_final_conv1x1_dt", _dev(x, "x", x.dtype), _dt(x), _dev(w, "w"), _dev(bias, "bias"), _dev(out, "out"), n, h, wd, cin, c,
          int(softmax), _stream())
    return out



_WORKSPACE = {}


def _workspace(nbytes, device):

    if nbytes < 0:
        raise ValueError("workspace query failed (RS_EINVAL)")
    key = (device, torch.cuda.current_stream().cuda_stream)
    ws = _WORKSPACE.get(key)
    if ws is None or ws.numel() < nbytes:
        ws = torch.empty(max(int(nbytes), 1 << 20), device=device, dtype=torch.uint8)
        _WORKSPACE[key] = ws
    return ctypes.c_void_p(ws.data_ptr())


def pack_dgrad_weight(w_krsc, dtype=torch.float32):

    cout, kh, kw, cin = w_krsc.shape
    out = torch.empty((cin, kh, kw, cout), device=w_krsc.device, dtype=dtype)
    _call("rs_pack_dgrad_weight_bf16" if dtype == BF16 else "rs_pack_dgrad_weight", _dev(w_krsc, "w"), _dev(out, "out", dtype), cout, kh,
          kw, cin, _stream())
    return out


def unpack_stem_weight(packed, kw, cin, out=None):
    cout, kh = packed.shape[:2]
    if out is None:
        out = torch.empty((cout, kh, kw, cin), device=packed.device, dtype=torch.float32)
    assert tuple(out.shape) == (cout, kh, kw, cin)
    _call("rs_unpack_stem_weight", _dev(packed, "packed"), _dev(out, "out"), cout, kh, kw, cin, _stream())
    return out


def conv2d_wgrad(dy, src1, kh, kw, src2=None, ups=0, stride=1, pad=0, stem=0, out=None):

    n, ho, wo, cout = dy.shape
    _, hs, ws, c1 = src1.shape
    c2 = 0 if src2 is None else src2.shape[3]
    d = ConvDesc(n, hs, ws, c1, c2, ups, kh, kw, stride, pad, ho, wo, cout, 0, int(bool(stem)))
    lib = _lib.lib()
    act = dy.dtype
    bf = act == BF16
    shape = (cout, kh, 8, 4) if stem else (cout, kh, kw, c1 + c2)
    dw = out if out is not None else torch.empty(shape, device=dy.device, dtype=torch.float32)
    assert tuple(dw.shape) == shape
    wsb = (lib.rs_conv2d_wgrad_bf16_workspace_bytes if bf else lib.rs_conv2d_wgrad_workspace_bytes)(ctypes.byref(d))
    ev = _start()
    _call("rs_conv2d_wgrad_bf16" if bf else "rs_conv2d_wgrad", ctypes.byref(d), _dev(dy, "dy", act), _dev(src1, "src1", act),
          _dev(src2, "src2", act), _dev(dw, "dw"), _workspace(wsb, dy.device), _stream())
    if ev:
        _stop(ev)
        nbytes = _esize(act) * (d.N * d.Ho * d.Wo * d.Cout + d.N * d.Hs * d.Ws * (4 if stem else d.C1 + d.C2)) + 4 * dw.numel()
        form = lib.rs_conv2d_wgrad_bf16_form(ctypes.byref(d)) if bf else 0
        if not bf and not stem:
            form = lib.rs_conv2d_wgrad_form(ctypes.byref(d))
        name = wgrad_kernel_name(d, form) if bf else ("conv_wgrad_f32" if stem or get_knob("wgrad_f32_dma") == 0 else
                                                      "conv_wgrad_wino_f32" if form == 3 else "conv_wgrad_wino33_f32" if form == 4 else
                                                      "conv_wgrad_f32_dma")
        _record(ev, name, conv_flops(d), _shape(d), nbytes, conv_flops(d) * (0.25 if form == 3 else 4.0 / 9.0 if form in (2, 4) else 1.0))
    return dw


def _bn_ws(m, c, device):
    return _workspace(_lib.lib().rs_bn_workspace_bytes(m, c) + 3 * c * 4, device)


def bn_train_stats(y, gamma, beta, eps, momentum, running_mean=None, running_var=None, num_batches_tracked=None):

    c = y.shape[-1]
    m = y.numel() // c
    mean, invstd, scale, shift = (torch.empty(c, device=y.device, dtype=torch.float32) for _ in range(4))
    _call("rs_bn_train_stats_dt", _dev(y, "y", y.dtype), _dt(y), m, c, ctypes.c_float(eps), ctypes.c_float(momentum), _dev(gamma, "gamma"),
          _dev(beta, "beta"), _dev(mean, "mean"), _dev(invstd, "invstd"), _dev(scale, "scale"), _dev(shift, "shift"),
          _dev(running_mean, "running_mean"), _dev(running_var, "running_var"),
          _dev(num_batches_tracked, "num_batches_tracked", torch.int64), _bn_ws(m, c, y.device), _stream())
    return mean, invstd, scale, shift


def bn_bits_ok(c):

    return 8 <= c <= 2048 and 2048 % c == 0


def bn_apply(y, scale, shift, residual=None, relu=False, want_bits=False):

    c = y.shape[-1]
    out = torch.empty_like(y)
    bits = torch.empty(y.numel() // 8, device=y.device, dtype=torch.uint8) if want_bits else None
    _call("rs_bn_apply_bits_dt", _dev(y, "y", y.dtype), _dev(scale, "scale"), _dev(shift, "shift"), _dev(residual, "residual", y.dtype),
          _dev(out, "out", y.dtype), _dev(bits, "bits", torch.uint8), _dt(y), y.numel() // c, c, int(relu), _stream())
    return (out, bits) if want_bits else out


def bn_bwd(dz, zmask, y, mean, invstd, gamma, want_masked=False, dgamma=None, dbeta=None):

    c = y.shape[-1]
    m = y.numel() // c
    dy = torch.empty_like(y)
    dmasked = torch.empty_like(y) if want_masked else None
    if dgamma is None:
        dgamma = torch.empty(c, device=y.device, dtype=torch.float32)
    if dbeta is None:
        dbeta = torch.empty(c, device=y.device, dtype=torch.float32)
    t = y.dtype
    _call("rs_bn_bwd_dt", _dev(dz, "dz", t), _dev(zmask, "zmask", t), _dev(y, "y", t), _dev(mean, "mean"), _dev(invstd, "invstd"),
          _dev(gamma, "gamma"), _dev(dy, "dy", t), _dev(dmasked, "dmasked", t), _dev(dgamma, "dgamma"), _dev(dbeta, "dbeta"), _dt(y), m, c,
          _bn_ws(m, c, y.device), _stream())
    return (dy, dgamma, dbeta, dmasked) if want_masked else (dy, dgamma, dbeta)


def scatter_add_stride2(t, out):

    n, hs, ws, c = t.shape
    assert out.shape[0] == n and out.shape[3] == c and out.dtype == t.dtype and out.is_contiguous()
    _call("rs_scatter_add_stride2_dt", _dev(t, "t", t.dtype), _dev(out, "out", t.dtype), _dt(t), n, hs, ws, out.shape[1], out.shape[2], c,
          _stream())
    return out


def maxpool2d_bwd(dy, argmax, in_shape, k, stride, pad, out=None, out_dtype=None):

    n, h, w, c = in_shape
    ho, wo = dy.shape[1:3]
    acc = out is not None
    if out is None:
        out = torch.empty(in_shape, device=dy.device, dtype=out_dtype or dy.dtype)
    _call("rs_maxpool2d_bwd_dt", _dev(dy, "dy", dy.dtype), _dt(dy), _dev(argmax, "argmax", torch.uint8), _dev(out, "dx", out.dtype),
          _dt(out), n, h, w, c, k, stride, pad, ho, wo, int(acc), _stream())
    return out


def upsample2x_bwd(dup, c1, c2=0, mask1=None, mask2=None, out1=None):

    n, h2, w2, ct = dup.shape
    assert ct == c1 + c2 and h2 % 2 == 0 and w2 % 2 == 0
    h, w = h2 // 2, w2 // 2
    acc = out1 is not None
    t = dup.dtype
    d1 = out1 if acc else torch.empty((n, h, w, c1), device=dup.device, dtype=t)
    d2 = torch.empty((n, h, w, c2), device=dup.device, dtype=t) if c2 else None
    _call("rs_upsample2x_bwd_dt", _dev(dup, "dup", t), _dev(d1, "d1", t), _dev(d2, "d2", t), _dev(mask1, "mask1", t),
          _dev(mask2, "mask2", t), _dt(dup), n, h, w, c1, c2, int(acc), _stream())
    return d1, d2


def final_conv1x1_bwd(x, w, dlogits, relu_mask=True, dw=None, db=None):

    n, h, wd, cin = x.shape
    c = w.shape[0]
    lib = _lib.lib()
    dx = torch.empty_like(x)
    if dw is None:
        dw = torch.empty((c, cin), device=x.device, dtype=torch.float32)
    if db is None:
        db = torch.empty(c, device=x.device, dtype=torch.float32)
    ws = _workspace(lib.rs_final_conv1x1_bwd_workspace_bytes(cin, c), x.device)
    _call("rs_final_conv1x1_bwd_dt", _dev(x, "x", x.dtype), _dev(w, "w"), _dev(dlogits, "dlogits"), _dev(dx, "dx", x.dtype), _dev(dw, "dw"),
          _dev(db, "db"), _dt(x), n, h, wd, cin, c, int(relu_mask), ws, _stream())
    return dx, dw, db



NLL_CROSS_ENTROPY, NLL_FOCAL = 0, 1


def nll_loss_fwd(logits, targets, weight, mode, gamma=2.0):
    n, c, h, w = logits.shape
    lib = _lib.lib()
    loss = torch.empty((), device=logits.device, dtype=torch.float32)
    stats = torch.empty(2, device=logits.device, dtype=torch.float32)
    _call("rs_nll_loss_fwd", _dev(logits, "logits"), _dev(targets, "targets", torch.int64), _dev(weight, "weight"), _dev(loss, "loss"),
          _dev(stats, "stats"), n, c, h, w, mode, ctypes.c_float(gamma), _workspace(lib.rs_nll_loss_workspace_bytes(), logits.device),
          _stream())
    return loss, stats


def nll_loss_bwd(logits, targets, weight, stats, grad_out, mode, gamma=2.0):
    n, c, h, w = logits.shape
    dlogits = torch.empty_like(logits)
    _call("rs_nll_loss_bwd", _dev(logits, "logits"), _dev(targets, "targets", torch.int64), _dev(weight, "weight"), _dev(stats, "stats"),
          _dev(grad_out, "grad_out"), _dev(dlogits, "dlogits"), n, c, h, w, mode, ctypes.c_float(gamma), _stream())
    return dlogits


def miou_loss_fwd(logits, targets, weight):
    n, c, h, w = logits.shape
    lib = _lib.lib()
    loss = torch.empty((), device=logits.device, dtype=torch.float32)
    stats = torch.empty(5 + 2 * n * c, device=logits.device, dtype=torch.float32)
    _call("rs_miou_loss_fwd", _dev(logits, "logits"), _dev(targets, "targets", torch.int64), _dev(weight, "weight"), _dev(loss, "loss"),
          _dev(stats, "stats"), n, c, h, w, _workspace(lib.rs_miou_loss_workspace_bytes(n, c), logits.device), _stream())
    return loss, stats


def miou_loss_bwd(logits, targets, weight, stats, grad_out):
    n, c, h, w = logits.shape
    dlogits = torch.empty_like(logits)
    _call("rs_miou_loss_bwd", _dev(logits, "logits"), _dev(targets, "targets", torch.int64), _dev(weight, "weight"), _dev(stats, "stats"),
          _dev(grad_out, "grad_out"), _dev(dlogits, "dlogits"), n, c, h, w, _stream())
    return dlogits


def lovasz_fwd(logits, targets, want_grad=True):

    n, c, h, w = logits.shape
    lib = _lib.lib()
    loss = torch.empty((), device=logits.device, dtype=torch.float32)
    grad = torch.empty_like(logits) if want_grad else None
    _call("rs_lovasz_fwd", _dev(logits, "logits"), _dev(targets, "targets", torch.int64), _dev(loss, "loss"), _dev(grad, "grad"), n, c, h,
          w, _workspace(lib.rs_lovasz_workspace_bytes(n, c, h, w), logits.device), _stream())
    return loss, grad


def lovasz_softmax_fwd(logits, targets, per_image=True, classes="present", want_grad=True, want_probs=False):

    if classes not in ("present", "all"):
        raise ValueError("classes must be \"present\" or \"all\" (got {!r})".format(classes))
    n, c, h, w = logits.shape
    lib = _lib.lib()
    pi = 1 if per_image else 0
    loss = torch.empty((), device=logits.device, dtype=torch.float32)
    grad = torch.empty_like(logits) if want_grad else None
    probs = torch.empty_like(logits) if want_probs else None
    nbytes = lib.rs_lovasz_softmax_workspace_bytes(n, c, h, w, pi)
    _call("rs_lovasz_softmax_fwd", _dev(logits, "logits"), _dev(targets, "targets", torch.int64), _dev(loss, "loss"), _dev(grad, "grad"),
          _dev(probs, "probs"), n, c, h, w, pi, 1 if classes == "all" else 0, _workspace(nbytes, logits.device), _stream())
    return loss, grad, probs


def scale_by_scalar(src, scalar):
    out = torch.empty_like(src)
    _call("rs_scale_by_scalar", _dev(src, "src"), _dev(scalar, "scalar"), _dev(out, "out"), src.numel(), _stream())
    return out


def confusion_counts(scores, targets, counts):

    n, c, h, w = scores.shape
    _call("rs_confusion_counts", _dev(scores, "scores"), _dev(targets, "targets", torch.int64), _dev(counts, "counts", torch.int64), n, c,
          h, w, _stream())
    return counts


def confusion_matrix(scores, targets, counts):

    n, c, h, w = scores.shape
    assert counts.numel() == c * c
    _call("rs_confusion_matrix", _dev(scores, "scores"), _dev(targets, "targets", torch.int64), _dev(counts, "counts", torch.int64), n, c,
          h, w, _stream())
    return counts


def label_histogram_u8(labels, counts256):

    _call("rs_label_histogram_u8", _dev(labels, "labels", torch.uint8), labels.numel(), _dev(counts256, "counts", torch.int64), _stream())
    return counts256


def softvote_masks(quantized, weights=None):

    if quantized.dim() == 2:
        quantized = quantized.unsqueeze(-1)
    k, p, cq = quantized.shape
    out = torch.empty(p, device=quantized.device, dtype=torch.uint8)
    wt = None if weights is None else torch.as_tensor(list(weights), dtype=torch.float64).to(quantized.device)
    _call("rs_softvote_masks", _dev(quantized, "quantized", torch.uint8), _dev(wt, "weights", torch.float64),
          _dev(_anchors(quantized.device), "anchors", torch.float64), _dev(out, "out", torch.uint8), k, p, cq + 1, _stream())
    return out


def augment_tiles(images, masks, index, op, mean, std):

    t, s, s2, c = images.shape
    assert s == s2, "square tiles (a 90-degree rotation must keep the shape)"
    n = index.numel()
    out = torch.empty((n, c, s, s), device=images.device, dtype=torch.float32)
    om = torch.empty((n, s, s), device=images.device, dtype=torch.int64) if masks is not None else None
    fm, fs = (ctypes.c_float * c)(*mean), (ctypes.c_float * c)(*std)
    _call("rs_augment_tiles", _dev(images, "images", torch.uint8), _dev(masks, "masks", torch.uint8), _dev(index, "index", torch.int32),
          _dev(op, "op", torch.int32), fm, fs, _dev(out, "out"), _dev(om, "out_masks", torch.int64), n, s, c, _stream())
    return out, om


CLEAN_AUTO, CLEAN_LDS, CLEAN_HBM = 0, 1, 2


def disc_rows(eps):

    import math

    r = c = eps // 2
    rows = []
    for i in range(eps):
        dy = i - r
        rows.append(int(round(c * math.sqrt((r * r - dy * dy) / (r * r)))) if r else 0)
    return rows


def disc(eps):

    import numpy as np

    k = np.zeros((eps, eps), dtype=np.uint8)
    c = eps // 2
    for i, dx in enumerate(disc_rows(eps)):
        k[i, max(c - dx, 0):min(c + dx + 1, eps)] = 1
    return k


def _disc_arg(eps):
    if eps < 0 or eps > 64:
        raise ValueError("robosat_amd: disc diameter must be in 0..64, got {}".format(eps))
    return (ctypes.c_int32 * max(eps, 1))(*(disc_rows(eps) or [0]))


def clean_form(h, w):

    return _lib.lib().rs_features_clean_form(h, w)


def clean_masks(images_u8, index, eps_open, eps_close, form=CLEAN_AUTO):

    b, h, w = images_u8.shape
    out = torch.empty_like(images_u8)
    lib = _lib.lib()
    ws = None
    if form != CLEAN_LDS:
        ws = torch.empty(lib.rs_features_clean_workspace_bytes(b, h, w), device=images_u8.device, dtype=torch.uint8)
    _call("rs_features_clean", _dev(images_u8, "images", torch.uint8), _dev(out, "out", torch.uint8), _dev(ws, "workspace", torch.uint8), b,
          h, w, index, eps_open, _disc_arg(eps_open), eps_close, _disc_arg(eps_close), form, _stream())
    return out


def label_components(masks):

    b, h, w = masks.shape
    labels = torch.empty((b, h, w), device=masks.device, dtype=torch.int32)
    err = torch.zeros(1, device=masks.device, dtype=torch.int32)
    _call("rs_features_label", _dev(masks, "masks", torch.uint8), _dev(labels, "labels", torch.int32), _dev(err, "err", torch.int32), b, h,
          w, _stream())
    if int(err.item()):
        raise RuntimeError("rs_features_label: a union-find loop ran out of its H*W bound (code {})".format(int(err.item())))
    return labels


def component_table(labels, min_area=0):

    b, h, w = labels.shape
    dev = labels.device
    slotmap = torch.empty((b, h, w), device=dev, dtype=torch.int32)
    counters = torch.empty(2, device=dev, dtype=torch.int32)
    capacity = 1 << 16
    for _ in range(2):
        raw = torch.empty((capacity, 6), device=dev, dtype=torch.int32)
        table = torch.empty((capacity, 7), device=dev, dtype=torch.int32)
        _call("rs_features_components", _dev(labels, "labels", torch.int32), _dev(slotmap, "slotmap", torch.int32),
              _dev(raw, "raw", torch.int32), _dev(table, "table", torch.int32), _dev(counters, "counters", torch.int32), capacity, b, h, w,
              int(min_area), _stream())
        found, kept = counters.tolist()
        if found <= capacity:
            break
        capacity = found
    else:
        raise RuntimeError("rs_features_components: {} components do not fit a table of {}".format(found, capacity))
    table = table[:kept]
    order = torch.argsort(table[:, 0].to(torch.int64) * (h * w + 1) + table[:, 1].to(torch.int64))
    return table[order].contiguous()


def boundary_edges(labels, table):

    b, h, w = labels.shape
    dev = labels.device
    keep = torch.empty(b * h * w, device=dev, dtype=torch.uint8)
    counter = torch.empty(1, device=dev, dtype=torch.int32)
    table = table.contiguous()

    def run(edges, capacity):
        _call("rs_features_edges", _dev(labels, "labels", torch.int32), _dev(table, "table", torch.int32) if len(table) else None,
              len(table), _dev(keep, "keep", torch.uint8), _dev(edges, "edges", torch.int32), capacity,
              _dev(counter, "counter", torch.int32), b, h, w, _stream())
        return int(counter.item())

    n = run(None, 0)
    edges = torch.empty((n, 5), device=dev, dtype=torch.int32)
    if n:
        got = run(edges, n)
        assert got == n, (got, n)
    return edges


def halo_apron(eps_open, eps_close):

    return (eps_open if eps_open > 1 else 0) + (eps_close if eps_close > 1 else 0)


def _halo(src, nbr, apron, fill, crop):
    t, hs, ws = src.shape
    h, w = (hs - 2 * apron, ws - 2 * apron) if crop else (hs, ws)
    if apron < 0 or h <= 0 or w <= 0 or apron > min(h, w):
        raise ValueError("robosat_amd: an apron of {} does not fit tiles of {}x{} (at most min(H, W))".format(apron, h, w))
    out = torch.empty((t, h, w) if crop else (t, h + 2 * apron, w + 2 * apron), device=src.device, dtype=torch.uint8)
    _call("rs_features_halo", _dev(src, "src", torch.uint8), _dev(out, "out", torch.uint8), _dev(nbr, "nbr", torch.int32), t, h, w, apron,
          fill, int(crop), _stream())
    return out


def gather_halo(images_u8, nbr, apron, fill=0):

    assert nbr.shape == (images_u8.shape[0], 8), "nbr is [T, 8]"
    return _halo(images_u8, nbr, apron, fill, False)


def crop_halo(padded_u8, apron):

    return _halo(padded_u8, None, apron, 0, True)


def clean_masks_stitched(images_u8, nbr, index, eps_open, eps_close):

    apron = halo_apron(eps_open, eps_close)
    if apron == 0:
        return clean_masks(images_u8, index, eps_open, eps_close)
    padded = gather_halo(images_u8, nbr, apron, fill=255 if index == 0 else 0)
    return crop_halo(clean_masks(padded, index, eps_open, eps_close), apron)


def stitch_labels(labels, nbr, inplace=False):

    t, h, w = labels.shape
    assert nbr.shape == (t, 8), "nbr is [T, 8]"
    out = labels if inplace else labels.clone()
    err = torch.zeros(1, device=labels.device, dtype=torch.int32)
    _call("rs_features_stitch_labels", _dev(out, "labels", torch.int32), _dev(nbr, "nbr", torch.int32), _dev(err, "err", torch.int32), t, h,
          w, _stream())
    if int(err.item()):
        raise RuntimeError("rs_features_stitch_labels: a union-find loop ran out of its T*H*W bound (code {})".format(int(err.item())))
    return out


def component_table_stitched(labels, origin, min_area=0):

    t, h, w = labels.shape
    assert origin.shape == (t, 2), "origin is [T, 2]"
    dev = labels.device
    slotmap = torch.empty((t, h, w), device=dev, dtype=torch.int32)
    counters = torch.empty(2, device=dev, dtype=torch.int32)
    capacity = 1 << 16
    for _ in range(2):
        raw = torch.empty((capacity, 6), device=dev, dtype=torch.int32)
        table = torch.empty((capacity, 6), device=dev, dtype=torch.int32)
        _call("rs_features_components_stitched", _dev(labels, "labels", torch.int32), _dev(origin, "origin", torch.int32),
              _dev(slotmap, "slotmap", torch.int32), _dev(raw, "raw", torch.int32), _dev(table, "table", torch.int32),
              _dev(counters, "counters", torch.int32), capacity, t, h, w, int(min_area), _stream())
        found, kept = counters.tolist()
        if found <= capacity:
            break
        capacity = found
    else:
        raise RuntimeError("rs_features_components_stitched: {} components do not fit a table of {}".format(found, capacity))
    table = table[:kept]
    return table[torch.argsort(table[:, 0])].contiguous()


def boundary_edges_stitched(labels, nbr, origin, table):

    t, h, w = labels.shape
    assert nbr.shape == (t, 8) and origin.shape == (t, 2)
    dev = labels.device
    keep = torch.empty(t * h * w, device=dev, dtype=torch.uint8)
    counter = torch.empty(1, device=dev, dtype=torch.int32)
    table = table.contiguous()

    def run(edges, capacity):
        _call("rs_features_edges_stitched", _dev(labels, "labels", torch.int32), _dev(nbr, "nbr", torch.int32),
              _dev(origin, "origin", torch.int32), _dev(table, "table", torch.int32) if len(table) else None, len(table),
              _dev(keep, "keep", torch.uint8), _dev(edges, "edges", torch.int32), capacity, _dev(counter, "counter", torch.int32), t, h, w,
              _stream())
        return int(counter.item())

    n = run(None, 0)
    edges = torch.empty((n, 4), device=dev, dtype=torch.int32)
    if n:
        got = run(edges, n)
        assert got == n, (got, n)
    return edges


def stitched_features(images_u8, nbr, origin, index, eps_open, eps_close, min_area=0):

    labels = stitch_labels(label_components(clean_masks_stitched(images_u8, nbr, index, eps_open, eps_close)), nbr, inplace=True)
    table = component_table_stitched(labels, origin, min_area)
    return table, boundary_edges_stitched(labels, nbr, origin, table)


THIN_PAIRS = 16


def thin_masks(masks_u8, nbr=None, pairs=None, want_pairs=False):

    b, h, w = masks_u8.shape
    pairs = THIN_PAIRS if pairs is None else int(pairs)
    if pairs < 1:
        raise ValueError("robosat_amd: thinning enqueues at least one pair per chunk, got {}".format(pairs))
    if nbr is not None:
        assert nbr.shape == (b, 8), "nbr is [T, 8]"
    dev = masks_u8.device
    out = torch.empty_like(masks_u8)
    masks, outp = _dev(masks_u8, "masks", torch.uint8), _dev(out, "out", torch.uint8)
    ws = torch.empty(max(_lib.lib().rs_features_clean_workspace_bytes(b, h, w), 1), device=dev, dtype=torch.uint8)
    counters = torch.empty(2, device=dev, dtype=torch.int32)
    done = 0
    while True:
        _call("rs_features_thin", masks, outp, _dev(ws, "workspace", torch.uint8), _dev(nbr, "nbr", torch.int32),
              _dev(counters, "counters", torch.int32), b, h, w, pairs, int(done > 0), _stream())
        done += pairs
        if counters[1].item() == 0:
            return (out, done) if want_pairs else out
        if done > b * h * w:
            raise RuntimeError("rs_features_thin: no fixed point after {} pairs on {} pixels".format(done, b * h * w))


def skeleton_links(skeleton, labels, table, nbr=None, origin=None):

    b, h, w = labels.shape
    if (nbr is None) != (origin is None):
        raise ValueError("robosat_amd: nbr and origin come together")
    assert skeleton.shape == labels.shape, "skeleton and labels are both [B, H, W]"
    if nbr is not None:
        assert nbr.shape == (b, 8) and origin.shape == (b, 2)
    dev = labels.device
    keep = torch.empty(b * h * w, device=dev, dtype=torch.uint8)
    counter = torch.empty(1, device=dev, dtype=torch.int32)
    table = table.contiguous()
    width = 5 if nbr is None else 4
    assert table.shape[1:] == (width + 2,), "table rows do not match the form"

    def run(links, capacity):
        _call("rs_features_skeleton_links", _dev(skeleton, "skeleton", torch.uint8), _dev(labels, "labels", torch.int32),
              _dev(nbr, "nbr", torch.int32), _dev(origin, "origin", torch.int32), _dev(table, "table", torch.int32) if len(table) else None,
              len(table), _dev(keep, "keep", torch.uint8), _dev(links, "links", torch.int32), capacity,
              _dev(counter, "counter", torch.int32), b, h, w, _stream())
        return int(counter.item())

    n = run(None, 0)
    links = torch.empty((n, width), device=dev, dtype=torch.int32)
    if n:
        got = run(links, n)
        assert got == n, (got, n)
    return links


def stitched_centerlines(images_u8, nbr, origin, index, eps_open, eps_close, min_area=0):

    cleaned = clean_masks_stitched(images_u8, nbr, index, eps_open, eps_close)
    labels = stitch_labels(label_components(cleaned), nbr, inplace=True)
    table = component_table_stitched(labels, origin, min_area)
    return table, skeleton_links(thin_masks(cleaned, nbr), labels, table, nbr, origin)
```

Baseline: 1631 tiles/s.

## Add split-K fp32 implicit-GEMM path for small phase-upsample convolutions

Adds a split-K variant of the fp32 implicit-GEMM conv kernel. Each K slice writes partial sums to a workspace, and a separate reduce kernel sums the slices and applies scale/shift/residual/relu, including the phase-to-pixel scatter. By default it is enabled only for phase (upsample) convs with at most 16 tiles per image and a deep K. The aim is to fill the GPU on low-parallelism decoder layers, at the cost of an extra workspace round-trip, a second kernel launch and a per-call workspace allocation.

```diff
diff --git a/include/robosat_hip.h b/include/robosat_hip.h
--- a/include/robosat_hip.h
+++ b/include/robosat_hip.h
@@ -168,6 +168,11 @@
 int rs_conv2d_fwd_phase_dt(const rs_conv_desc* d, int dtype, const void* src1, const void* src2, const void* weight_phase,
                            const float* scale, const float* shift, const void* residual, const void* relu_mask, void* out,
                            rs_stream_t stream);
+
+int rs_conv2d_splitk(const rs_conv_desc* d, int form, int* rowb);
+int rs_conv2d_fwd_splitk(const rs_conv_desc* d, int form, const float* src1, const float* src2, const float* weight,
+                         const float* scale, const float* shift, const float* residual, float* out, float* ws, int splits,
+                         rs_stream_t stream);
 
 int rs_conv2d_phase_wino_ok(const rs_conv_desc* d);
 const char* rs_conv2d_phase_wino_name(const rs_conv_desc* d);
diff --git a/robosat_amd/_lib.py b/robosat_amd/_lib.py
--- a/robosat_amd/_lib.py
+++ b/robosat_amd/_lib.py
@@ -93,6 +93,8 @@
     "rs_pack_phase_weight_dt": (c_int, [P, P, c_int, c_int, c_int, P]),
     "rs_pack_s2_dgrad_phase_weight_dt": (c_int, [P, P, c_int, c_int, c_int, P]),
     "rs_conv2d_fwd_phase_dt": (c_int, [POINTER(ConvDesc), c_int, P, P, P, P, P, P, P, P, P]),
+    "rs_conv2d_splitk": (c_int, [POINTER(ConvDesc), c_int, POINTER(c_int)]),
+    "rs_conv2d_fwd_splitk": (c_int, [POINTER(ConvDesc), c_int, P, P, P, P, P, P, P, P, c_int, P]),
     "rs_conv2d_phase_wino_ok": (c_int, [POINTER(ConvDesc)]),
     "rs_conv2d_phase_wino_name": (c_char_p, [POINTER(ConvDesc)]),
     "rs_pack_wino_phase_weight": (c_int, [P, P, c_int, c_int, P]),
diff --git a/robosat_amd/csrc/common.h b/robosat_amd/csrc/common.h
--- a/robosat_amd/csrc/common.h
+++ b/robosat_amd/csrc/common.h
@@ -185,6 +185,7 @@
   int conv_halo = 1;
   int conv_halo_min = 192;
   int conv_halo512 = -1;
+  int conv_splitk = -1;
   int conv1x1_ew = -1;
   int conv1x1_np = 0;
   int conv1x1_ew_bf16 = 0;
diff --git a/robosat_amd/csrc/conv_igemm_dma.hip b/robosat_amd/csrc/conv_igemm_dma.hip
--- a/robosat_amd/csrc/conv_igemm_dma.hip
+++ b/robosat_amd/csrc/conv_igemm_dma.hip
@@ -140,8 +140,64 @@
   return 128;
 }
 
+constexpr int kMaxSplitK = 16;
+int pick_splitk(const rs_conv_desc* d, bool phase4, bool plain) {
+  const int knob = rs_knobs().conv_splitk;
+  const int ft = tuning().tile;
+  if (knob == 0 || !plain || (ft >= 0 && ft != T64x64)) return 0;
+  const long n32 = (long)(phase4 ? 4 : d->kh * d->kw) * (d->C1 + d->C2) / 32;
+  int s = knob;
+  if (knob < 0) {
+    const long tiles_per_image = (long)rs_cdiv(phase4 ? d->Hs * d->Ws : d->Ho * d->Wo, 64) * rs_cdiv(d->Cout, 64) * (phase4 ? 4 : 1);
+    s = (phase4 && tiles_per_image <= 16 && n32 >= 128) ? 4 : 0;
+  }
+  if (s > kMaxSplitK) s = kMaxSplitK;
+  return s > n32 ? (int)n32 : s;
+}
+
+__global__ __launch_bounds__(256) void splitk_reduce_f32(const float* __restrict__ ws, int S, long rows, int M, int Cout,
+                                                         const float* __restrict__ scale, const float* __restrict__ shift,
+                                                         const float* __restrict__ res, float* __restrict__ out, int relu, int phase,
+                                                         int HsWs, int Ws, int Ho, int Wo) {
+  const int cp = Cout >> 2;
+  const long i = (long)blockIdx.x * 256 + threadIdx.x;
+  if (i >= rows * cp) return;
+  const long r = i / cp;
+  const int col = (int)(i - r * cp) * 4;
+  const long slice = rows * Cout;
+  const float* src = ws + r * Cout + col;
+  f32x4 v = *reinterpret_cast<const f32x4*>(src);
+#pragma unroll 4
+  for (int s = 1; s < S; ++s) {
+    const f32x4 t = *reinterpret_cast<const f32x4*>(src + s * slice);
+#pragma unroll
+    for (int e = 0; e < 4; ++e) v[e] += t[e];
+  }
+  long opix = r;
+  if (phase) {
+    const int par = (int)(r / M), m = (int)(r - (long)par * M);
+    const int n = m / HsWs, rem = m - n * HsWs;
+    const int a = rem / Ws, b = rem - a * Ws;
+    opix = ((long)n * Ho + 2 * a + (par >> 1)) * Wo + 2 * b + (par & 1);
+  }
+  const long o = opix * Cout + col;
+#pragma unroll
+  for (int e = 0; e < 4; ++e) v[e] = v[e] * (scale ? scale[col + e] : 1.f) + (shift ? shift[col + e] : 0.f);
+  if (res) {
+    const f32x4 t = *reinterpret_cast<const f32x4*>(res + o);
+#pragma unroll
+    for (int e = 0; e < 4; ++e) v[e] += t[e];
+  }
+  if (relu) {
+#pragma unroll
+    for (int e = 0; e < 4; ++e) v[e] = fmaxf(v[e], 0.f);
+  }
+  *reinterpret_cast<f32x4*>(out + o) = v;
+}
+
 void launch(int rowb, bool phase4, int epi, int tile, int grid, hipStream_t s, const ConvArgsT<float>& a) {
-  if (phase4) rs_conv_launch_f32_phase_eval(tile, rowb, grid, s, a);
+  if (epi == EPI_SPLITK) (phase4 ? rs_conv_launch_f32_phase_splitk : rs_conv_launch_f32_plain_splitk)(tile, rowb, grid, s, a);
+  else if (phase4) rs_conv_launch_f32_phase_eval(tile, rowb, grid, s, a);
   else if (epi == EPI_STATS) rs_conv_launch_f32_plain_stats(tile, rowb, grid, s, a);
   else if (epi == EPI_BWD) rs_conv_launch_f32_plain_bwd(tile, rowb, grid, s, a);
   else rs_conv_launch_f32_plain_eval(tile, rowb, grid, s, a);
@@ -221,8 +277,9 @@
              const float* shift, const void* residual, const void* relu_mask, void* out, rs_stream_t stream,
              float* stats = nullptr, const void* bn_y = nullptr, const float* bn_mean = nullptr,
              const float* bn_invstd = nullptr, bool phase4 = false, void* out2 = nullptr, const void* mask2 = nullptr,
-             int csplit = 0, const unsigned char* mask_bits = nullptr) {
+             int csplit = 0, const unsigned char* mask_bits = nullptr, float* ws = nullptr, int splits = 0) {
   if (!valid(d) || !src1 || !weight || !out) return RS_EINVAL;
+  if (ws && (sizeof(T) != 4 || stats || relu_mask || out2 || mask_bits || splits < 1 || splits != pick_splitk(d, phase4, true))) return RS_EINVAL;
   if (mask_bits && (relu_mask || !bn_y || (d->Cout & 7))) return RS_EINVAL;
   if (out2 && (csplit <= 0 || csplit >= d->Cout || residual || stats)) return RS_EINVAL;
   if (phase4 && (!phase_ok(d) || stats)) return RS_EINVAL;
@@ -288,6 +345,10 @@
   a.Kw = a.nk * kc;
   a.relu = d->relu;
   a.tpx = a.tpi = 0;
+  if (ws) {
+    a.ws = ws;
+    a.ksplit = splits;
+  }
 
   int epi = EPI_EVAL;
   if (stats) {
@@ -297,6 +358,17 @@
     if (epi == EPI_BWD && (!bn_mean || !bn_invstd)) return RS_EINVAL;
   }
   if constexpr (sizeof(T) == 4) {
+    if (ws) {
+      a.ntiles = rs_cdiv(d->Cout, 64);
+      const long rows = M * (phase4 ? 4 : 1);
+      const long grid = (long)rs_cdiv(M, 64) * a.ntiles * (phase4 ? 4 : 1) * splits;
+      if (grid >= (1L << 31) || rows * d->Cout / 4 >= (1L << 31) * 256) return RS_EINVAL;
+      hipStream_t s = (hipStream_t)stream;
+      launch(kc == kc128 ? 128 : 64, phase4, EPI_SPLITK, T64x64, (int)grid, s, a);
+      splitk_reduce_f32<<<(unsigned)rs_cdiv(rows * (d->Cout / 4), 256), 256, 0, s>>>(ws, splits, rows, (int)M, d->Cout, scale, shift, a.res, a.out, d->relu,
+                                                                                phase4 ? 1 : 0, d->Hs * d->Ws, d->Ws, d->Ho, d->Wo);
+      return RS_LAUNCH_RESULT();
+    }
     if (ew_f32_mode(d, phase4, epi == EPI_EVAL && !relu_mask && !out2 && !mask_bits)) return rs_conv1x1_ew_f32_launch(a, (hipStream_t)stream);
 #ifdef RS_EXP_BUILD
     if (np_f32_mode(d, phase4, epi == EPI_EVAL && !relu_mask && !out2 && !mask_bits, residual != nullptr)) return rs_conv1x1_np_f32_launch(a, (hipStream_t)stream);
@@ -389,6 +461,22 @@
   return 0;
 }
 
+extern "C" int rs_conv2d_splitk(const rs_conv_desc* d, int form, int* rowb) {
+  if (form < 0 || form > 3) return RS_EINVAL;
+  const bool phase4 = (form & 1) != 0;
+  if (!valid(d) || (phase4 && !phase_ok(d))) return RS_EINVAL;
+  if (rowb) *rowb = pick_rowb(d, 4, phase4) == 128 ? 128 : 64;
+  return pick_splitk(d, phase4, (form & 2) == 0);
+}
+
+extern "C" int rs_conv2d_fwd_splitk(const rs_conv_desc* d, int form, const float* src1, const float* src2, const float* weight,
+                                    const float* scale, const float* shift, const float* residual, float* out, float* ws, int splits,
+                                    rs_stream_t stream) {
+  if (form < 0 || form > 1 || !ws || (d && d->stem)) return RS_EINVAL;
+  return conv_fwd<float>(d, src1, src2, weight, scale, shift, residual, nullptr, out, stream, nullptr, nullptr, nullptr, nullptr,
+                         form == 1, nullptr, nullptr, 0, nullptr, ws, splits);
+}
+
 template <typename T>
 __global__ void pack_phase_weight_kernel(const float* __restrict__ w, T* __restrict__ out, int Cout, int Cin, long total) {
   const long i = (long)blockIdx.x * blockDim.x + threadIdx.x;
diff --git a/robosat_amd/csrc/conv_igemm_dma_f32_splitk.hip b/robosat_amd/csrc/conv_igemm_dma_f32_splitk.hip
--- /dev/null
+++ b/robosat_amd/csrc/conv_igemm_dma_f32_splitk.hip
@@ -0,0 +1,5 @@
+#define RS_CONV_INSTANTIATE
+#include "conv_igemm_dma_kernel.h"
+
+RS_CONV_DEFINE_SPLITK_LAUNCHER(rs_conv_launch_f32_plain_splitk, false)
+RS_CONV_DEFINE_SPLITK_LAUNCHER(rs_conv_launch_f32_phase_splitk, true)
diff --git a/robosat_amd/csrc/conv_igemm_dma_kernel.h b/robosat_amd/csrc/conv_igemm_dma_kernel.h
--- a/robosat_amd/csrc/conv_igemm_dma_kernel.h
+++ b/robosat_amd/csrc/conv_igemm_dma_kernel.h
@@ -6,7 +6,7 @@
 
 #include "lds_dma.h"
 
-enum { EPI_EVAL = 0, EPI_STATS = 1, EPI_BWD = 2 };
+enum { EPI_EVAL = 0, EPI_STATS = 1, EPI_BWD = 2, EPI_SPLITK = 3 };
 constexpr int kMaxK = 4;
 enum Tile { T128x128 = 0, T128x64, T128x32, T64x64, TSTEM_RESERVED, T256x128, T256x256, TTHIN, THALO, TEW, NTILES };
 enum { HALO_NONE = 0, HALO_33 = 1, HALO_PHASE = 2, HALO_DG4 = 3 };
@@ -21,14 +21,20 @@
   const T* res;
   const T* mask;
   T* out;
-  float* stats;
+  union {
+    float* stats;
+    float* ws;
+  };
   const T* bn_y;
   const float* bn_mean;
   const float* bn_invstd;
   const unsigned char* mask_bits;
   T* out2;
   const T* mask2;
-  int csplit;
+  union {
+    int csplit;
+    int ksplit;
+  };
   int N, Hs, Ws, C1, C2, Hv, Wv, ups;
   int kh, kw, stride, pad, Ho, Wo, Cout;
   int M, cpt, nk, Kw, relu, ntiles, ntaps, phase4;
@@ -42,6 +48,8 @@
 RS_CONV_LAUNCHER(rs_conv_launch_f32_plain_stats, float);
 RS_CONV_LAUNCHER(rs_conv_launch_f32_plain_bwd, float);
 RS_CONV_LAUNCHER(rs_conv_launch_f32_phase_eval, float);
+RS_CONV_LAUNCHER(rs_conv_launch_f32_plain_splitk, float);
+RS_CONV_LAUNCHER(rs_conv_launch_f32_phase_splitk, float);
 RS_CONV_LAUNCHER(rs_conv_launch_bf16_plain_eval, bf16_t);
 RS_CONV_LAUNCHER(rs_conv_launch_bf16_plain_stats, bf16_t);
 RS_CONV_LAUNCHER(rs_conv_launch_bf16_plain_bwd, bf16_t);
@@ -174,6 +182,9 @@
   static_assert(!HL || (sizeof(T) == 2 && NW == 8 && (IB % NW) == 0 && WM % 32 == 0 && HNT >= 4 && KS % 2 == 0 && (HALO == HALO_PHASE) == PHASE),
                 "halo forms: bf16, 8 waves, whole weight DMA instructions per wave");
   static_assert(MAINB + TABN * 4 <= 160 * 1024, "LDS");
+  constexpr bool SPLIT = EPI == EPI_SPLITK;
+  constexpr bool STATS = EPI == EPI_STATS || EPI == EPI_BWD;
+  static_assert(!SPLIT || (ES == 4 && !HL), "split K: the fp32 implicit-GEMM forms");
 
   __shared__ __attribute__((aligned(16))) unsigned char smem[MAINB + TABN * 4];
   int* taby = reinterpret_cast<int*>(smem + MAINB);
@@ -191,6 +202,12 @@
     py = (bid >> 1) & 1;
     px = bid & 1;
     bid >>= 2;
+  }
+  int ksl = 0;
+  if constexpr (SPLIT) {
+    const int tps = (int)(gridDim.x >> (PHASE ? 2 : 0)) / p.ksplit;
+    ksl = bid / tps;
+    bid -= ksl * tps;
   }
   const int mt = bid / p.ntiles, nt = bid - mt * p.ntiles;
   const int m0 = mt * BM, n0 = nt * BN;
@@ -270,6 +287,18 @@
     }
   };
   int lr = 0, ls = 0, lc = 0, lk = 0;
+  int nkl = p.nk;
+  if constexpr (SPLIT) {
+    const int u32 = KC == 32 ? 1 : 2, n32 = p.nk / u32;
+    const int k0 = (int)((long)ksl * n32 / p.ksplit) * u32, k1 = (int)((long)(ksl + 1) * n32 / p.ksplit) * u32;
+    nkl = k1 - k0;
+    lk = k0;
+    const int tap = k0 / p.cpt;
+    lc = k0 - tap * p.cpt;
+    lr = tap / p.kw;
+    ls = tap - lr * p.kw;
+    if (lc != 0) load_tap(pbase, lr, ls, lc * KC < p.C1);
+  }
   unsigned int fL = lds0;
   __amdgpu_buffer_rsrc_t frs = rsrc1;
   int fsa = 0, fsb = 0;
@@ -322,7 +351,7 @@
     for (int tn = 0; tn < TN; ++tn) b[tn] = *reinterpret_cast<const u32x4*>(L + bbase + 32 * tn * ROWB + foff[s]);
   };
   if constexpr (!HL) {
-  if (p.nk > 0) {
+  if (nkl > 0) {
     begin_chunk(0);
 #pragma unroll
     for (int q = 0; q < NI; ++q) issue_piece(q);
@@ -358,8 +387,8 @@
   };
   if constexpr (!HL) {
     int kc = 0;
-    for (; kc < p.nk - 1; ++kc) chunk(kc, std::true_type());
-    for (; kc < p.nk; ++kc) chunk(kc, std::false_type());
+    for (; kc < nkl - 1; ++kc) chunk(kc, std::true_type());
+    for (; kc < nkl; ++kc) chunk(kc, std::false_type());
   } else {
     constexpr int RPT = WM / 32;
     constexpr int NHI = (HROWS + RI - 1) / RI;
@@ -567,6 +596,7 @@
     }
   }
   T* outp = p.out;
+  if constexpr (SPLIT) outp = p.ws;
   const T* maskp = p.mask;
   int ostride = p.Cout, ocol = col;
   if (EPI == EPI_EVAL && p.out2) {
@@ -593,7 +623,7 @@
   constexpr int NIT = WN / (2 * EPP);
   constexpr int G = (ES == 4 && EPI == EPI_BWD) ? 1 : 2;
   static_assert(NIT * RPI == WGM * 32 && NIT % G == 0, "row groups tile the pass");
-  const bool has_res = EPI != EPI_STATS && p.res != nullptr, has_mask = EPI != EPI_STATS && maskp != nullptr;
+  const bool has_res = EPI != EPI_STATS && !SPLIT && p.res != nullptr, has_mask = EPI != EPI_STATS && !SPLIT && maskp != nullptr;
   const bool has_bits = EPI == EPI_BWD && p.mask_bits != nullptr;
   constexpr bool has_bny = EPI == EPI_BWD;
   auto load_group = [&](int tm, int g0, long (&o)[G], bool (&ok)[G], u32x4 (&rr_)[G], u32x4 (&rm_)[G], u32x4 (&ry_)[G])
@@ -604,7 +634,8 @@
       const int row = (lrow >> 5) * WM + 32 * tm + (lrow & 31);
       const int opix = orow[row];
       ok[i] = opix >= 0 && cvalid;
-      o[i] = ok[i] ? (long)opix * ostride + ocol : 0;
+      if constexpr (SPLIT) o[i] = ok[i] ? (((long)ksl * (PHASE ? 4 : 1) + (2 * py + px)) * p.M + m0 + row) * p.Cout + col : 0;
+      else o[i] = ok[i] ? (long)opix * ostride + ocol : 0;
     }
     if (has_res) {
 #pragma unroll
@@ -672,7 +703,7 @@
         }
       }
       if (ok[i]) Piece<T>::store(outp + o[i], v);
-      if constexpr (EPI != EPI_EVAL) {
+      if constexpr (STATS) {
         float w[EPP];
         Piece<T>::round(v, w);
         const float keep = ok[i] ? 1.f : 0.f;
@@ -724,7 +755,7 @@
       finish_group(g0, o, ok, rr_, rm_, ry_);
     }
   }
-  if constexpr (EPI != EPI_EVAL) {
+  if constexpr (STATS) {
     __syncthreads();
     float* r0 = lds;
     float* r1 = lds + RPI * BN;
@@ -763,6 +794,11 @@
   }
 }
 
+template <int ROWB, bool PHASE>
+void launch_splitk(int grid, hipStream_t s, const ConvArgsT<float>& a) {
+  conv_igemm_dma<float, 64, 64, 2, 2, ROWB, PHASE, EPI_SPLITK><<<grid, 256, 0, s>>>(a);
+}
+
 }
 
 template <int HALO, bool PHASE, int EPI>
@@ -777,4 +813,9 @@
     if (rowb == 128) launch_rows<T, 128, PHASE, EPI>(tile, grid, s, a);                         \
     else launch_rows<T, 64, PHASE, EPI>(tile, grid, s, a);                                      \
   }
+#define RS_CONV_DEFINE_SPLITK_LAUNCHER(name, PHASE)                                              \
+  void name(int, int rowb, int grid, hipStream_t s, const ConvArgsT<float>& a) {                \
+    if (rowb == 128) launch_splitk<128, PHASE>(grid, s, a);                                     \
+    else launch_splitk<64, PHASE>(grid, s, a);                                                  \
+  }
 #endif
diff --git a/robosat_amd/csrc/knobs.hip b/robosat_amd/csrc/knobs.hip
--- a/robosat_amd/csrc/knobs.hip
+++ b/robosat_amd/csrc/knobs.hip
@@ -27,6 +27,7 @@
     {"conv_halo", "RS_CONV_HALO", &RsKnobs::conv_halo, 0, 1},
     {"conv_halo_min", "RS_CONV_HALO_MIN", &RsKnobs::conv_halo_min, 0, 1048576},
     {"conv_halo512", "RS_CONV_HALO512", &RsKnobs::conv_halo512, -1, 1},
+    {"conv_splitk", "RS_CONV_SPLITK", &RsKnobs::conv_splitk, -1, 16},
     {"conv1x1_ew", "RS_CONV1X1_EW", &RsKnobs::conv1x1_ew, -1, 1},
     {"conv1x1_np", "RS_CONV1X1_NP", &RsKnobs::conv1x1_np, -1, 1},
     {"conv1x1_ew_bf16", "RS_CONV1X1_EW_BF16", &RsKnobs::conv1x1_ew_bf16, 0, 1},
diff --git a/robosat_amd/ops.py b/robosat_amd/ops.py
--- a/robosat_amd/ops.py
+++ b/robosat_amd/ops.py
@@ -100,6 +100,31 @@
     if rows <= 0:
         raise ValueError("{}: invalid arguments".format(rows_fn))
     return torch.empty((rows, 2, d.Cout), device=device, dtype=torch.float32)
+
+
+def _splitk(d, device, phase=False, plain=True):
+
+    rowb = ctypes.c_int(0)
+    s = _lib.lib().rs_conv2d_splitk(ctypes.byref(d), int(bool(phase)) | (0 if plain else 2), ctypes.byref(rowb))
+    if s < 0:
+        check(s, "rs_conv2d_splitk")
+    if s == 0:
+        return None, 0
+    return torch.empty((s, d.N * d.Ho * d.Wo, d.Cout), device=device, dtype=torch.float32), rowb.value
+
+
+def _splitk_name(ws, rowb, phase=False, split=False):
+
+    return "conv_igemm_f32<{}64x64,r{}{}>".format("phase," if phase else "", rowb, ",k{}".format(ws.shape[0]) if split else "")
+
+
+def conv_splitk_name(d, phase=False, plain=True):
+
+    rowb = ctypes.c_int(0)
+    s = _lib.lib().rs_conv2d_splitk(ctypes.byref(d), int(bool(phase)) | (0 if plain else 2), ctypes.byref(rowb))
+    if s < 0:
+        check(s, "rs_conv2d_splitk")
+    return "conv_igemm_f32<{}64x64,r{},k{}>".format("phase," if phase else "", rowb.value, s) if s else None
 
 
 def conv_flops(d):
@@ -145,17 +170,23 @@
         assert residual.shape == out.shape
     if relu_mask is not None:
         assert relu_mask.shape == out.shape
-    ev = _start()
-    _call("rs_conv2d_fwd_bf16" if bf else "rs_conv2d_fwd", ctypes.byref(d), _dev(src1, "src1", act), _dev(src2, "src2", act),
-          _dev(weight, "weight", act), _dev(scale, "scale"), _dev(shift, "shift"), _dev(residual, "residual", act),
-          _dev(relu_mask, "relu_mask", act), _dev(out, "out", act), _stream())
-    if ev:
-        _stop(ev)
-        name = conv_tile_name(d, bf, plain=relu_mask is None)
+    ws, ws_rowb = (None, 0) if bf or stem else _splitk(d, src1.device, plain=relu_mask is None)
+    ev = _start()
+    if ws is not None:
+        _call("rs_conv2d_fwd_splitk", ctypes.byref(d), 0, _dev(src1, "src1"), _dev(src2, "src2"), _dev(weight, "weight"), _dev(scale, "scale"),
+              _dev(shift, "shift"), _dev(residual, "residual"), _dev(out, "out"), _dev(ws, "ws"), ws.shape[0], _stream())
+    else:
+        _call("rs_conv2d_fwd_bf16" if bf else "rs_conv2d_fwd", ctypes.byref(d), _dev(src1, "src1", act), _dev(src2, "src2", act),
+              _dev(weight, "weight", act), _dev(scale, "scale"), _dev(shift, "shift"), _dev(residual, "residual", act),
+              _dev(relu_mask, "relu_mask", act), _dev(out, "out", act), _stream())
+    if ev:
+        _stop(ev)
+        name = conv_tile_name(d, bf, plain=relu_mask is None) if ws is None else _splitk_name(ws, ws_rowb)
         if alg_scale != 1.0 and not name.startswith(("conv_thin", "conv_halo")):
             name = name.replace("<", "<dgrad4x4,")
         _record(ev, name, conv_flops(d) * alg_scale, _shape(d),
-                conv_bytes(d, _esize(act), (residual is not None) + (relu_mask is not None)), conv_flops(d))
+                conv_bytes(d, _esize(act), (residual is not None) + (relu_mask is not None)) + (0 if ws is None else 8 * ws.numel()),
+                conv_flops(d))
     return out
 
 
@@ -311,14 +342,20 @@
     act = src1.dtype
     d = _phase_desc(n, hs, ws, c1, c2, cout, relu)
     out = torch.empty((n, 2 * hs, 2 * ws, cout), device=src1.device, dtype=act)
-    ev = _start()
-    _call("rs_conv2d_fwd_phase_dt", ctypes.byref(d), _dt(src1), _dev(src1, "src1", act), _dev(src2, "src2", act),
-          _dev(weight_phase, "weight", act), _dev(scale, "scale"), _dev(shift, "shift"), _dev(residual, "residual", act),
-          _dev(relu_mask, "relu_mask", act), _dev(out, "out", act), _stream())
-    if ev:
-        _stop(ev)
-        _record(ev, conv_tile_name(d, act == BF16, phase=True), conv_flops(d), _shape(d),
-                conv_bytes(d, _esize(act), (residual is not None) + (relu_mask is not None)), conv_flops(d) * 4.0 / 9.0)
+    ws, ws_rowb = (None, 0) if act == BF16 else _splitk(d, src1.device, phase=True, plain=relu_mask is None)
+    ev = _start()
+    if ws is not None:
+        _call("rs_conv2d_fwd_splitk", ctypes.byref(d), 1, _dev(src1, "src1"), _dev(src2, "src2"), _dev(weight_phase, "weight"),
+              _dev(scale, "scale"), _dev(shift, "shift"), _dev(residual, "residual"), _dev(out, "out"), _dev(ws, "ws"), ws.shape[0], _stream())
+    else:
+        _call("rs_conv2d_fwd_phase_dt", ctypes.byref(d), _dt(src1), _dev(src1, "src1", act), _dev(src2, "src2", act),
+              _dev(weight_phase, "weight", act), _dev(scale, "scale"), _dev(shift, "shift"), _dev(residual, "residual", act),
+              _dev(relu_mask, "relu_mask", act), _dev(out, "out", act), _stream())
+    if ev:
+        _stop(ev)
+        _record(ev, conv_tile_name(d, act == BF16, phase=True) if ws is None else _splitk_name(ws, ws_rowb, phase=True), conv_flops(d), _shape(d),
+                conv_bytes(d, _esize(act), (residual is not None) + (relu_mask is not None)) + (0 if ws is None else 8 * ws.numel()),
+                conv_flops(d) * 4.0 / 9.0)
     return out
 
 
```

After: 1652 tiles/s (median of 6 runs). 1.3% higher.
